# fruttasecca/approximated_personalized_pagerank

Measured on AMD Instinct MI355X. Metric: source-nodes/sec grank K=64 L=128 on RMAT-22; 1/2/4/8 MI355X + HBM GB/s, higher is better.
Workload: dtype f64

## Files before the change

approximated_personalized_pagerank_amd/csrc/grank.hip:

```cpp
#include <hip/hip_runtime.h>
#include <rccl/rccl.h>
#include <hipcub/hipcub.hpp>

#include <algorithm>
#include <atomic>
#include <chrono>
#include <cmath>
#include <condition_variable>
#include <cstdio>
#include <cstdlib>
#include <cstring>
#include <mutex>
#include <new>
#include <thread>
#include <vector>

#include "../../include/ppr_hip.h"
#include "merge_wave.h"
#include "wg_merge.h"
#include "merge_hub.h"
#include "merge_glb.h"
#include "merge_hot.h"
#include "merge_xs.h"
#include "merge_sv.h"
// ... 48 lines not shown
    for (int j = 0; j < l; j++) below += (uint32_t)__shfl((int)slot, j) == slot;
    if (below == 0) bad |= prev != 0xffffffffull;
    else bad |= (uint32_t)prev == 0xffffffffu || got != below;
    wave_fence();
  }
  if (bad) atomicAnd(&ok[1], 0);
}

}

int plan_alloc(int64_t n, const int64_t* row_ptr, const int32_t* colx, uint32_t K, uint32_t L,
               double damping, const ppr_opts* o, ppr_plan** out, bool mc) {
  const int64_t m = n ? row_ptr[n] : 0;
  for (int64_t v = 0; v < n; v++)
    if ((row_ptr[v + 1] - row_ptr[v]) * (int64_t)L + 1 > (int64_t)INT32_MAX) return PPR_ERR_RANGE;
  ppr_plan* p = new (std::nothrow) ppr_plan();
  if (!p) return PPR_ERR_OOM;
  p->n = n; p->m = m; p->K = K; p->L = L; p->damping = damping;
  p->Lp = pow2_at_least(L);
  p->flags = o ? o->flags : 0;
  p->device = (o && o->device >= 0) ? o->device : -1;
  if (p->device >= 0) { if (hipSetDevice(p->device) != hipSuccess) { plan_free(p); return PPR_ERR_HIP; } }
  else { if (hipGetDevice(&p->device) != hipSuccess) { plan_free(p); return PPR_ERR_HIP; } }
  if (o && o->stream) p->stream = (hipStream_t)o->stream;
  else {
    if (hipStreamCreateWithFlags(&p->stream, hipStreamNonBlocking) != hipSuccess) { plan_free(p); return PPR_ERR_HIP; }
    p->own_stream = true;
  }
  if (hipEventCreate(&p->ev_a) != hipSuccess || hipEventCreate(&p->ev_b) != hipSuccess ||
      hipEventCreate(&p->ev_m0) != hipSuccess || hipEventCreate(&p->ev_m1) != hipSuccess) { plan_free(p); return PPR_ERR_HIP; }

  {
    const char* env = getenv("PPR_TIER_MASK");
    const int mask = env ? (int)strtol(env, nullptr, 0) : 0xef;
    int T0 = 256;
    for (int t = 0; t < NT; t++) {
      const int T = T0 << t;
      if (!((mask >> t) & 1) || lds_wave_bytes(T, p->Lp) * WAVES_PER_BLOCK > 160 * 1024) { p->tierT[t] = 0; p->tierCap[t] = 0; continue; }
      p->tierT[t] = T;
      p->tierCap[t] = T / 4 * 3;
    }
    p->tierCap[NT] = 0;
    p->wg_lds = wg_lds_bytes(WG_T, p->Lp, wg_pl(p->Lp));
    const int pmax = WG_TIER_PASSES;
    p->hub_enabled = ((mask >> (NT + 1)) & 1) && pmax >= 1 && p->wg_lds <= 160 * 1024;
    if (((mask >> NT) & 1) && pmax >= 1 && p->wg_lds <= 160 * 1024)
      p->tierCap[NT] = pmax * WG_PASS_CAP;
    int run = 0;
    for (int t = 0; t <= NT; t++) {
      if (!p->tierCap[t]) continue;
      if (p->tierCap[t] < run) p->tierCap[t] = 0;
      else run = p->tierCap[t];
    }
  }
  std::vector<int32_t> all(n > 0 ? n : 1);
  {
    int64_t k = 0;
    for (int64_t v = 0; v < n; v++)
      if (row_ptr[v + 1] > row_ptr[v]) all[k++] = (int32_t)v;
    p->n_nd = k;
    for (int64_t v = 0; v < n; v++)
      if (row_ptr[v + 1] == row_ptr[v]) all[k++] = (int32_t)v;
  }
  p->h_rp.assign(row_ptr, row_ptr + n + 1);
  for (int64_t v = 0; v < n; v++) p->max_deg = std::max<int64_t>(p->max_deg, row_ptr[v + 1] - row_ptr[v]);

  const size_t slab = (size_t)2 * n * L;
  TRY(dalloc(&p->d_rp, n + 1));
  TRY(dalloc(&p->d_colx, m));
  TRY(dalloc(&p->d_part, n));
  TRY(dalloc(&p->d_ids, slab));
  TRY(dalloc(&p->d_sc, slab));
  TRY(dalloc(&p->d_len, 2 * n));
  TRY(dalloc(&p->d_rix, (size_t)2 * n * NRANGE));
  TRY(dalloc(&p->d_rmin, 2 * n));
  TRY(dalloc(&p->d_all, n));
  TRY(dalloc(&p->d_cand, n));
  TRY(dalloc(&p->d_tier_lists, (size_t)NLISTS * (n > 0 ? n : 1)));
  TRY(dalloc(&p->d_tier_cnt, NLISTS + 2));
  TRY(dalloc(&p->d_big, n));
  TRY(dalloc(&p->d_tier_cap, NT + 1));
  TRY(dalloc(&p->d_ovf, n));
  TRY(dalloc(&p->d_maxdiff, PPR_MAX_ITER_STATS + 1));
  TRY(dalloc(&p->d_stats, PPR_NSTATS));
  TRY(dalloc(&p->d_out_ids, (size_t)n * K));
  TRY(dalloc(&p->d_out_sc, (size_t)n * K));
  TRY(dalloc(&p->d_out_len, n));
  if (getenv("PPR_DIAG")) {
    TRY(dalloc(&p->d_diag, PPR_DIAG_SLOTS));
    if (hipMemset(p->d_diag, 0, PPR_DIAG_SLOTS * 8) != hipSuccess) { plan_free(p); return PPR_ERR_HIP; }
  }
  hipStream_t st = p->stream;
  if (n) {
    if (hipMemcpyAsync(p->d_rp, row_ptr, 8 * (n + 1), hipMemcpyHostToDevice, st) != hipSuccess ||
        (m && hipMemcpyAsync(p->d_colx, colx, 4 * m, hipMemcpyHostToDevice, st) != hipSuccess) ||
        hipMemsetAsync(p->d_part, 0, n, st) != hipSuccess ||
        hipMemsetAsync(p->d_len, 0, 8 * n, st) != hipSuccess ||
        hipMemsetAsync(p->d_rix, 0, sizeof(uint16_t) * 2 * n * NRANGE, st) != hipSuccess ||
        hipMemsetAsync(p->d_rmin, 0, 16 * n, st) != hipSuccess ||
        hipMemcpyAsync(p->d_all, all.data(), 4 * n, hipMemcpyHostToDevice, st) != hipSuccess) {
      plan_free(p); return PPR_ERR_HIP;
    }
  }
  int32_t caps[NT + 1];
  for (int t = 0; t <= NT; t++) caps[t] = p->tierCap[t];
  if (hipMemcpyAsync(p->d_tier_cap, caps, sizeof(caps), hipMemcpyHostToDevice, st) != hipSuccess ||
      hipStreamSynchronize(st) != hipSuccess) { plan_free(p); return PPR_ERR_HIP; }
  for (int t = 0; t < NT; t++)
    if (p->tierT[t]) {
      const size_t bytes = lds_wave_bytes(p->tierT[t], p->Lp) * WAVES_PER_BLOCK;
      if (bytes > 64 * 1024) {
        hipFuncSetAttribute((const void*)k_merge_lds<false>, hipFuncAttributeMaxDynamicSharedMemorySize, 160 * 1024);
        hipFuncSetAttribute((const void*)k_merge_lds<true>, hipFuncAttributeMaxDynamicSharedMemorySize, 160 * 1024);
        hipFuncSetAttribute((const void*)k_merge_lds<false, true>, hipFuncAttributeMaxDynamicSharedMemorySize, 160 * 1024);
        hipFuncSetAttribute((const void*)k_merge_lds<true, true>, hipFuncAttributeMaxDynamicSharedMemorySize, 160 * 1024);
      }
    }
  if (p->tierCap[NT])
    hipFuncSetAttribute((const void*)k_merge_wg, hipFuncAttributeMaxDynamicSharedMemorySize, 160 * 1024);
  p->hub_lds_wg = wg_lds_bytes(WG_T, p->Lp, wg_pl(p->Lp));
  p->hub_lds_final = wg_lds_bytes(0, p->Lp, 0);
  {
    const char* e1 = getenv("PPR_HUB_BUCKET");
    const char* e2 = getenv("PPR_HUB_WAVE_T");
    p->hub_bucket = e1 ? std::max(64, atoi(e1)) : (mc ? HUB_BUCKET_MC : HUB_BUCKET);
    p->hub_wave_t = e2 ? (std::max(256, atoi(e2)) + 63) / 64 * 64 : (mc ? HUB_WAVE_T_MC : HUB_WAVE_T);
    p->hub_wave_t = std::min(p->hub_wave_t, 8192);
    const char* e17 = getenv("PPR_BW_FILL");
    const int fill = e17 ? std::max(50, std::min(100, atoi(e17))) : 85;
    p->hub_bw_budget = std::max(WAVE, std::min(p->hub_wave_t, p->hub_wave_t * fill / 100));
  }
  {
    const char* e4 = getenv("PPR_BW_NG");
    const char* e5 = getenv("PPR_BW_WAVES");
    const char* s1 = getenv("PPR_HUB_SEG");
    const char* s2 = getenv("PPR_SEG_BUCKET");
    const char* s3 = getenv("PPR_SEG_T");
    const char* s4 = getenv("PPR_SEG_WPB");
    p->seg_enabled = s1 ? atoi(s1) != 0 : false;

    p->seg_bucket = s2 ? std::max(32, atoi(s2)) : 256;
    p->seg_t = s3 ? pow2_at_least(std::max(256, atoi(s3))) : 512;
    p->seg_t = std::min(p->seg_t, 4096);
    p->seg_wpb = s4 ? std::max(1, std::min(4, atoi(s4))) : 1;
    p->hub_bw_ng = e4 ? (atoi(e4) == 8 ? 8 : atoi(e4) == 4 ? 4 : atoi(e4) == 1 ? 1 : 2) : 2;
    p->hub_bw_waves = e5 ? std::max(1, std::min(4, atoi(e5))) : 1;
    const char* e19 = getenv("PPR_HUB_RANGE");
    if (e19) p->hub_range = std::max(0, std::min(32, atoi(e19)));
    const char* e6 = getenv("PPR_HUB_SLICE");
    p->hub_slice = std::max<int>(std::max<int>(64, (int)L), e6 ? atoi(e6) : HUB_SLICE);
    const char* e21 = getenv("PPR_RED_LDS");
    const size_t red_lds = wg_lds_bytes(0, p->Lp, p->hub_slice);
    p->red_pl = (!(e21 && atoi(e21) == 0) && red_lds <= 160 * 1024) ? p->hub_slice : 0;
    p->hub_lds_red = p->red_pl ? red_lds : p->hub_lds_final;
    if (p->red_pl)
      hipFuncSetAttribute((const void*)k_hub_reduce, hipFuncAttributeMaxDynamicSharedMemorySize, 160 * 1024);
    const char* e7 = getenv("PPR_HUB_STREAMS");
    p->hub_streams = (e7 && atoi(e7) == 1) ? 1 : 2;
    const char* e14 = getenv("PPR_WAVE_WPB");
    p->wave_wpb = e14 ? (atoi(e14) >= 4 ? 4 : atoi(e14) >= 2 ? 2 : 1) : 1;
    const char* e15 = getenv("PPR_TILE_WPB_P");
    p->tile_wpb_p = e15 ? std::max(1, atoi(e15)) : 4096;
    const char* e18 = getenv("PPR_HUB_REGIONS");
    p->hub_regions = e18 ? std::max(2, std::min(ppr_plan::MAX_REGIONS, atoi(e18))) : 3;
    const char* e10 = getenv("PPR_HUB_MIX");
    p->hub_mix = e10 ? std::max(0, std::min(HUB_MAX_LOGP, atoi(e10))) : 6;
    const char* e9 = getenv("PPR_HUB_TILE_PB");
    p->hub_tile_pb = e9 ? std::max(0, std::min(64, atoi(e9))) : HUB_TILE_PER_BUCKET;
    const char* e9b = getenv("PPR_HUB_TILE_CAND");
    if (e9b) p->hub_tile_cand = std::max(256, std::min(1 << 20, atoi(e9b)));
    const char* ets = getenv("PPR_TILE_SPLIT_LOGP");
    if (ets) p->tile_split_logp = std::max(0, std::min(HUB_MAX_LOGP, atoi(ets)));
    const char* esp = getenv("PPR_SPEC");
    if (esp) p->spec_ratio = std::max(0.0, std::min(1.0, atof(esp)));
    const char* esf = getenv("PPR_SPEC_FROM");
    if (esf) p->spec_from = std::max(0, atoi(esf));
    const char* ent = getenv("PPR_NT");
    if (ent) p->nt_loads = (int)strtol(ent, nullptr, 0) & 3;
    const char* ewi = getenv("PPR_WHATIF");
    if (ewi) p->whatif = (int)strtol(ewi, nullptr, 0);
    const char* ebd = getenv("PPR_WAVE_BY_D");
    if (ebd) p->wave_by_d = atoi(ebd) != 0;
    const char* etd = getenv("PPR_WAVE_TDIV");
    if (etd) p->wave_tdiv = std::max(0, std::min(6, atoi(etd)));
    const char* exr = getenv("PPR_XROUTE");
    if (exr && atoi(exr) == 0) p->xroute = false;
    const char* exb = getenv("PPR_XTEST_BADSIZE");
    if (exb) p->xtest_badsize = atoi(exb);
    const char* erp = getenv("PPR_TEST_RANK_PERMUTE");
    p->rank_permute = erp && atoi(erp) != 0;
    const char* exf = getenv("PPR_XTEST_FAIL");
    if (exf && sscanf(exf, "%d,%d", &p->xtest_fail_rank, &p->xtest_fail_it) != 2) p->xtest_fail_rank = -1;
    const char* ext = getenv("PPR_XTIMEOUT");
    if (ext) p->x_timeout_s = std::max(1.0, atof(ext));
    const char* e9e = getenv("PPR_WG_PASSES");
    if (e9e) p->wg_max_passes = std::max(1, std::min(WG_MAX_PASSES, atoi(e9e)));
    const char* e9d = getenv("PPR_FUSED_MAX");
    if (e9d) p->fused_max = std::max(0LL, atoll(e9d));
    const char* e9c = getenv("PPR_HUB_LONG_MIN");
    if (e9c) p->hub_long_min = std::max(0LL, atoll(e9c));
    const char* e8 = getenv("PPR_HUB_BUDGET");
    if (e8) p->hub_budget = std::max<int64_t>(1024, std::min<int64_t>(1LL << 28, atoll(e8)));
    const char* h1 = getenv("PPR_HOT_N");
    const char* h2 = getenv("PPR_HOT_AT");
    const char* h3 = getenv("PPR_HOT_STRIDE");
    if (h1) p->hot_cap = std::max(0, std::min(16384, atoi(h1)));
    if (h2) p->hot_at = std::max(0, atoi(h2));
    if (h3) p->hot_stride = std::max(1, atoi(h3));
    if (hot_wave_lds(p->hot_cap) > 160 * 1024) p->hot_cap = 0;
    const char* h4 = getenv("PPR_HOT_MAX");
    if (h4) p->hot_max_need = std::max(0, atoi(h4));
  }
  {
    const char* e = getenv("PPR_BW2");
    p->hub_bw2 = !(e && atoi(e) == 0);
  }
  p->hub_wave_stride = (int)std::max(hub_wave_lds(p->hub_wave_t, p->hub_bw_ng), p->hub_bw2 ? bw2_lds(p->hub_wave_t) : 0);
  p->hub_lds_wave = (size_t)p->hub_wave_stride * p->hub_bw_waves;
  if (p->hub_streams == 2) {
    const char* epr = getenv("PPR_SV_PRIO");
    int prio_lo = 0, prio_hi = 0;
    hipDeviceGetStreamPriorityRange(&prio_lo, &prio_hi);
    const int prio4 = (epr && atoi(epr) == 1) ? prio_hi : (epr && atoi(epr) == 2) ? prio_lo : 0;
    if (hipStreamCreateWithFlags(&p->stream2, hipStreamNonBlocking) != hipSuccess ||
        hipStreamCreateWithPriority(&p->stream4, hipStreamNonBlocking, prio4) != hipSuccess ||
        hipStreamCreateWithFlags(&p->stream3, hipStreamNonBlocking) != hipSuccess ||
        hipEventCreateWithFlags(&p->ev_wave, hipEventDisableTiming) != hipSuccess) { plan_free(p); return PPR_ERR_HIP; }
    if (hipStreamCreateWithFlags(&p->stream5, hipStreamNonBlocking) != hipSuccess ||
        hipEventCreateWithFlags(&p->ev_hot0, hipEventDisableTiming) != hipSuccess) { plan_free(p); return PPR_ERR_HIP; }
    for (int i = 0; i < ppr_plan::MAX_REGIONS; i++)
      if (hipEventCreateWithFlags(&p->ev_part[i], hipEventDisableTiming) != hipSuccess ||
          hipEventCreateWithFlags(&p->ev_buck[i], hipEventDisableTiming) != hipSuccess ||
          hipEventCreateWithFlags(&p->ev_fin[i], hipEventDisableTiming) != hipSuccess ||
          hipEventCreateWithFlags(&p->ev_hot[i], hipEventDisableTiming) != hipSuccess) { plan_free(p); return PPR_ERR_HIP; }
  }
  p->stream_wave = p->stream3;
  {
    hipDeviceProp_t prop;
    p->num_cus = hipGetDeviceProperties(&prop, p->device) == hipSuccess ? prop.multiProcessorCount : 256;
    const int per_cu = std::max<int>(1, std::min<int>(32 / p->hub_bw_waves, (int)((160 * 1024) / p->hub_lds_wave)));
    p->hub_bw_blocks = p->num_cus * per_cu;
  }
  {
    const char* e = getenv("PPR_LDS_RANK");
    int* d_ok = nullptr;
    int ok[2] = {0, 0};
    if ((!e || atoi(e) != 0) && hipMalloc(&d_ok, sizeof(ok)) == hipSuccess) {
      ok[0] = ok[1] = 1;
      if (hipMemcpy(d_ok, ok, sizeof(ok), hipMemcpyHostToDevice) == hipSuccess) {
        hipFuncSetAttribute((const void*)k_probe_lds_rank, hipFuncAttributeMaxDynamicSharedMemorySize, 160 * 1024);
        hipLaunchKernelGGL(k_probe_lds_rank, dim3((unsigned)p->hub_bw_blocks), dim3(64 * p->hub_bw_waves),
                           p->hub_lds_wave, p->stream, d_ok, 64, p->hub_wave_t,
                           p->hub_wave_stride);
        if (hipGetLastError() != hipSuccess || hipStreamSynchronize(p->stream) != hipSuccess ||
            hipMemcpy(ok, d_ok, sizeof(ok), hipMemcpyDeviceToHost) != hipSuccess)
          ok[0] = ok[1] = 0;
      } else {
        ok[0] = ok[1] = 0;
      }
      hipFree(d_ok);
    }
    p->lds_rank = ok[0] ? 1u : 0u;
    p->lds_rank64 = ok[1] ? 1u : 0u;
// ... 293 lines not shown
  const auto t4 = now();
  std::vector<int32_t> act[2];
  for (int64_t v = 0; v < n; v++)
    if (g->row_ptr[v + 1] > g->row_ptr[v]) act[part[v]].push_back((int32_t)v);
  for (int q = 0; q < 2; q++) {
    p->work[q].resize(act[q].size());
    pprh::parallel_for((int64_t)act[q].size(), nth, [&](int64_t b, int64_t e2, int) {
      for (int64_t i = b; i < e2; i++) {
        const int v = act[q][i];
        double w = 1.0;
        for (int64_t e = g->row_ptr[v]; e < g->row_ptr[v + 1]; e++) {
          const int u = g->col[e];
          w += (double)std::min<int64_t>(L, g->row_ptr[u + 1] - g->row_ptr[u] + 1);
        }
        p->work[q][i] = w;
      }
    });
  }
  if (timing)
    fprintf(stderr, "ppr_timing plan_create partitions_s %.3f colx_s %.3f alloc_upload_s %.3f work_s %.3f\n",
            sec(t0, t1) + part_dev_s, sec(t1, t2), sec(t2, t3), sec(t4, now()));
  p->nact[0] = (int64_t)act[0].size();
  p->nact[1] = (int64_t)act[1].size();
  if (p->hot_cap > 0 && n > 0) {
    std::vector<int32_t> indeg(n, 0);
    for (int64_t e = 0; e < m; e++) indeg[g->col[e]]++;
    p->hot_list_cap = p->hot_cap + 2 * std::min<int64_t>(n, 1 << 20);
    TRY(dalloc(&p->d_hot_bits, (n + 31) / 32));
    TRY(dalloc(&p->d_hot_idx, n));
    TRY(dalloc(&p->d_hot_keys, p->hot_cap));
    TRY(dalloc(&p->d_hot_w, n));
    TRY(dalloc(&p->d_hot_hist, HOT_BINS + 2));
    TRY(dalloc(&p->d_hot_list, p->hot_list_cap));
    TRY(dalloc(&p->d_indeg, n));
    if (hipMemcpy(p->d_indeg, indeg.data(), 4 * (size_t)n, hipMemcpyHostToDevice) != hipSuccess) {
      plan_free(p); return PPR_ERR_HIP;
    }
  } else {
    p->hot_cap = 0;
  }
  TRY(dalloc(&p->d_act[0], p->nact[0]));
  TRY(dalloc(&p->d_act[1], p->nact[1]));
  hipStream_t st = p->stream;
  if (n) {
    if (hipMemcpyAsync(p->d_part, part.data(), n, hipMemcpyHostToDevice, st) != hipSuccess ||
        (p->nact[0] && hipMemcpyAsync(p->d_act[0], act[0].data(), 4 * p->nact[0], hipMemcpyHostToDevice, st) != hipSuccess) ||
        (p->nact[1] && hipMemcpyAsync(p->d_act[1], act[1].data(), 4 * p->nact[1], hipMemcpyHostToDevice, st) != hipSuccess) ||
        hipStreamSynchronize(st) != hipSuccess) {
      plan_free(p); return PPR_ERR_HIP;
    }
  }
  *out = p;
  return PPR_OK;
}

extern "C" void ppr_grank_plan_destroy(ppr_plan* p) { plan_free(p); }
extern "C" void* ppr_grank_plan_stream(ppr_plan* p) { return p ? (void*)p->stream : nullptr; }

static IterArgs iter_args(const ppr_plan* p, int it, bool unit) {
  IterArgs a;
  a.damping = p->damping;
  a.mc = 0u;
  a.rp = p->d_rp;
  a.diag = p->d_diag;
  a.unit = unit ? 1u : 0u;
  a.stats = (p->flags & PPR_FLAG_STATS) ? 1u : 0u;
  a.lds_rank = p->lds_rank;
  a.nt = (uint32_t)p->nt_loads;
  a.whatif = ((uint32_t)p->whatif & 0xffffu) | (p->sv_p2skip ? 0u : WI_SV_NO_P2SKIP) |
             (p->rank_permute ? WI_RANK_PERMUTE : 0u);
  a.iter = unit ? -1 : it;
  a.spec = (unit || p->hot_cap > 0 || it < p->spec_from) ? 0.0 : p->spec_ratio;
  a.xs = p->xsum ? 1u : 0u;
  a.xsf = XS_F;
  if (unit) { a.sA = 0; a.sB = 0; a.active = -1; return a; }
  a.sA = ((it + 1) / 2) & 1;
  a.sB = (it / 2) & 1;
  a.active = it & 1;
  return a;
}

static int run_merge_impl(ppr_plan* p, const IterArgs& a, const int32_t* list, int64_t count,
                          unsigned long long* maxdiff);

static int ensure_scratch(ppr_plan* p, size_t need) {
  if (need <= p->scratch_bytes) return PPR_OK;
  HIP_OK(hipStreamSynchronize(p->stream));
  hipFree(p->d_scratch);
  p->d_scratch = nullptr;
  p->scratch_bytes = 0;
  if (hipMalloc(&p->d_scratch, need) != hipSuccess) return PPR_ERR_OOM;
  p->scratch_bytes = need;
  return PPR_OK;
}

static int ensure_dev(unsigned char** ptr, size_t* cap, size_t need);

static int ceil_log2(int64_t x) { return x <= 1 ? 0 : 64 - __builtin_clzll((unsigned long long)(x - 1)); }

static int run_hubs(ppr_plan* p, const IterArgs& a, const int32_t* big,
                    const int32_t* cand , size_t nbig, unsigned long long* maxdiff,
                    std::vector<int32_t>& fallback, const int32_t* dest = nullptr) {
  hipStream_t st = p->stream;
  DevGraph g{p->d_rp, p->d_colx, p->n};
  const DevSlab s = dev_slab(p);
  const int64_t L = p->L;
  const int64_t budget = p->hub_budget;
  const auto t_plan0 = std::chrono::steady_clock::now();
  p->last_nbig = (int64_t)nbig;
  p->last_maxneed = 0;
  for (size_t i = 0; i < nbig; i++) p->last_maxneed = std::max<int64_t>(p->last_maxneed, cand[i]);
  const int slice = p->hub_slice;
  using Batch = HubBatch;
  std::vector<Batch>& batches = p->hub_batches;
  batches.clear();
  {
    int rc0 = ensure_pinned(&p->h_desc_pin, &p->h_desc_bytes, sizeof(HubDesc) * (nbig + 1));
    if (rc0) return rc0;
  }
  HubDesc* desc = (HubDesc*)p->h_desc_pin;
  size_t nd_all = 0;
  const bool hot = p->hot_n > 0 && !a.unit && !a.mc;
  const HotSet H{p->d_hot_bits, p->d_hot_idx, p->d_hot_keys, hot ? p->hot_n : 0};
  const uint32_t hb = (uint32_t)p->hub_bucket, sgb = (uint32_t)p->seg_bucket;
  auto cdiv32 = [](uint32_t x, uint32_t d) { return x / d + (x % d != 0); };
  auto logp_of = [&](int64_t need) {
    return std::max(1, std::min(HUB_MAX_LOGP, ceil_log2((int64_t)cdiv32((uint32_t)need, hb))));
  };
  std::vector<uint8_t> lpv(nbig);
  if (a.xs) {
    const int64_t capb = (int64_t)p->xr_T * p->xr_fill / 100;
    for (size_t i = 0; i < nbig; i++)
      lpv[i] = (uint8_t)std::max(1, std::min(p->hub_max_logp, ceil_log2((dest[i] + capb - 1) / capb)));
  } else {
    for (size_t i = 0; i < nbig; i++) lpv[i] = (uint8_t)logp_of(cand[i]);
  }
  std::vector<uint32_t> order(nbig);
  if (p->hub_mix > 0) {
    std::vector<uint32_t> lg, sm;
    lg.reserve(nbig);
    sm.reserve(nbig);
    for (size_t i = 0; i < nbig; i++) (lpv[i] >= p->hub_mix ? lg : sm).push_back((uint32_t)i);
    size_t a0 = 0, b0 = 0, k = 0;
    while (a0 < lg.size() || b0 < sm.size()) {
      const bool take_lg = b0 >= sm.size() || (a0 < lg.size() && a0 * sm.size() <= b0 * lg.size());
      order[k++] = take_lg ? lg[a0++] : sm[b0++];
    }
  } else {
    for (size_t i = 0; i < nbig; i++) order[i] = (uint32_t)i;
  }
  const auto t_plan1 = std::chrono::steady_clock::now();
  int64_t need_all = 0;
  for (size_t i = 0; i < nbig; i++) need_all += cand[i];
  const int tile_pb = need_all >= p->hub_long_min ? p->hub_tile_pb : 1;
  int tw_of[HUB_MAX_LOGP + 1], nsl_of[HUB_MAX_LOGP + 1];
  int64_t ptc_of[HUB_MAX_LOGP + 1];
  for (int lp = 0; lp <= HUB_MAX_LOGP; lp++) {
    const int64_t tcand = std::max<int64_t>(p->hub_tile_cand, (int64_t)tile_pb << lp);
    const int64_t tw0 = std::max<int64_t>(1, tcand / L);
    tw_of[lp] = (int)(tw0 > WAVE ? (tw0 + WAVE - 1) / WAVE * WAVE : tw0);
    ptc_of[lp] = (int64_t)(1 << lp) * L;
    nsl_of[lp] = ptc_of[lp] > 2 * slice ? (int)((ptc_of[lp] + slice - 1) / slice) : 0;
  }
  {
    size_t oi = 0;
    while (oi < nbig) {
// ... 387 lines not shown
    const size_t o_b = off;  off = al(off + 8 * (size_t)T);
    const size_t o_st = off; off = al(off + sizeof(XgState));
    const size_t o_h = off;  off = al(off + 4 * (size_t)XG_BINS);
    const size_t o_e = off;  off = al(off + 4);
    const size_t zeroed = off;
    const size_t o_dk = off; off = al(off + 4 * (size_t)XG_CAP);
    const size_t o_dv = off; off = al(off + 8 * (size_t)XG_CAP);
    { int rc = ensure_dev(&p->d_xg, &p->xg_bytes, off); if (rc) return rc; }
    unsigned char* b = p->d_xg;
    uint32_t* keys = (uint32_t*)(b + o_k);
    unsigned long long* A = (unsigned long long*)(b + o_a);
    unsigned long long* B = (unsigned long long*)(b + o_b);
    XgState* stp = (XgState*)(b + o_st);
    uint32_t* hist = (uint32_t*)(b + o_h);
    int32_t* err = (int32_t*)(b + o_e);
    int32_t* dk = (int32_t*)(b + o_dk);
    double* dv = (double*)(b + o_dv);
    HIP_OK(hipMemsetAsync(b, 0, zeroed, st));
    const int64_t deg = p->h_rp[v + 1] - p->h_rp[v];
    const int64_t blocks = std::max<int64_t>(1, (deg + 4 * WAVE - 1) / (4 * WAVE));
    hipLaunchKernelGGL(k_xg_walk, dim3((unsigned)blocks), dim3(256), 0, st, g, s, a, v, T, keys, A, B, stp);
    HIP_OK(hipGetLastError());
    const unsigned gb = (unsigned)std::min<int64_t>(2048, (T + 1023) / 1024);
    for (int lvl = 0; lvl < XG_LEVELS; lvl++) {
      hipLaunchKernelGGL(k_xg_hist, dim3(gb), dim3(1024), 0, st, v, T, keys, A, B, stp, lvl, hist, a.xsf);
      HIP_OK(hipGetLastError());
      hipLaunchKernelGGL(k_xg_pick, dim3(1), dim3(256), 0, st, stp, lvl, hist, (int)p->L, p->xg_cap);
      HIP_OK(hipGetLastError());
    }
    hipLaunchKernelGGL(k_xg_compact, dim3((unsigned)std::min<int64_t>(8192, (T + 255) / 256)), dim3(256), 0, st, v, T,
                       keys, A, B, stp, dk, dv, a.xsf);
    HIP_OK(hipGetLastError());
    hipLaunchKernelGGL(k_xg_fin, dim3(1), dim3(64), xg_fin_lds_bytes(p->Lp), st, s, a, v, stp, dk, dv, p->Lp, maxdiff,
                       p->d_stats, err);
    HIP_OK(hipGetLastError());
    p->merge_launches += 4 + 2 * XG_LEVELS;
    int32_t herr = 0;
    HIP_OK(hipMemcpyAsync(&herr, err, 4, hipMemcpyDeviceToHost, st));
    HIP_OK(hipStreamSynchronize(st));
    if (herr) return PPR_ERR_HIP;
    p->xg_sources++;
  }
  return PPR_OK;
}

static void kst_reset(ppr_plan* p) {
  for (int g = 0; g < ppr_plan::NKST; g++) {
    p->kst_ms[g] = 0.0; p->kst_bytes[g] = 0.0; p->kst_pend_bytes[g] = 0.0;
    p->kst_launches[g] = 0; p->kst_live[g] = false;
  }
}
static void kst_begin(ppr_plan* p, int g, hipStream_t s) {
  if (!p->ev_k[2 * g] && hipEventCreate(&p->ev_k[2 * g]) != hipSuccess) return;
  if (!p->ev_k[2 * g + 1] && hipEventCreate(&p->ev_k[2 * g + 1]) != hipSuccess) return;
  hipEventRecord(p->ev_k[2 * g], s);
}
static void kst_end(ppr_plan* p, int g, hipStream_t s, double bytes) {
  if (!p->ev_k[2 * g + 1]) return;
  hipEventRecord(p->ev_k[2 * g + 1], s);
  p->kst_live[g] = true;
  p->kst_pend_bytes[g] = bytes;
}
static void kst_fold(ppr_plan* p, int g) {
  if (!p->kst_live[g]) return;
  p->kst_live[g] = false;
  float ms = 0.f;
  if (hipEventElapsedTime(&ms, p->ev_k[2 * g], p->ev_k[2 * g + 1]) == hipSuccess) {
    p->kst_ms[g] += ms;
    p->kst_bytes[g] += p->kst_pend_bytes[g];
    p->kst_launches[g]++;
  }
}

struct XhDefer {
  bool want = false;
  bool live = false;
  int depth = 0;
  size_t o_ov = 0;
  const std::vector<int32_t>* src = nullptr;
  const std::vector<int32_t>* cand = nullptr;
  const std::vector<int32_t>* deg = nullptr;
  const std::vector<int64_t>* dest = nullptr;
  std::vector<int32_t> xv;
};
static int xhubs_finish(ppr_plan* p, const IterArgs& a, XhDefer& df, unsigned long long* maxdiff);

static inline void sub_lap(ppr_plan* p, int k, std::chrono::steady_clock::time_point& t) {
  const auto t2 = std::chrono::steady_clock::now();
  p->xh_sub[k] += std::chrono::duration<double>(t2 - t).count();
  t = t2;
}

static int run_xhubs_list(ppr_plan* p, const IterArgs& a, const std::vector<int32_t>& src,
                          const std::vector<int32_t>& cand, const std::vector<int32_t>& deg,
                          const std::vector<int64_t>& dest, unsigned long long* maxdiff, int depth,
                          XhDefer* defer = nullptr) {
  const size_t n = src.size();
  if (!n) return PPR_OK;
  auto tsub = std::chrono::steady_clock::now();
  hipStream_t st = p->stream;
  hipStream_t sw = p->stream3 ? p->stream3 : st;
  DevGraph g{p->d_rp, p->d_colx, p->n};
  const DevSlab s = dev_slab(p);
  const int64_t L = p->L;
  struct Cls { int T, W; };
  const Cls cls[3] = {{std::min(2048, p->xr_T), std::min(2048, p->xr_T) / 512},
                      {std::min(4096, p->xr_T), std::min(4096, p->xr_T) / 512},
                      {p->xr_T, p->xr_T / 512}};
  auto cap_of = [&](int T) { return (int64_t)T * p->xr_fill / 100; };
  static thread_local std::vector<int32_t> rng_tl;
  static thread_local std::vector<uint8_t> ci_tl;
  static thread_local std::vector<XDesc> xd_tl;
  static thread_local std::vector<XTask> tasks_tl[3];
  std::vector<int32_t>& rng = rng_tl;
  std::vector<uint8_t>& ci = ci_tl;
  rng.resize(n);
  ci.resize(n);
  std::vector<int32_t> bsrc, bcand;
  std::vector<int32_t> bdest;
  const int64_t capA = cap_of(p->xr_T);
  const int64_t reach = capA << p->hub_max_logp;
  constexpr int XG_REDO = 8;
  std::vector<int32_t> xgs, xgc;
  for (size_t i = 0; i < n; i++) {
    const int64_t R = std::max<int64_t>(1, (dest[i] + capA - 1) / capA);
    if (depth > XG_REDO || (p->hub_enabled && R > p->xr_rmax && dest[i] > reach)) {
      rng[i] = -1;
      xgs.push_back(src[i]);
      xgc.push_back(cand[i]);
    } else if (R <= p->xr_rmax || !p->hub_enabled) {
      rng[i] = (int32_t)R;
      int c = 2;
      if (R == 1) c = dest[i] <= cap_of(cls[0].T) ? 0 : dest[i] <= cap_of(cls[1].T) ? 1 : 2;
      ci[i] = (uint8_t)c;
    } else {
      rng[i] = 0;
      bsrc.push_back(src[i]);
      bdest.push_back((int32_t)std::min<int64_t>(dest[i], INT32_MAX));
    }
  }
  sub_lap(p, 0, tsub);
  std::vector<XDesc>& xd = xd_tl;
  std::vector<XTask>* tasks = tasks_tl;
  xd.clear();
  for (int c = 0; c < 3; c++) tasks[c].clear();
  xd.reserve(n);
  tasks[0].reserve(n);
  int64_t pt = 0;
  for (int pass = 0; pass < 2; pass++)
    for (size_t i = 0; i < n; i++) {
      if (rng[i] <= 0 || (rng[i] > 1) != (pass == 0)) continue;
      const int32_t d = (int32_t)xd.size();
      XDesc x;
      x.v = src[i];
      x.R = rng[i];
      x.pt_off = pt;
      x.factor = a.mc ? 1.0 : p->damping / (double)deg[i];
      x.selfval = a.mc ? 1.0 / (p->damping / (double)deg[i]) : 1.0 - p->damping;
      pt += rng[i] == 1 ? (int64_t)std::max<int64_t>(L, p->xr_cap) : (int64_t)rng[i] * L;
      xd.push_back(x);
      for (int r = 0; r < rng[i]; r++) tasks[ci[i]].push_back(XTask{d, r});
    }
  sub_lap(p, 1, tsub);
  int64_t nmulti = 0;
  for (const XDesc& x : xd) nmulti += x.R > 1;
  const size_t nx = xd.size();
  const bool use_xm = p->xm && !a.unit && p->Lp <= 2 * WAVE && xm_lds_bytes(cls[0].T) <= 160 * 1024;
  std::vector<XmTask> xmt;
  if (use_xm) {
    xmt.reserve(tasks[0].size());
    for (const XTask& t : tasks[0]) {
      const XDesc& x = xd[(size_t)t.d];
      xmt.push_back(XmTask{x.pt_off, x.factor, x.selfval, t.d, x.v});
    }
    tasks[0].clear();
  }
  size_t ntask = 0;
  for (int c = 0; c < 3; c++) ntask += tasks[c].size();
  auto al = [](size_t x) { return (x + 255) & ~(size_t)255; };
  size_t off = 0;
  const size_t o_d = off;  off = al(off + sizeof(XDesc) * (nx + 1));
  const size_t o_t = off;  off = al(off + sizeof(XTask) * (ntask + 1));
  const size_t o_m = off;  off = al(off + sizeof(XmTask) * (xmt.size() + 1));
  const size_t o_k = off;  off = al(off + 4 * (size_t)(pt + 1));
  const size_t o_s = off;  off = al(off + 8 * (size_t)(pt + 1));
  const size_t o_z = off;
  const size_t o_pc = off; off = al(off + 4 * (nx + 1));
  const size_t o_ds = off; off = al(off + 4 * (nx + 1));
  const size_t o_of = off; off = al(off + 4 * (nx + 1));
  const size_t o_ov = off; off = al(off + 4 * (nx + 2));
  const size_t o_xt = off; off = al(off + 8 * (nx + 1));
  const size_t total = off;
  std::vector<int32_t> ovl_h;
  if (nx) {
    {
      int rc = ensure_dev(&p->d_xs, &p->xs_bytes, total);
      if (rc) return rc;
    }
    unsigned char* b = p->d_xs;
    XDesc* d_xd = (XDesc*)(b + o_d);
    XTask* d_tk = (XTask*)(b + o_t);
    int32_t* d_pk = (int32_t*)(b + o_k);
    double* d_ps = (double*)(b + o_s);
    uint32_t* d_pc = (uint32_t*)(b + o_pc);
    uint32_t* d_ds = (uint32_t*)(b + o_ds);
    int32_t* d_of = (int32_t*)(b + o_of);
    int32_t* d_ov = (int32_t*)(b + o_ov);
    unsigned long long* d_xt = (unsigned long long*)(b + o_xt);
    const size_t up = o_m + sizeof(XmTask) * xmt.size();
    {
      int rc = ensure_pinned(&p->h_xs_pin, &p->h_xs_bytes, up);
      if (rc) return rc;
    }
    unsigned char* hb = (unsigned char*)p->h_xs_pin;
    std::memcpy(hb + o_d, xd.data(), sizeof(XDesc) * nx);
    if (!xmt.empty()) std::memcpy(hb + o_m, xmt.data(), sizeof(XmTask) * xmt.size());
    size_t tofs[3];
    {
      size_t k = 0;
      for (int c = 0; c < 3; c++) {
        tofs[c] = k;
        if (!tasks[c].empty()) std::memcpy(hb + o_t + sizeof(XTask) * k, tasks[c].data(), sizeof(XTask) * tasks[c].size());
        k += tasks[c].size();
      }
    }
    sub_lap(p, 2, tsub);
    HIP_OK(hipMemcpyAsync(b, hb, up, hipMemcpyHostToDevice, sw));
    HIP_OK(hipMemsetAsync(b + o_z, 0, total - o_z, sw));
    if (!a.unit && !a.mc) {
      double bytes = 0.0;
      for (size_t i = 0; i < n; i++)
        if (rng[i] > 0)
          bytes += 8.0 + 8.0 * deg[i] + 12.0 * ((double)cand[i] - 1.0) +
                   24.0 * (double)std::min<int64_t>(L, (int64_t)cand[i] + 1) + 4.0;
      kst_begin(p, 5, sw);
      p->kst_pend_bytes[5] = bytes;
    }
    const bool big_first = p->xr_big_first;
    if (!xmt.empty()) {
      const int T = cls[0].T, W = cls[0].W;
      const int budget = p->xr_budget_over ? 2 * T : std::min(T * 85 / 100, T - W * WAVE - WAVE);
      hipLaunchKernelGGL(k_xm<4>, dim3((unsigned)xmt.size()), dim3(64 * 4), xm_lds_bytes(T), sw, g, s, a,
                         (const XmTask*)(b + o_m), T, budget, d_pk, d_ps, d_pc, d_ds, d_of, d_ov);
      HIP_OK(hipGetLastError());
      p->merge_launches++;
    }
    for (int c0 = 0; c0 < 3; c0++) {
      const int c = big_first ? 2 - c0 : c0;
      if (tasks[c].empty()) continue;
      const int T = cls[c].T, W = cls[c].W;
      const int budget = p->xr_budget_over ? 2 * T : std::min(T * 85 / 100, T - W * WAVE - WAVE);
      hipLaunchKernelGGL(k_xr, dim3((unsigned)tasks[c].size()), dim3(64 * W), xr_lds_bytes(T, W, p->Lp), sw, g, s, a,
                         d_xd, d_tk + tofs[c], T, budget, p->Lp, d_xt, d_pk, d_ps, d_pc, d_ds, d_of, d_ov, p->xr_cap);
      HIP_OK(hipGetLastError());
      p->merge_launches++;
    }
    if (nmulti) {
      hipLaunchKernelGGL(k_xfinal<XDesc>, dim3((unsigned)nmulti), dim3(256), xf_lds_bytes(p->Lp, p->xf_stage), sw, s, a,
                         d_xd, d_xt, d_pk, d_ps, d_pc, d_ds, d_of, p->d_dlast, p->Lp, p->xf_stage, maxdiff, p->d_stats);
      HIP_OK(hipGetLastError());
      p->merge_launches++;
    }
    if ((int64_t)nx > nmulti) {
      hipLaunchKernelGGL(k_xfin1, dim3((unsigned)((int64_t)nx - nmulti)), dim3(64), xf1_lds_bytes(p->Lp), sw, s, a, d_xd,
                         (int)nmulti, d_pk, d_ps, d_pc, d_ds, d_of, p->d_dlast, p->Lp, maxdiff, p->d_stats);
      HIP_OK(hipGetLastError());
      p->merge_launches++;
    }
    if (!a.unit && !a.mc) kst_end(p, 5, sw, p->kst_pend_bytes[5]);
  }
  sub_lap(p, 3, tsub);
  if (defer && defer->want && nx && bsrc.empty() && xgs.empty()) {
    defer->live = true;
    defer->depth = depth;
    defer->o_ov = o_ov;
    defer->src = &src; defer->cand = &cand; defer->deg = &deg; defer->dest = &dest;
    defer->xv.resize(nx);
    for (size_t i = 0; i < nx; i++) defer->xv[i] = xd[i].v;
    return PPR_OK;
  }
  std::vector<int32_t> fallback;
  if (!bsrc.empty()) {
    const size_t nb = bsrc.size();
    std::vector<int32_t> cd(2 * nb);
    {
      size_t k = 0;
      for (size_t i = 0; i < n; i++)
        if (rng[i] == 0) { cd[k] = cand[i]; cd[nb + k] = deg[i]; k++; }
    }
    int rc = run_hubs(p, a, bsrc.data(), cd.data(), nb, maxdiff, fallback, bdest.data());
    if (rc) return rc;
  }
  if (nx) {
    int32_t novf = 0;
    HIP_OK(hipMemcpyAsync(&novf, p->d_xs + o_ov, 4, hipMemcpyDeviceToHost, sw));
    HIP_OK(hipStreamSynchronize(sw));
    kst_fold(p, 5);
    if (novf) {
      std::vector<int32_t> od(novf);
      HIP_OK(hipMemcpyAsync(od.data(), p->d_xs + o_ov + 4, 4 * (size_t)novf, hipMemcpyDeviceToHost, sw));
      HIP_OK(hipStreamSynchronize(sw));
      for (int32_t d : od) fallback.push_back(xd[d].v);
    }
  }
  if (!xgs.empty()) { int rc = run_xg(p, a, xgs, xgc, maxdiff); if (rc) return rc; }
  if (fallback.empty()) return PPR_OK;
  p->xr_redo += (int64_t)fallback.size();
  std::vector<int32_t> rsrc, rcand, rdeg;
  std::vector<int64_t> rdest;
  {
    std::vector<std::pair<int32_t, int32_t>> idx(n);
    for (size_t i = 0; i < n; i++) idx[i] = {src[i], (int32_t)i};
    std::sort(idx.begin(), idx.end());
    for (int32_t v : fallback) {
      auto it = std::lower_bound(idx.begin(), idx.end(), std::make_pair(v, (int32_t)-1));
      if (it == idx.end() || it->first != v) return PPR_ERR_HIP;
      const size_t i = (size_t)it->second;
      rsrc.push_back(src[i]);
      rcand.push_back(cand[i]);
      rdeg.push_back(deg[i]);
      const int64_t grown = 4 * dest[i] + 64;
      rdest.push_back(dest[i] >= (int64_t)cand[i] ? grown : std::min<int64_t>((int64_t)cand[i], grown));
    }
  }
  return run_xhubs_list(p, a, rsrc, rcand, rdeg, rdest, maxdiff, depth + 1);
}

static int xhubs_finish(ppr_plan* p, const IterArgs& a, XhDefer& df, unsigned long long* maxdiff) {
  if (!df.live) return PPR_OK;
  df.live = false;
  hipStream_t sw = p->stream3 ? p->stream3 : p->stream;
  int32_t novf = 0;
  HIP_OK(hipMemcpyAsync(&novf, p->d_xs + df.o_ov, 4, hipMemcpyDeviceToHost, sw));
  HIP_OK(hipStreamSynchronize(sw));
  kst_fold(p, 5);
  if (!novf) return PPR_OK;
  std::vector<int32_t> od(novf);
  HIP_OK(hipMemcpyAsync(od.data(), p->d_xs + df.o_ov + 4, 4 * (size_t)novf, hipMemcpyDeviceToHost, sw));
  HIP_OK(hipStreamSynchronize(sw));
  p->xr_redo += novf;
  const std::vector<int32_t>& dsrc = *df.src;
  const std::vector<int32_t>& dcand = *df.cand;
  const std::vector<int32_t>& ddeg = *df.deg;
  const std::vector<int64_t>& ddest = *df.dest;
  std::vector<std::pair<int32_t, int32_t>> idx(dsrc.size());
  for (size_t i = 0; i < dsrc.size(); i++) idx[i] = {dsrc[i], (int32_t)i};
  std::sort(idx.begin(), idx.end());
  std::vector<int32_t> rsrc, rcand, rdeg;
  std::vector<int64_t> rdest;
  for (int32_t d : od) {
    const int32_t v = df.xv[(size_t)d];
    auto it = std::lower_bound(idx.begin(), idx.end(), std::make_pair(v, (int32_t)-1));
    if (it == idx.end() || it->first != v) return PPR_ERR_HIP;
    const size_t i = (size_t)it->second;
    rsrc.push_back(dsrc[i]);
    rcand.push_back(dcand[i]);
    rdeg.push_back(ddeg[i]);
    const int64_t grown = 4 * ddest[i] + 64;
    rdest.push_back(ddest[i] >= (int64_t)dcand[i] ? grown : std::min<int64_t>((int64_t)dcand[i], grown));
  }
  return run_xhubs_list(p, a, rsrc, rcand, rdeg, rdest, maxdiff, df.depth + 1);
}

struct SvRun {
  std::vector<int32_t> pos;
  size_t o_ovl = 0;
  size_t o_os = 0;
  size_t o_om = 0;
  size_t o_ol = 0;
  size_t o_cnt = 0;
  int part = 0;
  int64_t grid[SvHist::NLIST] = {-1, -1, -1};
  int64_t cnt[SvHist::NLIST] = {0, 0, 0};
  size_t cls_end[4] = {0, 0, 0, 0};
  bool live = false;
};

static int sieve_launch(ppr_plan* p, const IterArgs& a, const std::vector<int32_t>& src,
                        const std::vector<int32_t>& cand, const std::vector<int32_t>& deg, unsigned long long* maxdiff,
                        SvRun& run) {
  const size_t n = src.size();
  run.live = false;
  if (!n) return PPR_OK;
  auto tsub = std::chrono::steady_clock::now();
  DevGraph g{p->d_rp, p->d_colx, p->n};
  const DevSlab s = dev_slab(p);
  const int Lp = p->Lp;
  auto klass = [&](int64_t c) { return c > p->sv_slice ? 0 : c >= p->sv_mid ? 1 : c >= p->sv_small ? 2 : 3; };
  auto step = [](int64_t c) { return std::min(255, (int)(8.0 * std::log2((double)std::max<int64_t>(1, c)))); };
  constexpr int NKEY = 4 * 256;
  std::vector<uint32_t>& cnt = p->xhs.svcnt;
  cnt.assign(NKEY + 1, 0u);
  std::vector<uint16_t>& key = p->xhs.svkey;
  key.resize(n);
  for (size_t i = 0; i < n; i++) {
    key[i] = (uint16_t)(klass(cand[i]) * 256 + (255 - step(cand[i])));
    cnt[key[i] + 1]++;
  }
  for (int k = 0; k < NKEY; k++) cnt[k + 1] += cnt[k];
  const size_t nm = cnt[256], nx = n;
  size_t cls_end[3] = {cnt[512], cnt[768], cnt[NKEY]};
  run.pos.resize(nx);
  for (size_t i = 0; i < n; i++) run.pos[cnt[key[i]]++] = (int32_t)i;
  auto sv_algo_bytes = [&](size_t i) {
    return 8.0 + 8.0 * deg[i] + 12.0 * ((double)cand[i] - 1.0) + 24.0 * (double)p->L + 4.0;
  };
  sub_lap(p, 4, tsub);
  std::vector<SvDesc> desc(nm);
  std::vector<SvTask> tasks;
  int64_t tg_total = 0;
  for (size_t k = 0; k < nm; k++) {
    const size_t i = (size_t)run.pos[k];
    SvDesc& d = desc[k];
    d = SvDesc{};
    d.v = src[i];
    d.S = (int32_t)std::min<int64_t>(((int64_t)cand[i] + p->sv_slice - 1) / p->sv_slice, std::max<int32_t>(1, deg[i]));
    d.factor = p->damping / (double)deg[i];
    d.gsk = (int64_t)k * SV_R * (1 << SV_LARGE.wlog);
    d.gpt = (int64_t)k * 2 * Lp;
    d.tg = pow2_at_least(std::min<int64_t>(2 * (int64_t)d.S * (SV_LARGE.budget + SV_LARGE.threads() + 1),
                                           2 * (int64_t)cand[i] + 64));
    d.gxt = tg_total;
    tg_total += d.tg;
    for (int s2 = 0; s2 < d.S; s2++) tasks.push_back(SvTask{(int32_t)k, s2});
  }
  const size_t nt = tasks.size();
  auto al = [](size_t x) { return (x + 255) & ~(size_t)255; };
  size_t off = 0;
  const size_t o_v = off; off = al(off + 4 * nx);
  const size_t o_d = off; off = al(off + sizeof(SvDesc) * (nm + 1));
  const size_t o_t = off; off = al(off + sizeof(SvTask) * (nt + 1));
  const size_t up = off;
  const size_t o_sk = off; off = al(off + 4 * (size_t)sv_ostride(Lp) * nx);
  const size_t o_sv = off; off = al(off + 8 * (size_t)sv_ostride(Lp) * nx);
  const size_t o_z = off;
  const size_t o_ov = off; off = al(off + 4 * (1 + nx));
  const size_t o_os = off; off = al(off + 4 * (1 + nx));
  const size_t o_om = off; off = al(off + 4 * (1 + nx));
  const size_t o_ol = off; off = al(off + 4 * (1 + nx));
  const size_t o_sn = off; off = al(off + 4 * nx);
  const size_t o_cn = off; off = al(off + 4 * SVC_N);
  const size_t o_of = off; off = al(off + 4 * (nm + 1));
  const size_t o_mk = off; off = al(off + 4 * (nm + 1));
  const size_t o_sd = off; off = al(off + 4 * (size_t)Lp * (nm + 1));
  const size_t o_pt = off; off = al(off + 8 * 2 * (size_t)Lp * nm);
  const size_t o_gs = off; off = al(off + 4 * (size_t)SV_R * ((size_t)1 << SV_LARGE.wlog) * nm);
  const size_t o_gk = off; off = al(off + 4 * (size_t)tg_total);
  const size_t o_ga = off; off = al(off + 8 * (size_t)tg_total);
  const size_t o_gb = off; off = al(off + 8 * (size_t)tg_total);
  const size_t total = off;
  { int r = ensure_dev(&p->d_sv, &p->sv_bytes, total); if (r) return r; }
  { int r = ensure_pinned(&p->h_sv_pin, &p->h_sv_bytes, up); if (r) return r; }
  unsigned char* hb = (unsigned char*)p->h_sv_pin;
  int32_t* hv = (int32_t*)(hb + o_v);
  for (size_t k = 0; k < nx; k++) hv[k] = src[(size_t)run.pos[k]];
  if (nm) std::memcpy(hb + o_d, desc.data(), sizeof(SvDesc) * nm);
  if (nt) std::memcpy(hb + o_t, tasks.data(), sizeof(SvTask) * nt);
  unsigned char* b = p->d_sv;
  hipStream_t s1 = p->stream_sv, s2 = p->stream_sv2, s3 = p->stream_sv3;
  sub_lap(p, 5, tsub);
  HIP_OK(hipMemcpyAsync(b, hb, up, hipMemcpyHostToDevice, s3));
  HIP_OK(hipMemsetAsync(b + o_z, 0, total - o_z, s3));
  HIP_OK(hipEventRecord(p->ev_sv, s3));
  if (s1 != s3) HIP_OK(hipStreamWaitEvent(s1, p->ev_sv, 0));
  if (s2 != s3) HIP_OK(hipStreamWaitEvent(s2, p->ev_sv, 0));
  const int32_t* d_v = (const int32_t*)(b + o_v);
  const SvDesc* d_d = (const SvDesc*)(b + o_d);
  const SvTask* d_t = (const SvTask*)(b + o_t);
  int32_t* d_ov = (int32_t*)(b + o_ov);
  int32_t* d_os = (int32_t*)(b + o_os);
  int32_t* d_om = (int32_t*)(b + o_om);
  int32_t* d_of = (int32_t*)(b + o_of);
  int32_t* d_ol = (int32_t*)(b + o_ol);
  int32_t* d_cn = (int32_t*)(b + o_cn);
  int32_t* d_mk = (int32_t*)(b + o_mk);
  int32_t* d_sd = (int32_t*)(b + o_sd);
  auto seed_on = [&](const SvGeom& G) { return p->sv_reseed && std::min(p->sv_budget, G.budget) >= Lp; };
  auto seed_budget = [&](const SvGeom& G) {
    return std::min(p->sv_reseed_budget >= 0 ? p->sv_reseed_budget : p->sv_budget, G.budget);
  };
  unsigned long long* d_pt = (unsigned long long*)(b + o_pt);
  uint32_t* d_sk = (uint32_t*)(b + o_gs);
  int32_t* d_ok = (int32_t*)(b + o_sk);
  double* d_ovv = (double*)(b + o_sv);
  int32_t* d_on = (int32_t*)(b + o_sn);
  uint32_t* d_gk = (uint32_t*)(b + o_gk);
  unsigned long long* d_ga = (unsigned long long*)(b + o_ga);
  unsigned long long* d_gb = (unsigned long long*)(b + o_gb);
  const size_t lds = sv_lds_bytes(Lp, SV_LARGE);
  run.part = a.active == 1 ? 1 : 0;
  for (int k = 0; k < SvHist::NLIST; k++) run.grid[k] = -1;
  const SvHist& hist = p->sv_hist[run.part];
  auto retry_grid = [&](int list, size_t cnt) {
    const int64_t gr = hist.grid(list, (int64_t)cnt, p->sv_retry_mode);
    run.grid[list] = gr;
    run.cnt[list] = (int64_t)cnt;
    (gr > 0 ? p->sv_retry_launched : p->sv_retry_skipped)++;
    return gr;
  };
  {
    const SvGeom geo[3] = {SV_LARGE, SV_MID, SV_SMALL};
    hipStream_t cs[3] = {s2, s3, s3};
    size_t c0 = nm;
    for (int c = 0; c < 3; c++) {
      const size_t cnt_c = cls_end[c] - c0;
      const int d0 = (int)c0;
      double bytes = 0.0;
      for (size_t k = c0; k < cls_end[c]; k++) bytes += sv_algo_bytes((size_t)run.pos[k]);
      c0 = cls_end[c];
      if (!cnt_c) continue;
      const SvGeom G = geo[c];
      kst_begin(p, 1 + c, cs[c]);
      const bool redo = c == 2 && p->sv_redo_mid;
      const bool redo_l = c == 1 && p->sv_redo_large;
      const bool redo_s = c == 0 && seed_on(G);
      const int64_t gl = (redo_l || redo_s) ? retry_grid(c == 0 ? SvHist::LARGE : SvHist::MID, cnt_c) : -1;
      int32_t* first = redo ? d_os : gl <= 0 ? nullptr : redo_l ? d_om : d_ol;
      const int on = first && seed_on(G) ? 1 : 0;
      const SvSeed sd1{on ? first : nullptr, d_cn, on, 0,
                       gl == 0 ? d_cn + (c == 0 ? SVC_MISS_LARGE : SVC_MISS_MID) : nullptr};
      hipLaunchKernelGGL(k_sv1, dim3((unsigned)cnt_c), dim3(G.threads()), sv_lds_bytes(Lp, G), cs[c], g, s, a, d_v, d0,
                         Lp, G, std::min(p->sv_budget, G.budget), ((redo || redo_l) && first) ? first : d_ov, d_ok,
                         d_ovv, d_on, sd1);
      HIP_OK(hipGetLastError());
      if (gl > 0) {
        const SvSeed sd2{nullptr, d_cn, on, seed_budget(SV_LARGE), nullptr};
        hipLaunchKernelGGL(k_sv1_list, dim3((unsigned)gl), dim3(SV_LARGE.threads()), sv_lds_bytes(Lp, SV_LARGE), cs[c],
                           g, s, a, d_v, first, Lp, SV_LARGE, std::min(p->sv_budget, SV_LARGE.budget), d_ov, d_ok, d_ovv,
                           d_on, sd2);
        HIP_OK(hipGetLastError());
        p->merge_launches++;
      }
      if (redo) {
        const SvSeed sd2{nullptr, d_cn, on, seed_budget(SV_MID), nullptr};
        hipLaunchKernelGGL(k_sv1_redo, dim3((unsigned)std::min<size_t>(cnt_c, 512)), dim3(SV_MID.threads()),
                           sv_lds_bytes(Lp, SV_MID), cs[c], g, s, a, d_v, d_os, Lp, SV_MID,
                           std::min(p->sv_budget, SV_MID.budget), d_ov, d_ok, d_ovv, d_on, sd2);
        HIP_OK(hipGetLastError());
        p->merge_launches++;
      }
      hipLaunchKernelGGL(k_svfin, dim3((unsigned)cnt_c), dim3(64), svfin_lds_bytes(Lp), cs[c], s, a, d_v, d0, d_ok,
                         d_ovv, d_on, Lp, maxdiff, p->d_stats);
      HIP_OK(hipGetLastError());
      kst_end(p, 1 + c, cs[c], bytes);
      p->merge_launches += 2;
    }
  }
  if (nm) {
    double bytes = 0.0;
    for (size_t k = 0; k < nm; k++) bytes += sv_algo_bytes((size_t)run.pos[k]);
    kst_begin(p, 4, s1);
    const bool rs_can = seed_on(SV_LARGE);
    const int64_t gm = rs_can ? retry_grid(SvHist::MULTI, nm) : -1;
    const SvSeed rs{d_mk, d_cn, gm > 0 ? 1 : 0, seed_budget(SV_LARGE), gm == 0 ? d_cn + SVC_MISS_MULTI : nullptr};
    for (int retry = 0; retry <= rs.on; retry++) {
      hipLaunchKernelGGL(k_svA, dim3((unsigned)nt), dim3(SV_THREADS), lds, s1, g, s, a, d_d, d_t, Lp, d_sk, d_pt, rs,
                         d_sd, retry);
      HIP_OK(hipGetLastError());
      hipLaunchKernelGGL(k_svB, dim3((unsigned)nt), dim3(SV_THREADS), lds, s1, g, s, a, d_d, d_t, Lp, p->sv_budget,
                         d_sk, d_pt, d_gk, d_ga, d_gb, d_of, rs, d_sd, retry);
      HIP_OK(hipGetLastError());
      hipLaunchKernelGGL(k_svF, dim3((unsigned)nm), dim3(256), svf_lds_bytes(Lp), s1, s, a, d_d, Lp, d_pt, d_gk, d_ga,
                         d_gb, d_of, d_ov, maxdiff, p->d_stats, rs, d_sd, retry);
      HIP_OK(hipGetLastError());
      p->merge_launches += 3;
      if (!retry && rs.on) {
        hipLaunchKernelGGL(k_svS, dim3((unsigned)nm), dim3(256), 0, s1, s, a, d_d, Lp, d_pt, d_gk, d_ga, d_gb, d_sk,
                           d_of, rs, d_sd);
        HIP_OK(hipGetLastError());
        p->merge_launches++;
      }
    }
    kst_end(p, 4, s1, bytes);
  }
  sub_lap(p, 6, tsub);
  p->sv_sources += (int64_t)nx;
  run.o_ovl = o_ov;
  run.o_os = o_os;
  run.o_om = o_om;
  run.o_ol = o_ol;
  run.o_cnt = o_cn;
  run.cls_end[0] = nm;
  for (int c = 0; c < 3; c++) run.cls_end[1 + c] = cls_end[c];
  run.live = true;
  return PPR_OK;
}

static int sieve_collect(ppr_plan* p, SvRun& run, std::vector<int32_t>& back) {
  if (!run.live) return PPR_OK;
  run.live = false;
  if (p->stream_sv2 != p->stream_sv) {
    HIP_OK(hipEventRecord(p->ev_sv, p->stream_sv2));
    HIP_OK(hipStreamWaitEvent(p->stream_sv, p->ev_sv, 0));
  }
  if (p->stream_sv3 != p->stream_sv) {
    HIP_OK(hipEventRecord(p->ev_sv, p->stream_sv3));
    HIP_OK(hipStreamWaitEvent(p->stream_sv, p->ev_sv, 0));
  }
  int32_t novf = 0, nsm = 0, nmd = 0, nlg = 0, nrs[SVC_N] = {};
  HIP_OK(hipMemcpyAsync(nrs, p->d_sv + run.o_cnt, 4 * SVC_N, hipMemcpyDeviceToHost, p->stream_sv));
  HIP_OK(hipMemcpyAsync(&nlg, p->d_sv + run.o_ol, 4, hipMemcpyDeviceToHost, p->stream_sv));
  HIP_OK(hipMemcpyAsync(&novf, p->d_sv + run.o_ovl, 4, hipMemcpyDeviceToHost, p->stream_sv));
  HIP_OK(hipMemcpyAsync(&nsm, p->d_sv + run.o_os, 4, hipMemcpyDeviceToHost, p->stream_sv));
  HIP_OK(hipMemcpyAsync(&nmd, p->d_sv + run.o_om, 4, hipMemcpyDeviceToHost, p->stream_sv));
  HIP_OK(hipStreamSynchronize(p->stream_sv));
  p->sv_redo_dev += nsm + nmd;
  p->sv_reseed_n += nrs[0];
  p->sv_reseed_ok += nrs[1];
  p->sv_seedless_n += nrs[SVC_SEEDLESS];
  p->sv_seedless_done += nrs[SVC_SEEDLESS_DONE];
  {
    const int64_t first[SvHist::NLIST] = {(int64_t)nlg + nrs[SVC_MISS_LARGE],
                                          (run.grid[SvHist::MID] > 0 ? (int64_t)nmd : 0) + nrs[SVC_MISS_MID],
                                          (int64_t)nrs[SVC_MULTI] + nrs[SVC_MISS_MULTI]};
    for (int k = 0; k < SvHist::NLIST; k++) {
      if (run.grid[k] < 0) continue;
      p->sv_hist[run.part].push(k, first[k], run.cnt[k]);
      p->sv_past_grid += run.grid[k] == 0 ? first[k] : k == SvHist::MULTI ? 0 : std::max<int64_t>(0, first[k] - run.grid[k]);
    }
  }
  for (int g = 1; g < ppr_plan::NKST; g++) kst_fold(p, g);
  if (!novf) return PPR_OK;
  std::vector<int32_t> od(novf);
  HIP_OK(hipMemcpyAsync(od.data(), p->d_sv + run.o_ovl + 4, 4 * (size_t)novf, hipMemcpyDeviceToHost, p->stream_sv));
  HIP_OK(hipStreamSynchronize(p->stream_sv));
  for (int32_t d : od) back.push_back(run.pos[(size_t)d]);
  p->sv_redo += novf;
  return PPR_OK;
}

static int run_xhubs(ppr_plan* p, const IterArgs& a, const int32_t* d_list, int64_t count, unsigned long long* maxdiff) {
  if (count <= 0) return PPR_OK;
  auto now = [] { return std::chrono::steady_clock::now(); };
  double lapv[8] = {0, 0, 0, 0, 0, 0, 0, 0};
  auto lap = [&](int k, std::chrono::steady_clock::time_point& t) {
    const auto t2 = now();
    const double d = std::chrono::duration<double>(t2 - t).count();
    p->xh_s[k] += d;
    lapv[k] += d;
    t = t2;
  };
  auto tl = now();
  const auto t_in = tl;
  struct LapLog {
    ppr_plan* p; const IterArgs& a; double* v; std::chrono::steady_clock::time_point t0;
    ~LapLog() {
      if (!getenv("PPR_SV_LOG")) return;
      const double tot = std::chrono::duration<double>(std::chrono::steady_clock::now() - t0).count();
      fprintf(stderr, "ppr_xh_laps it %d total %.2f gather %.2f classify %.2f sieve_launch %.2f engines %.2f "
              "sieve_wait %.2f handback %.2f\n", a.iter, 1e3 * tot, 1e3 * v[0], 1e3 * v[1], 1e3 * v[2], 1e3 * v[3],
              1e3 * v[4], 1e3 * (v[5] + v[6]));
      const double* u = p->xh_sub;
      fprintf(stderr, "ppr_xh_sub it %d range classes %.2f descriptors %.2f staging %.2f launches %.2f sieve order %.2f "
              "descriptors+staging %.2f launches %.2f\n", a.iter, 1e3 * u[0], 1e3 * u[1], 1e3 * u[2], 1e3 * u[3],
              1e3 * u[4], 1e3 * u[5], 1e3 * u[6]);
      for (int k = 0; k < 8; k++) p->xh_sub[k] = 0.0;
    }
  } laplog{p, a, lapv, t_in};
  hipStream_t st = p->stream;
  const size_t nh = (size_t)count;
  {
    size_t capb = p->h_hub_cap * 12;
    void* ptr = p->h_hub_pin;
    int r = ensure_pinned(&ptr, &capb, 20 * nh);
    if (r) return r;
    p->h_hub_pin = (int32_t*)ptr;
    p->h_hub_cap = capb / 12;
  }
  if (4 * nh > (size_t)p->n) { int r = ensure_dev((unsigned char**)&p->d_gath, &p->gath_bytes, 16 * nh); if (r) return r; }
  int32_t* d_g = 4 * nh > (size_t)p->n ? p->d_gath : p->d_ovf;
  int32_t* h = p->h_hub_pin;
  HIP_OK(hipMemcpyAsync(h, d_list, 4 * nh, hipMemcpyDeviceToHost, st));
  hipLaunchKernelGGL(k_gather_sv, dim3((unsigned)((nh + 255) / 256)), dim3(256), 0, st, d_list, (int64_t)nh,
                     p->d_cand, p->d_rp, (const int32_t*)p->d_dlast, dev_slab(p), a, d_g);
  HIP_OK(hipGetLastError());
  HIP_OK(hipMemcpyAsync(h + nh, d_g, 16 * nh, hipMemcpyDeviceToHost, st));
  HIP_OK(hipStreamSynchronize(st));
  std::vector<int32_t>& hcopy = p->xhs.h;
  hcopy.assign(h, h + 5 * nh);
  h = hcopy.data();
  lap(0, tl);
  const bool sieve = p->sv_enabled && a.xs && !a.unit && !a.mc && p->hot_n == 0;
  std::vector<int32_t>& src = p->xhs.src; std::vector<int32_t>& cand = p->xhs.cand;
  std::vector<int32_t>& deg = p->xhs.deg; std::vector<int32_t>& ssrc = p->xhs.ssrc;
  std::vector<int32_t>& scand = p->xhs.scand; std::vector<int32_t>& sdeg = p->xhs.sdeg;
  std::vector<int32_t>& sidx = p->xhs.sidx;
  std::vector<int64_t>& dest = p->xhs.dest;
  src.clear(); cand.clear(); deg.clear(); ssrc.clear(); scand.clear(); sdeg.clear(); sidx.clear(); dest.clear();
  auto estimate = [&](size_t i) {
    const int64_t dl = h[3 * nh + i];
    const int64_t c = (int64_t)h[nh + i];
    int64_t x = std::min<int64_t>(c, dl > 0 ? dl + dl / 8 + 64 : c * 3 / 5 + 64);
    if (p->xr_dscale != 100) x = std::max<int64_t>(1, x * p->xr_dscale / 100);
    return x;
  };
  src.reserve(nh); cand.reserve(nh); deg.reserve(nh); dest.reserve(nh);
  if (sieve) { ssrc.reserve(nh); scand.reserve(nh); sdeg.reserve(nh); sidx.reserve(nh); }
  const bool seedless = sieve && p->sv_seedless && p->sv_reseed && std::min(p->sv_budget, SV_SMALL.budget) >= p->Lp;
  const SvHist& hist = p->sv_hist[a.active == 1 ? 1 : 0];
  auto retried = [&](int list) {
    return hist.grid(list, 1, p->sv_retry_mode) > 0;
  };
  const bool short_large = seedless && retried(SvHist::LARGE);
  const bool short_mid = seedless && p->sv_redo_large && retried(SvHist::MID);
  auto short_ok = [&](int64_t c) {
    if (c > p->sv_slice) return false;
    return c >= p->sv_mid ? short_large : c >= p->sv_small ? short_mid : p->sv_redo_mid;
  };
  for (size_t i = 0; i < nh; i++) {
    const int32_t c = h[nh + i];
    if (sieve && c >= p->sv_min && c < (1 << 30) &&
        (h[4 * nh + i] == (int32_t)p->L || (seedless && short_ok(c)))) {
      ssrc.push_back(h[i]);
      scand.push_back(c);
      sdeg.push_back(h[2 * nh + i]);
      sidx.push_back((int32_t)i);
    } else {
      src.push_back(h[i]);
      cand.push_back(c);
      deg.push_back(h[2 * nh + i]);
      dest.push_back(estimate(i));
    }
  }
  lap(1, tl);
  SvRun run;
  const int64_t rl0 = p->sv_retry_launched, rp0 = p->sv_retry_skipped;
  XhDefer df;
  df.want = p->xh_first && src.size() > ssrc.size();
  if (df.want) { int r = run_xhubs_list(p, a, src, cand, deg, dest, maxdiff, 0, &df); if (r) return r; }
  if (!ssrc.empty()) { int r = sieve_launch(p, a, ssrc, scand, sdeg, maxdiff, run); if (r) return r; }
  lap(2, tl);
  if (df.want) {
    int r = xhubs_finish(p, a, df, maxdiff);
    if (r) return r;
  } else if (!src.empty()) {
    int r = run_xhubs_list(p, a, src, cand, deg, dest, maxdiff, 0);
    if (r) return r;
  }
  lap(3, tl);
  std::vector<int32_t>& back = p->xhs.back;
  back.clear();
  const int64_t dev0 = p->sv_redo_dev, rs0 = p->sv_reseed_n, rk0 = p->sv_reseed_ok;
  const int64_t pg0 = p->sv_past_grid, sl0 = p->sv_seedless_n, sd0 = p->sv_seedless_done;
  { int r = sieve_collect(p, run, back); if (r) return r; }
  lap(4, tl);
  if (getenv("PPR_SV_LOG")) {
    long long hn[4] = {0, 0, 0, 0}, hc[4] = {0, 0, 0, 0}, sc = 0;
    std::vector<int32_t> desc_of(ssrc.size(), 0);
    for (size_t d = 0; d < run.pos.size(); d++) desc_of[(size_t)run.pos[d]] = (int32_t)d;
    for (size_t k = 0; k < back.size(); k++) {
      int c = 0;
      while (c < 3 && (size_t)desc_of[(size_t)back[k]] >= run.cls_end[c]) c++;
      hn[c]++;
      hc[c] += h[nh + (size_t)sidx[(size_t)back[k]]];
    }
    for (int32_t c : scand) sc += c;
    fprintf(stderr, "ppr_sv_log it %d sieved %zu range %zu dev_redo %lld handed_back %zu sieved_cand %lld "
            "hb_large %lld %lld hb_mid %lld %lld hb_small %lld %lld hb_multi %lld %lld reseed %lld reseed_ok %lld "
            "retry_launched %lld retry_skipped %lld past_grid %lld seedless %lld seedless_done %lld\n",
            a.iter, ssrc.size(), src.size(), (long long)(p->sv_redo_dev - dev0), back.size(), sc, hn[1], hc[1], hn[2],
            hc[2], hn[3], hc[3], hn[0], hc[0], (long long)(p->sv_reseed_n - rs0), (long long)(p->sv_reseed_ok - rk0),
            (long long)(p->sv_retry_launched - rl0), (long long)(p->sv_retry_skipped - rp0),
            (long long)(p->sv_past_grid - pg0), (long long)(p->sv_seedless_n - sl0),
            (long long)(p->sv_seedless_done - sd0));
  }
  if (back.empty()) return PPR_OK;
  src.clear(); cand.clear(); deg.clear(); dest.clear();
  for (int32_t k : back) {
    const size_t i = (size_t)sidx[(size_t)k];
    src.push_back(h[i]);
    cand.push_back(h[nh + i]);
    deg.push_back(h[2 * nh + i]);
    dest.push_back(estimate(i));
  }
  lap(5, tl);
  const int r = run_xhubs_list(p, a, src, cand, deg, dest, maxdiff, 0);
  lap(6, tl);
  return r;
}

int run_merge(ppr_plan* p, const IterArgs& a, const int32_t* list, int64_t count,
              unsigned long long* maxdiff) {
  if (count <= 0) return PPR_OK;
  if (!a.mc) HIP_OK(hipEventRecord(p->ev_m0, p->stream));
  p->wave_x_launched = false;
  int rc = run_merge_impl(p, a, list, count, maxdiff);
  if (p->stream_wave && p->stream_wave != p->stream) {
    HIP_OK(hipEventRecord(p->ev_wave, p->stream_wave));
    HIP_OK(hipStreamWaitEvent(p->stream, p->ev_wave, 0));
  }
  if (!rc && p->wave_x_launched) {
    int32_t nw = 0;
    HIP_OK(hipMemcpyAsync(&nw, p->d_wovl, 4, hipMemcpyDeviceToHost, p->stream));
    HIP_OK(hipStreamSynchronize(p->stream));
    if (nw) {
      p->wave_redo += nw;
      rc = run_xhubs(p, a, p->d_wovl + 1, nw, maxdiff);
    }
  }
  if (rc || a.mc) return rc;
  HIP_OK(hipEventRecord(p->ev_m1, p->stream));
  HIP_OK(hipEventSynchronize(p->ev_m1));
  kst_fold(p, 0);
  float ms = 0.f;
  HIP_OK(hipEventElapsedTime(&ms, p->ev_m0, p->ev_m1));
  if (!a.unit) p->merge_ms += ms;
  return PPR_OK;
}

static int run_glb(ppr_plan* p, const IterArgs& a, std::vector<int32_t>& big, unsigned long long* maxdiff) {
  hipStream_t st = p->stream;
  DevGraph g{p->d_rp, p->d_colx, p->n};
  const DevSlab s = dev_slab(p);
  if (big.empty()) return PPR_OK;
  std::vector<int32_t> cand(p->n);
  HIP_OK(hipMemcpyAsync(cand.data(), p->d_cand, 4 * (size_t)p->n, hipMemcpyDeviceToHost, st));
  HIP_OK(hipStreamSynchronize(st));
  const size_t budget_slots = (size_t)1 << 26;
  size_t i0 = 0;
  while (i0 < big.size()) {
    std::vector<GlbWork> work;
    int64_t off = 0;
    size_t i = i0;
    while (i < big.size()) {
      const int64_t T = pow2_at_least(std::max<int64_t>(2 * (int64_t)cand[big[i]], 64));
      if (!work.empty() && (size_t)(off + T) > budget_slots) break;
      work.push_back(GlbWork{big[i], 0, off, T});
      off += T;
      i++;
    }
    const size_t need = (size_t)off * 24;
    if (need > p->scratch_bytes) {
      hipFree(p->d_scratch);
      p->d_scratch = nullptr;
      if (hipMalloc(&p->d_scratch, need) != hipSuccess) return PPR_ERR_OOM;
      p->scratch_bytes = need;
    }
    if ((int64_t)work.size() > p->work_cap) {
      hipFree(p->d_work);
      if (hipMalloc((void**)&p->d_work, sizeof(GlbWork) * work.size()) != hipSuccess) return PPR_ERR_OOM;
      p->work_cap = (int64_t)work.size();
    }
    HIP_OK(hipMemcpyAsync(p->d_work, work.data(), sizeof(GlbWork) * work.size(), hipMemcpyHostToDevice, st));
    int32_t* gkeys = (int32_t*)p->d_scratch;
    double* gacc = (double*)((char*)p->d_scratch + (size_t)off * 4);
    int32_t* ckeys = (int32_t*)((char*)p->d_scratch + (size_t)off * 12);
    double* cacc = (double*)((char*)p->d_scratch + (size_t)off * 16);
    const size_t lds = (size_t)p->Lp * 12 + 1024 + (size_t)p->Lp * 4 * 5;
    hipLaunchKernelGGL(k_merge_glb, dim3((unsigned)work.size()), dim3(64), lds, st, g, s, a,
                       p->d_work, (int64_t)work.size(), gkeys, gacc, ckeys, cacc, p->Lp, maxdiff,
                       p->d_stats);
    HIP_OK(hipGetLastError());
    p->merge_launches++;
    HIP_OK(hipStreamSynchronize(st));
    i0 = i;
  }
  return PPR_OK;
}

static int flush_ovl(ppr_plan* p, const IterArgs& a, unsigned long long* maxdiff) {
  int32_t* ovl = p->ovl_pending;
  if (!ovl) return PPR_OK;
  p->ovl_pending = nullptr;
  hipStream_t st = p->stream;
  int32_t novf = 0;
  HIP_OK(hipMemcpyAsync(&novf, ovl, 4, hipMemcpyDeviceToHost, st));
  HIP_OK(hipStreamSynchronize(st));
  if (!novf) return PPR_OK;
  if (p->d_diag) fprintf(stderr, "ppr_diag: deferred hub overflow redo %d\n", novf);
  std::vector<int32_t> big(novf);
  HIP_OK(hipMemcpyAsync(big.data(), ovl + 1, 4 * (size_t)novf, hipMemcpyDeviceToHost, st));
  HIP_OK(hipStreamSynchronize(st));
  return run_glb(p, a, big, maxdiff);
}

int run_merge_flush(ppr_plan* p, const IterArgs& a, unsigned long long* maxdiff) {
  return flush_ovl(p, a, maxdiff);
}

static int run_merge_impl(ppr_plan* p, const IterArgs& a, const int32_t* list, int64_t count,
                          unsigned long long* maxdiff) {
  hipStream_t st = p->stream;
  DevGraph g{p->d_rp, p->d_colx, p->n};
  const DevSlab s = dev_slab(p);
  const bool fused = a.mc && count <= p->fused_max && GATHER_HDR + 3 * count <= p->n;
  if (!fused) {
    int r = flush_ovl(p, a, maxdiff);
    if (r) return r;
  } else {
    size_t capb = p->h_hub_cap * 12;
    void* ptr = p->h_hub_pin;
    int r = ensure_pinned(&ptr, &capb, 4 * (GATHER_HDR + 3 * (size_t)count));
    if (r) return r;
    p->h_hub_pin = (int32_t*)ptr;
    p->h_hub_cap = capb / 12;
  }
reclassify:
  HIP_OK(hipMemsetAsync(p->d_tier_cnt, 0, sizeof(uint32_t) * (NLISTS + 2), st));
  const int cls_pw = count <= CLS_SMALL ? 1 : CLS_PER_WAVE;
  const int64_t cls_pb = (int64_t)cls_pw * WAVES_PER_BLOCK;
  const int64_t nb = (count + cls_pb - 1) / cls_pb;
  hipLaunchKernelGGL(k_classify, dim3((unsigned)nb), dim3(256), 0, st, g, s, a, list, count,
                     p->d_tier_cap, p->d_tier_lists, p->d_tier_cnt, p->n, p->d_cand, p->d_stats, p->d_big, cls_pw,
                     (p->wave_by_d && a.xs && !a.unit && !a.mc) ? (const int32_t*)p->d_dlast : nullptr);
  HIP_OK(hipGetLastError());
  if (!a.unit && p->max_deg > CLS_BIG_DEG) {
    hipLaunchKernelGGL(k_classify_big, dim3((unsigned)std::min<int64_t>(256, count)), dim3(CLS_BIG_THREADS), 0, st, g,
                       s, a, p->d_tier_cap,
                       p->d_tier_lists, p->d_tier_cnt, p->n, p->d_cand, p->d_stats, p->d_big,
                       (p->wave_by_d && a.xs && !a.unit && !a.mc) ? (const int32_t*)p->d_dlast : nullptr);
  }
  HIP_OK(hipGetLastError());
  uint32_t cnt[NLISTS + 1];
  if (fused) {
    static_assert(NLISTS + 1 < GATHER_HDR, "tier counters and the pending count fit the header");
    hipLaunchKernelGGL(k_gather_cand_deg_dev, dim3((unsigned)((count + 255) / 256)), dim3(256), 0, st,
                       p->d_tier_lists + (int64_t)TIER_BIG * p->n, p->d_tier_cnt, NLISTS + 1, TIER_BIG,
                       p->ovl_pending, count, p->d_cand, p->d_rp, p->d_ovf);
    HIP_OK(hipGetLastError());
    HIP_OK(hipMemcpyAsync(p->h_hub_pin, p->d_ovf, 4 * (GATHER_HDR + 3 * (size_t)count), hipMemcpyDeviceToHost, st));
    HIP_OK(hipStreamSynchronize(st));
    std::memcpy(cnt, p->h_hub_pin, sizeof(cnt));
    const int32_t pend = p->h_hub_pin[NLISTS + 1];
    if (p->ovl_pending) {
      if (pend) {
        int r = flush_ovl(p, a, maxdiff);
        if (r) return r;
        goto reclassify;
      }
      p->ovl_pending = nullptr;
    }
  } else {
    HIP_OK(hipMemcpyAsync(cnt, p->d_tier_cnt, sizeof(cnt), hipMemcpyDeviceToHost, st));
    HIP_OK(hipStreamSynchronize(st));
  }
  hipStream_t sw = p->stream_wave ? p->stream_wave : st;
  bool wave_ev = false;
  WList wls[NT];
  const int wcap = p->wave_cap ? std::max<int>((int)p->L, p->wave_cap) : 2 * p->Lp;
  const size_t wrec = (size_t)wcap * 12 + 4;
  const int64_t wchunk = std::max<int64_t>(1, (int64_t)((p->wl_max - 512) / wrec));
  {
    int64_t most = 0;
    for (int t = 0; t < NT; t++) {
      wls[t] = WList{nullptr, nullptr, nullptr, 0};
      const int split_T = a.xs ? p->wave_split_T : a.mc ? p->wave_split_mc : p->wave_split_chain;
      if (!cnt[t] || !p->tierT[t] || a.unit || split_T <= 0 || std::max(64, p->tierT[t] >> p->wave_tdiv) < split_T)
        continue;
      wls[t].cap = wcap;
      most = std::max<int64_t>(most, std::min<int64_t>((int64_t)cnt[t], wchunk));
    }
    if (most) {
      int rc = ensure_dev(&p->d_wl, &p->wl_bytes, (size_t)most * wrec + 512);
      if (rc) return rc;
      const size_t nk = (size_t)most * (size_t)wcap;
      for (int t = 0; t < NT; t++)
        if (wls[t].cap) {
          wls[t].v = reinterpret_cast<double*>(p->d_wl);
          wls[t].k = reinterpret_cast<int32_t*>(p->d_wl + nk * 8);
          wls[t].n = reinterpret_cast<int32_t*>(p->d_wl + nk * 12);
        }
    }
  }
#ifndef PPR_WFIN_WPB
#define PPR_WFIN_WPB 1
#endif
  auto launch_wfin = [&](const int32_t* tl, int64_t c, const WList& wl) {
    constexpr int wpb = PPR_WFIN_WPB;
    hipLaunchKernelGGL(k_wfin, dim3((unsigned)((c + wpb - 1) / wpb)), dim3(64 * wpb), wfin_lds_bytes(p->Lp) * wpb, sw, s,
                       a, tl, c, wl, p->Lp, maxdiff, p->d_stats);
    p->merge_launches++;
  };
  for (int t = 0; t < NT; t++) {
    if (!cnt[t] || !p->tierT[t]) continue;
    if (!wave_ev && !a.unit && !a.mc) { kst_begin(p, 0, sw); wave_ev = true; }
    const int wpb = p->wave_wpb;
    const int64_t blocks = ((int64_t)cnt[t] + wpb - 1) / wpb;
    if (a.xs) {
      if (!p->wave_x_launched) HIP_OK(hipMemsetAsync(p->d_wovl, 0, 4, sw));
      p->wave_x_launched = true;
      const int Tw = std::max(64, p->tierT[t] >> p->wave_tdiv);
      const WList wl = wls[t];
      const bool split = wl.cap != 0;
      const int32_t* tl = p->d_tier_lists + (int64_t)t * p->n;
      const size_t wlds = split ? lds_wave_bytes_xs(Tw) : lds_wave_bytes_x(Tw, p->Lp);
      const int64_t step = split ? wchunk : (int64_t)cnt[t];
      for (int64_t c0 = 0; c0 < (int64_t)cnt[t]; c0 += step) {
        const int64_t c = std::min<int64_t>(step, (int64_t)cnt[t] - c0);
        hipLaunchKernelGGL(split ? k_merge_lds_x<true> : k_merge_lds_x<false>, dim3((unsigned)((c + wpb - 1) / wpb)),
                           dim3(64 * wpb), wlds * wpb, sw, g, s, a, tl + c0, c, Tw, p->Lp, maxdiff, p->d_stats,
                           p->d_dlast, p->d_wovl, wl);
        if (split) {
          HIP_OK(hipGetLastError());
          launch_wfin(tl + c0, c, wl);
        }
      }
    } else {
      const int Tw = std::max(64, p->tierT[t] >> p->wave_tdiv);
      const WList wl = wls[t];
      const bool split = wl.cap != 0;
      const int32_t* tl = p->d_tier_lists + (int64_t)t * p->n;
      const size_t bytes = (split ? lds_wave_bytes_s(Tw) : lds_wave_bytes(Tw, p->Lp)) * wpb;
      const bool hk = p->hot_n > 0;
      const int64_t step = split ? wchunk : (int64_t)cnt[t];
      for (int64_t c0 = 0; c0 < (int64_t)cnt[t]; c0 += step) {
        const int64_t c = std::min<int64_t>(step, (int64_t)cnt[t] - c0);
        hipLaunchKernelGGL(split ? (hk ? k_merge_lds<true, true> : k_merge_lds<false, true>)
                                 : (hk ? k_merge_lds<true, false> : k_merge_lds<false, false>),
                           dim3((unsigned)((c + wpb - 1) / wpb)), dim3(64 * wpb), bytes, sw, g, s, a, tl + c0, c, Tw,
                           p->Lp, maxdiff, p->d_stats, wl);
        if (split) {
          HIP_OK(hipGetLastError());
          launch_wfin(tl + c0, c, wl);
        }
      }
    }
    HIP_OK(hipGetLastError());
    p->merge_launches++;
  }
  if (wave_ev) kst_end(p, 0, sw, 0.0);
  if (a.xs) {
    int r = PPR_OK;
    for (int t = 0; t < NT && !r; t++)
      if (cnt[t] && !p->tierT[t]) r = run_xhubs(p, a, p->d_tier_lists + (int64_t)t * p->n, cnt[t], maxdiff);
    if (!r && cnt[TIER_WG]) r = run_xhubs(p, a, p->d_tier_lists + (int64_t)TIER_WG * p->n, cnt[TIER_WG], maxdiff);
    if (!r && cnt[TIER_BIG]) r = run_xhubs(p, a, p->d_tier_lists + (int64_t)TIER_BIG * p->n, cnt[TIER_BIG], maxdiff);
    return r;
  }
  if (cnt[TIER_WG]) {
    hipLaunchKernelGGL(k_merge_wg, dim3(cnt[TIER_WG]), dim3(WG_THREADS), p->wg_lds, st, g, s, a,
                       p->d_tier_lists + (int64_t)TIER_WG * p->n, (int64_t)cnt[TIER_WG], p->d_cand,
                       p->Lp, maxdiff, p->d_stats, p->d_ovf, p->d_tier_cnt + NLISTS, p->wg_max_passes);
    HIP_OK(hipGetLastError());
    p->merge_launches++;
    HIP_OK(hipMemcpyAsync(&cnt[NLISTS], p->d_tier_cnt + NLISTS, 4, hipMemcpyDeviceToHost, st));
    HIP_OK(hipStreamSynchronize(st));
  }
  std::vector<int32_t> big;
  auto pull = [&](const int32_t* dptr, uint32_t k) -> int {
    if (!k) return PPR_OK;
    std::vector<int32_t> tmp(k);
    HIP_OK(hipMemcpyAsync(tmp.data(), dptr, 4 * (size_t)k, hipMemcpyDeviceToHost, st));
    HIP_OK(hipStreamSynchronize(st));
    big.insert(big.end(), tmp.begin(), tmp.end());
    return PPR_OK;
  };
  for (int t = 0; t < NT; t++)
    if (cnt[t] && !p->tierT[t]) { int r = pull(p->d_tier_lists + (int64_t)t * p->n, cnt[t]); if (r) return r; }
  { int r = pull(p->d_ovf, cnt[NLISTS]); if (r) return r; }
  if (cnt[TIER_BIG] && fused) {
    const size_t nh = cnt[TIER_BIG];
    if (p->hub_enabled) {
      int r = run_hubs(p, a, p->h_hub_pin + GATHER_HDR, p->h_hub_pin + GATHER_HDR + count, nh, maxdiff, big);
      if (r) return r;
    } else {
      big.insert(big.end(), p->h_hub_pin + GATHER_HDR, p->h_hub_pin + GATHER_HDR + nh);
    }
  } else if (cnt[TIER_BIG]) {
    const size_t nh = cnt[TIER_BIG];
    {
      size_t capb = p->h_hub_cap * 12;
      void* ptr = p->h_hub_pin;
      int r = ensure_pinned(&ptr, &capb, 12 * nh);
      if (r) return r;
      p->h_hub_pin = (int32_t*)ptr;
      p->h_hub_cap = capb / 12;
    }
    int32_t* hubs = p->h_hub_pin;
    int32_t* hcand = p->h_hub_pin + nh;
    HIP_OK(hipMemcpyAsync(hubs, p->d_tier_lists + (int64_t)TIER_BIG * p->n, 4 * nh, hipMemcpyDeviceToHost, st));
    if (2 * nh > (size_t)p->n) { int r = ensure_dev((unsigned char**)&p->d_gath, &p->gath_bytes, 8 * nh); if (r) return r; }
    int32_t* d_g = 2 * nh > (size_t)p->n ? p->d_gath : p->d_ovf;
    hipLaunchKernelGGL(k_gather_cand_deg, dim3((unsigned)((nh + 255) / 256)), dim3(256), 0, st,
                       p->d_tier_lists + (int64_t)TIER_BIG * p->n, (int64_t)nh, p->d_cand, p->d_rp, d_g);
    HIP_OK(hipGetLastError());
    HIP_OK(hipMemcpyAsync(hcand, d_g, 8 * nh, hipMemcpyDeviceToHost, st));
    HIP_OK(hipStreamSynchronize(st));
    if (p->hub_enabled) {
      int r = run_hubs(p, a, hubs, hcand, nh, maxdiff, big);
      if (r) return r;
    } else {
      big.insert(big.end(), hubs, hubs + nh);
    }
  }
  if (!big.empty() && p->ovl_pending) {
    int r = flush_ovl(p, a, maxdiff);
    if (r) return r;
  }
  return run_glb(p, a, big, maxdiff);
}

static double xs_single_host(double p, int F) {
  uint64_t b;
  std::memcpy(&b, &p, 8);
  int e = (int)((b >> 52) & 0x7ffu);
  uint64_t m = b & ((1ull << 52) - 1ull);
  if (e) m |= 1ull << 52; else e = 1;
  const int sh = e - 1075 + F;
  const unsigned __int128 X = sh >= 0 ? ((unsigned __int128)m << sh) : (sh > -64 ? (unsigned __int128)(m >> -sh) : 0);
  return std::ldexp((double)X, -F);
}

static int init_dangling(ppr_plan* p, const int32_t* list, int64_t cnt) {
  if (cnt <= 0) return PPR_OK;
  const int64_t th = cnt * NRANGE;
  const double seed = p->xsum ? xs_single_host(1.0 - p->damping, XS_F) : 1.0 - p->damping;
  hipLaunchKernelGGL(k_init_dangling, dim3((unsigned)std::min<int64_t>((th + 255) / 256, 1 << 20)), dim3(256), 0,
                     p->stream, dev_slab(p), list, cnt, seed);
  HIP_OK(hipGetLastError());
  return PPR_OK;
}

extern "C" int ppr_grank_plan_init(ppr_plan* p) {
  if (!p) return PPR_ERR_ARG;
  HIP_OK(hipSetDevice(p->device));
  p->md_shared_it = -1;
  p->hot_n = 0;
  p->hot_built_it = -1;
  if (p->d_dlast) HIP_OK(hipMemsetAsync(p->d_dlast, 0, 4 * (size_t)std::max<int64_t>(1, p->n), p->stream));
  p->sv_hist[0] = p->sv_hist[1] = SvHist{};
  IterArgs a = iter_args(p, 0, true);
  int rc = init_dangling(p, p->d_all + p->n_nd, p->n - p->n_nd);
  if (rc) return rc;
  return run_merge(p, a, p->d_all, p->n_nd, p->d_maxdiff + PPR_MAX_ITER_STATS);
}

extern "C" int ppr_grank_plan_active_count(ppr_plan* p, int32_t it, int64_t* count) {
  if (!p || !count || it < 0) return PPR_ERR_ARG;
  *count = p->nact[it & 1];
  return PPR_OK;
}

extern "C" int ppr_grank_plan_iterate(ppr_plan* p, int32_t it, int64_t begin, int64_t end) {
  if (!p || it < 0) return PPR_ERR_ARG;
  HIP_OK(hipSetDevice(p->device));
  const int part = it & 1;
  begin = std::max<int64_t>(0, begin);
  end = std::min<int64_t>(p->nact[part], end);
  if (p->hot_cap > 0 && it == p->hot_at && p->hot_built_it != it) {
    int rc0 = hot_build(p, it);
    if (rc0) return rc0;
    p->hot_built_it = it;
  }
  unsigned long long* md = p->d_maxdiff + (it < PPR_MAX_ITER_STATS ? it : PPR_MAX_ITER_STATS);
  if (it >= PPR_MAX_ITER_STATS && p->md_shared_it != it) {
    HIP_OK(hipMemsetAsync(md, 0, 8, p->stream));
    p->md_shared_it = it;
  }
  if (end <= begin) return PPR_OK;
  IterArgs a = iter_args(p, it, false);
  int rc = run_merge(p, a, p->d_act[part] + begin, end - begin, md);
  if (rc) return rc;
  if (a.stats) {
    const DevSlab s = dev_slab(p);
    const int64_t cnt = end - begin;
    const unsigned blocks = (unsigned)std::min<int64_t>((cnt + 255) / 256, 1024);
    hipLaunchKernelGGL(k_stat_written, dim3(blocks), dim3(256), 0, p->stream, s, a,
                       p->d_act[part] + begin, cnt, p->d_stats);
    HIP_OK(hipGetLastError());
  }
  return PPR_OK;
}

extern "C" int ppr_grank_plan_read_maxdiff(ppr_plan* p, int32_t it, double* maxdiff) {
  if (!p || !maxdiff || it < 0) return PPR_ERR_ARG;
  unsigned long long b = 0;
  HIP_OK(hipMemcpyAsync(&b, p->d_maxdiff + (it < PPR_MAX_ITER_STATS ? it : PPR_MAX_ITER_STATS),
                        8, hipMemcpyDeviceToHost, p->stream));
  HIP_OK(hipStreamSynchronize(p->stream));
  double d;
  std::memcpy(&d, &b, 8);
  *maxdiff = d;
  return PPR_OK;
}

int probe_take() {
  unsigned int v = 0u;
  HIP_OK(hipMemcpyFromSymbol(&v, HIP_SYMBOL(g_probe_err), sizeof(v), 0, hipMemcpyDeviceToHost));
  if (!v) return PPR_OK;
  const unsigned int z = 0u;
  HIP_OK(hipMemcpyToSymbol(HIP_SYMBOL(g_probe_err), &z, sizeof(z), 0, hipMemcpyHostToDevice));
  return PPR_ERR_PROBE;
}

extern "C" int ppr_grank_plan_finish(ppr_plan* p, int32_t iterations_run) {
  if (!p || iterations_run < 0) return PPR_ERR_ARG;
  if (p->n == 0) return PPR_OK;
  HIP_OK(hipSetDevice(p->device));
  const int rc = launch_topk(p, ((iterations_run + 1) / 2) & 1, (iterations_run / 2) & 1, nullptr, 0);
  if (rc) return rc;
  return probe_take();
}

int launch_topk(ppr_plan* p, int sA, int sB, const int8_t* owner, int rank) {
  if (p->n == 0) return PPR_OK;
  const DevSlab s = dev_slab(p);
  const int wpb = p->Lp <= 1024 ? 4 : 1;
  const int64_t blocks = (p->n + wpb - 1) / wpb;
  hipLaunchKernelGGL(k_topk, dim3((unsigned)blocks), dim3(64 * wpb), (size_t)wpb * p->Lp * 12, p->stream, s,
                     p->d_part, sA, sB, (int)p->K, p->Lp, p->d_out_ids, p->d_out_sc, p->d_out_len, owner, rank);
  HIP_OK(hipGetLastError());
  return PPR_OK;
}
// ... 122 lines not shown
    std::vector<int32_t> ti(p->n * L), tl(p->n);
    std::vector<double> ts(p->n * L);
    if (p->n) {
      HIP_OK(hipMemcpyAsync(ti.data(), p->d_ids + (size_t)sl * p->n * L, 4 * p->n * L, hipMemcpyDeviceToHost, st));
      HIP_OK(hipMemcpyAsync(ts.data(), p->d_sc + (size_t)sl * p->n * L, 8 * p->n * L, hipMemcpyDeviceToHost, st));
      HIP_OK(hipMemcpyAsync(tl.data(), p->d_len + (size_t)sl * p->n, 4 * p->n, hipMemcpyDeviceToHost, st));
      HIP_OK(hipStreamSynchronize(st));
    }
    std::vector<std::pair<double, int32_t>> row(L);
    for (int64_t v = 0; v < p->n; v++) {
      const int want = part[v] ? sB : sA;
      if (want != sl) continue;
      const int ln = tl[v];
      if (len) len[v] = ln;
      for (int i = 0; i < ln; i++) {
        const int32_t id = ti[v * L + i];
        row[i] = {ts[v * L + i], id >= 0 ? id : p->h_hot_keys[(uint32_t)id & 0x7fffffffu]};
      }
      std::sort(row.begin(), row.begin() + ln, [](const std::pair<double, int32_t>& x, const std::pair<double, int32_t>& y) {
        return x.first > y.first || (x.first == y.first && x.second < y.second);
      });
      for (size_t i = 0; i < L; i++) {
        const bool in = (int)i < ln;
        if (ids) ids[v * L + i] = in ? row[i].second : -1;
        if (scores) scores[v * L + i] = in ? row[i].first : 0.0;
      }
    }
  }
  return PPR_OK;
}

extern "C" int ppr_grank_plan_row_bytes(ppr_plan* p, int64_t* bytes) {
  if (!p || !bytes) return PPR_ERR_ARG;
  const int64_t Le = ((int64_t)p->L + 1) & ~1LL;
  *bytes = 8 + 4 * Le + 8 * (int64_t)p->L;
  return PPR_OK;
}

static int ensure_dev(unsigned char** ptr, size_t* cap, size_t need);

struct XRange {
  int64_t begin, cnt;
  int nxt;
  const int32_t* list;
};

static int xrange(ppr_plan* p, int32_t it, int64_t begin, int64_t end, XRange* x) {
  if (!p || it < 0) return PPR_ERR_ARG;
  const int part = it & 1;
  begin = std::max<int64_t>(0, begin);
  end = std::min<int64_t>(p->nact[part], end);
  x->begin = begin;
  x->cnt = std::max<int64_t>(0, end - begin);
  const IterArgs a = iter_args(p, it, false);
  x->nxt = ((a.active == 1) ? a.sB : a.sA) ^ 1;
  x->list = p->d_act[part] + begin;
  return PPR_OK;
}

static int xpack_nodes(ppr_plan* p, int nxt, const int32_t* list, int64_t cnt, unsigned char* buf, int64_t* d_total) {
  hipStream_t st = p->stream;
  int64_t* off = reinterpret_cast<int64_t*>(buf);
  if (cnt == 0) {
    HIP_OK(hipMemsetAsync(buf, 0, 8, st));
    if (d_total) hipLaunchKernelGGL(k_xtotal, dim3(1), dim3(64), 0, st, (const int64_t*)off, (int64_t)0, d_total);
    HIP_OK(hipGetLastError());
    return PPR_OK;
  }
  const DevSlab s = dev_slab(p);
  int64_t* sz = reinterpret_cast<int64_t*>(buf + 8 * (cnt + 1));
  hipLaunchKernelGGL(k_xsize, dim3((unsigned)((cnt + 256) / 256)), dim3(256), 0, st, s, nxt, list, cnt, sz);
  size_t tmp = 0;
  HIP_OK(hipcub::DeviceScan::ExclusiveSum(nullptr, tmp, sz, off, (int)(cnt + 1), st));
  int rc = ensure_dev(&p->d_xtmp, &p->xtmp_bytes, tmp);
  if (rc) return rc;
  HIP_OK(hipcub::DeviceScan::ExclusiveSum(p->d_xtmp, tmp, sz, off, (int)(cnt + 1), st));
  hipLaunchKernelGGL(k_xpack, dim3((unsigned)((cnt + 3) / 4)), dim3(256), 0, st, s, nxt, list, cnt, buf);
  if (d_total) hipLaunchKernelGGL(k_xtotal, dim3(1), dim3(64), 0, st, (const int64_t*)off, cnt, d_total);
  HIP_OK(hipGetLastError());
  return PPR_OK;
}

static int xunpack_nodes(ppr_plan* p, int nxt, const int32_t* list, int64_t cnt, const unsigned char* buf) {
  if (cnt == 0) return PPR_OK;
  hipLaunchKernelGGL(k_xunpack, dim3((unsigned)((cnt + 3) / 4)), dim3(256), 0, p->stream, dev_slab(p), nxt, list, cnt,
                     buf);
  HIP_OK(hipGetLastError());
  return PPR_OK;
}

static int xpack(ppr_plan* p, int32_t it, int64_t begin, int64_t end, unsigned char* buf, int64_t cap,
                 int64_t* d_total) {
  XRange x;
  int rc = xrange(p, it, begin, end, &x);
  if (rc) return rc;
  int64_t rb = 0;
  ppr_grank_plan_row_bytes(p, &rb);
  if (!buf || cap < 8 + x.cnt * rb) return PPR_ERR_ARG;
  HIP_OK(hipSetDevice(p->device));
  return xpack_nodes(p, x.nxt, x.list, x.cnt, buf, d_total);
}

static int xunpack(ppr_plan* p, int32_t it, int64_t begin, int64_t end, const unsigned char* buf) {
  XRange x;
  int rc = xrange(p, it, begin, end, &x);
  if (rc) return rc;
  if (x.cnt == 0) return PPR_OK;
  if (!buf) return PPR_ERR_ARG;
  HIP_OK(hipSetDevice(p->device));
  return xunpack_nodes(p, x.nxt, x.list, x.cnt, buf);
}

extern "C" int ppr_grank_plan_pack(ppr_plan* p, int32_t it, int64_t begin, int64_t end, void* dev_buf,
                                   int64_t cap) {
  return xpack(p, it, begin, end, (unsigned char*)dev_buf, cap, nullptr);
}

extern "C" int ppr_grank_plan_unpack(ppr_plan* p, int32_t it, int64_t begin, int64_t end, const void* dev_buf) {
  return xunpack(p, it, begin, end, (const unsigned char*)dev_buf);
}

extern "C" int ppr_grank_plan_fold_maxdiff(ppr_plan* p, int32_t it, double maxdiff) {
  if (!p || it < 0) return PPR_ERR_ARG;
  unsigned long long b;
  std::memcpy(&b, &maxdiff, 8);
  HIP_OK(hipMemcpyAsync(p->d_maxdiff + (it < PPR_MAX_ITER_STATS ? it : PPR_MAX_ITER_STATS), &b, 8,
                        hipMemcpyHostToDevice, p->stream));
  HIP_OK(hipStreamSynchronize(p->stream));
  return PPR_OK;
}

extern "C" int ppr_grank_plan_active_list(ppr_plan* p, int32_t it, int32_t* out) {
  if (!p || !out || it < 0) return PPR_ERR_ARG;
  const int part = it & 1;
  if (p->nact[part])
    HIP_OK(hipMemcpy(out, p->d_act[part], 4 * (size_t)p->nact[part], hipMemcpyDeviceToHost));
  return PPR_OK;
}

#define NCCL_OK(expr)                                                                        \
  do {                                                                                       \
    ncclResult_t _r = (expr);                                                                \
    if (_r != ncclSuccess) {                                                                 \
      fprintf(stderr, "ppr_hip: %s failed: %s\n", #expr, ncclGetErrorString(_r));           \
      return PPR_ERR_HIP;                                                                    \
    }                                                                                        \
  } while (0)

extern "C" int ppr_device_count(int32_t* count) {
  if (!count) return PPR_ERR_ARG;
  int c = 0;
  if (hipGetDeviceCount(&c) != hipSuccess) c = 0;
  *count = c;
  return PPR_OK;
}

extern "C" int ppr_comm_unique_id(void* id_out) {
  if (!id_out) return PPR_ERR_ARG;
  ncclUniqueId id;
  NCCL_OK(ncclGetUniqueId(&id));
  std::memcpy(id_out, &id, sizeof(id));
  return PPR_OK;
}

extern "C" int ppr_grank_plan_comm_init(ppr_plan* p, const void* id, int32_t nranks, int32_t rank) {
  if (!p || !id || nranks < 1 || rank < 0 || rank >= nranks) return PPR_ERR_ARG;
// ... 385 lines not shown
  if (rc) return rc;
  rc = ensure_dev(&p->d_xrecv, &p->xrecv_bytes, std::max<size_t>(8, xo[W]));
  if (rc) return rc;
  const int64_t mine = b[me + 1] - b[me];
  const int32_t* ml = p->d_act[q] + b[me];
  unsigned char* buf = p->d_xsend;
  int64_t* off = reinterpret_cast<int64_t*>(buf);
  if (mine == 0) {
    HIP_OK(hipMemsetAsync(buf, 0, 8, s));
  } else {
    int64_t* rsz = reinterpret_cast<int64_t*>(buf + 8 * (mine + 1));
    hipLaunchKernelGGL(k_osize, dim3((unsigned)((mine + 256) / 256)), dim3(256), 0, s, p->d_out_len, ml, mine, rsz);
    size_t tmp = 0;
    HIP_OK(hipcub::DeviceScan::ExclusiveSum(nullptr, tmp, rsz, off, (int)(mine + 1), s));
    rc = ensure_dev(&p->d_xtmp, &p->xtmp_bytes, tmp);
    if (rc) return rc;
    HIP_OK(hipcub::DeviceScan::ExclusiveSum(p->d_xtmp, tmp, rsz, off, (int)(mine + 1), s));
    hipLaunchKernelGGL(k_opack, dim3((unsigned)((mine + 3) / 4)), dim3(256), 0, s, p->d_out_ids, p->d_out_sc,
                       p->d_out_len, (int)K, ml, mine, buf);
    HIP_OK(hipGetLastError());
  }
  p->x_bytes += (int64_t)xo[W];
  rc = x_blocks(p, b, sz, xo, s);
  if (rc) return rc;
  for (int r = 0; r < W; r++) {
    const int64_t c = b[r + 1] - b[r];
    if (r == me || !c) continue;
    hipLaunchKernelGGL(k_ounpack, dim3((unsigned)((c + 3) / 4)), dim3(256), 0, s, p->d_out_ids, p->d_out_sc,
                       p->d_out_len, (int)K, p->d_act[q] + b[r], c, p->d_xrecv + xo[r]);
    HIP_OK(hipGetLastError());
  }
  return PPR_OK;
}

extern "C" int ppr_grank_plan_ends_time(ppr_plan* p, int32_t world, int32_t rank, int32_t iterations_run,
                                        int32_t what, double* ms_out) {
  if (!p || world < 1 || rank < 0 || rank >= world || world > 127 || iterations_run < 0 || what < 0 || what > 1)
    return PPR_ERR_ARG;
  HIP_OK(hipSetDevice(p->device));
  hipStream_t s = p->stream;
  std::vector<int64_t> bd[2];
  shard_bounds(p->work[0], world, bd[0]);
  shard_bounds(p->work[1], world, bd[1]);
  float ms = 0.f;
  if (what == 0) {
    if (!p->d_xowner) { int rc = dalloc(&p->d_xowner, p->n); if (rc) return rc; }
    HIP_OK(hipMemsetAsync(p->d_xowner, 0xff, (size_t)p->n, s));
    for (int q = 0; q < 2; q++) {
      if (!p->nact[q]) continue;
      XBounds xb{};
      xb.world = world;
      for (int r = 0; r <= world; r++) xb.b[r] = bd[q][r];
      hipLaunchKernelGGL(k_xowner, dim3((unsigned)((p->nact[q] + 255) / 256)), dim3(256), 0, s, p->d_act[q],
                         p->nact[q], xb, p->d_xowner);
    }
    HIP_OK(hipGetLastError());
    HIP_OK(hipEventRecord(p->ev_a, s));
    int rc = launch_topk(p, ((iterations_run + 1) / 2) & 1, (iterations_run / 2) & 1, p->d_xowner, rank);
    if (rc) return rc;
  } else {
    const int64_t m0 = bd[0][rank + 1] - bd[0][rank], m1 = bd[1][rank + 1] - bd[1][rank];
    if (!p->d_own) { int rc = dalloc(&p->d_own, std::max<int64_t>(1, p->n)); if (rc) return rc; }
    p->own_world = 0;
    if (m0) HIP_OK(hipMemcpyAsync(p->d_own, p->d_act[0] + bd[0][rank], 4 * (size_t)m0, hipMemcpyDeviceToDevice, s));
    if (m1) HIP_OK(hipMemcpyAsync(p->d_own + m0, p->d_act[1] + bd[1][rank], 4 * (size_t)m1, hipMemcpyDeviceToDevice, s));
    HIP_OK(hipEventRecord(p->ev_a, s));
    IterArgs a = iter_args(p, 0, true);
    int rc = init_dangling(p, p->d_all + p->n_nd, p->n - p->n_nd);
    if (rc) return rc;
    rc = run_merge(p, a, p->d_own, m0 + m1, p->d_maxdiff + PPR_MAX_ITER_STATS);
    if (rc) return rc;
  }
  HIP_OK(hipEventRecord(p->ev_b, s));
  HIP_OK(hipEventSynchronize(p->ev_b));
  hipEventElapsedTime(&ms, p->ev_a, p->ev_b);
  if (ms_out) *ms_out = ms;
  return probe_take();
}

static int run_sharded_impl(ppr_plan* p, uint32_t iterations, double tolerance, ppr_stats* st) {
  if (iterations == 0) return PPR_ERR_ITERS;
  if (p->nranks > 1 && !p->comm && !p->lgroup) return PPR_ERR_ARG;
  HIP_OK(hipSetDevice(p->device));
  hipStream_t s = p->stream;
  HIP_OK(hipMemsetAsync(p->d_maxdiff, 0, 8 * (PPR_MAX_ITER_STATS + 1), s));
  HIP_OK(hipMemsetAsync(p->d_stats, 0, 8 * PPR_NSTATS, s));
  p->merge_launches = 0;
  p->merge_ms = 0.0;
  p->x_bytes = 0;
  p->x_rows_sent = 0;
  HIP_OK(hipEventRecord(p->ev_a, s));
  std::vector<int64_t> bd[2];
  shard_bounds(p->work[0], p->nranks, bd[0]);
  shard_bounds(p->work[1], p->nranks, bd[1]);
  const bool route = p->nranks > 1 && p->nranks <= 32 && p->xroute;
  const bool shard_ends = route && p->xshard_ends;
  XRoute xr;
  int rc = PPR_OK;
  if (route) { rc = xroute_build(p, bd, xr); if (rc) return rc; }
  rc = shard_ends ? init_sharded(p, bd, xr) : ppr_grank_plan_init(p);
  if (rc) return rc;
  double md[2] = {tolerance, tolerance};
  uint32_t it = 0;
  for (; it < iterations && std::max(md[0], md[1]) >= tolerance; it++) {
    const std::vector<int64_t>& b = bd[it & 1];
    rc = ppr_grank_plan_iterate(p, (int32_t)it, b[p->rank], b[p->rank + 1]);
    if (rc) return rc;
    if (p->rank == p->xtest_fail_rank && (int)it == p->xtest_fail_it) return PPR_ERR_HIP;
    unsigned long long* mdp = p->d_maxdiff + (it < PPR_MAX_ITER_STATS ? it : PPR_MAX_ITER_STATS);
    if (p->nranks > 1) {
      rc = route ? x_exchange_routed(p, it, xr) : x_exchange_bulk(p, it, bd[it & 1]);
      if (rc) return rc;
      rc = x_allreduce_max(p, mdp, s);
      if (rc) return rc;
      rc = x_sync(p, s);
      if (rc) return rc;
    }
    if (tolerance > 0) {
      double d = 0.0;
      rc = ppr_grank_plan_read_maxdiff(p, (int32_t)it, &d);
      if (rc) return rc;
      md[0] = d;
      std::swap(md[0], md[1]);
    }
  }
  if (shard_ends) {
    rc = x_sync(p, s);
    if (rc) return rc;
    rc = launch_topk(p, ((it + 1) / 2) & 1, (it / 2) & 1, p->d_xowner, p->rank);
    if (rc) return rc;
    for (int q = 0; q < 2; q++) {
      rc = x_gather_topk(p, q, bd[q]);
      if (rc) return rc;
    }
    rc = probe_take();
    if (rc) return rc;
  } else {
    if (route)
      for (int q = 0; q < 2; q++) {
        const int64_t last = (int64_t)it - 1 - (((int64_t)it - 1 - q) & 1);
        if (last < 0 || (last & 1) != q) continue;
        rc = x_exchange_bulk(p, (uint32_t)last, bd[q]);
        if (rc) return rc;
      }
    rc = x_sync(p, s);
    if (rc) return rc;
    rc = ppr_grank_plan_finish(p, (int32_t)it);
    if (rc) return rc;
  }
  HIP_OK(hipEventRecord(p->ev_b, s));
  rc = x_sync_event(p, p->ev_b);
  if (rc) return rc;
  if (st) {
    rc = read_maxdiff_history(p, it, st);
    if (rc) return rc;
    float ms = 0;
    hipEventElapsedTime(&ms, p->ev_a, p->ev_b);
    st->iterations_run = (int32_t)it;
    st->device_ms = ms;
    st->merge_ms = p->merge_ms;
    unsigned long long sv[2];
    HIP_OK(hipMemcpyAsync(sv, p->d_stats, 16, hipMemcpyDeviceToHost, s));
    HIP_OK(hipStreamSynchronize(s));
    st->candidates = (int64_t)sv[0];
    st->algo_bytes = (int64_t)sv[1];
    st->merge_launches = p->merge_launches;
// ... 269 lines not shown
```

approximated_personalized_pagerank_amd/csrc/mccp2.hip:

```cpp
#include <hip/hip_runtime.h>

#include <algorithm>
#include <cmath>
#include <cstring>
#include <new>
#include <vector>

#include "plan.h"
#include "merge_mc.h"

namespace {
int mc_table_slots(uint32_t L) {
  return pow2_at_least(((int64_t)L + 64) * 3 / 2);
}
}

extern "C" int ppr_mccp2_plan_create(const ppr_csr* g, uint32_t K, uint32_t L, double damping,
                                     const ppr_opts* o, ppr_plan** out) {
  if (!g || !out || g->n < 0 || (g->n > 0 && !g->row_ptr)) return PPR_ERR_ARG;
  if (g->n > 0 && g->row_ptr[g->n] > 0 && !g->col) return PPR_ERR_ARG;
  int rc = check_params(K, L, 1, damping);
  if (rc != PPR_OK) return rc;
  if (L > (uint32_t)MAX_L) return PPR_ERR_RANGE;
  if (g->n >= (1LL << 31) - 1) return PPR_ERR_RANGE;
// ... 5 lines not shown
  std::vector<int32_t> order(n > 0 ? n : 1);
  if (n) { rc = ppr_execution_order_csr(g, order.data()); if (rc) return rc; }
  std::vector<int32_t> pos(n > 0 ? n : 1);
  for (int64_t i = 0; i < n; i++) pos[order[i]] = (int32_t)i;

  std::vector<int32_t> colx(m > 0 ? m : 1);
  std::vector<uint8_t> inW(n > 0 ? n : 1, 0);
  for (int64_t v = 0; v < n; v++)
    for (int64_t e = rp[v]; e < rp[v + 1]; e++) {
      const int32_t s = g->col[e];
      const bool walk = pos[s] >= pos[v];
      colx[e] = s | (walk ? (int32_t)0x80000000 : 0);
      if (walk) inW[s] = 1;
    }
  std::vector<int32_t> level(n > 0 ? n : 1, -1);
  int32_t maxlev = -1;
  for (int64_t i = 0; i < n; i++) {
    const int32_t v = order[i];
    if (rp[v + 1] == rp[v]) continue;
    int32_t lv = 0;
    for (int64_t e = rp[v]; e < rp[v + 1]; e++)
      if (colx[e] >= 0) lv = std::max(lv, level[colx[e]] + 1);
    level[v] = lv;
    maxlev = std::max(maxlev, lv);
  }
  ppr_plan* p = nullptr;
  rc = plan_alloc(n, rp, colx.data(), K, L, damping, o, &p, true);
  if (rc) return rc;
  p->mc = true;
  std::vector<int64_t> off(maxlev + 2, 0);
  std::vector<int32_t> walk, dang;
  for (int64_t v = 0; v < n; v++) {
    if (level[v] >= 0) off[level[v] + 1]++;
    else dang.push_back((int32_t)v);
    if (inW[v]) walk.push_back((int32_t)v);
  }
  for (int32_t l = 0; l <= maxlev; l++) off[l + 1] += off[l];
  std::vector<int32_t> byl(off[maxlev + 1] > 0 ? off[maxlev + 1] : 1);
  {
    std::vector<int64_t> fill(off.begin(), off.end() - 1);
    for (int64_t i = 0; i < n; i++) {
      const int32_t v = order[i];
      if (level[v] >= 0) byl[fill[level[v]]++] = v;
    }
  }
  p->mc_level_off = off;
  p->mc_nwalk = (int64_t)walk.size();
  p->mc_ndangling = (int64_t)dang.size();
  p->mc_T = mc_table_slots(L);
  TRY(dalloc(&p->d_mc_walk, walk.size()));
  TRY(dalloc(&p->d_mc_levels, byl.size()));
  TRY(dalloc(&p->d_mc_dangling, dang.size()));
  hipStream_t st = p->stream;
  if ((!walk.empty() && hipMemcpyAsync(p->d_mc_walk, walk.data(), 4 * walk.size(), hipMemcpyHostToDevice, st) != hipSuccess) ||
      (off[maxlev + 1] > 0 && hipMemcpyAsync(p->d_mc_levels, byl.data(), 4 * (size_t)off[maxlev + 1], hipMemcpyHostToDevice, st) != hipSuccess) ||
      (!dang.empty() && hipMemcpyAsync(p->d_mc_dangling, dang.data(), 4 * dang.size(), hipMemcpyHostToDevice, st) != hipSuccess) ||
      hipStreamSynchronize(st) != hipSuccess) {
    plan_free(p);
    return PPR_ERR_HIP;
  }
  const size_t lds = mc_wave_lds(p->mc_T);
  if (lds > 160 * 1024) { plan_free(p); return PPR_ERR_RANGE; }
  if (lds > 64 * 1024)
    hipFuncSetAttribute((const void*)k_mc_walk, hipFuncAttributeMaxDynamicSharedMemorySize, 160 * 1024);
  *out = p;
  return PPR_OK;
}

extern "C" int ppr_mccp2_plan_info(ppr_plan* p, int64_t* walk_nodes, int64_t* levels, int64_t* dangling) {
  if (!p || !p->mc) return PPR_ERR_ARG;
  if (walk_nodes) *walk_nodes = p->mc_nwalk;
  if (levels) *levels = (int64_t)p->mc_level_off.size() - 1;
  if (dangling) *dangling = p->mc_ndangling;
  return PPR_OK;
}

extern "C" int ppr_mccp2_plan_walk(ppr_plan* p, uint32_t walks, uint64_t seed, int64_t begin, int64_t end) {
  if (!p || !p->mc) return PPR_ERR_ARG;
  if (walks == 0) return PPR_ERR_ITERS;
  begin = std::max<int64_t>(0, begin);
  end = std::min<int64_t>(p->mc_nwalk, end);
  if (end <= begin) return PPR_OK;
  HIP_OK(hipSetDevice(p->device));
  McArgs m;
  m.R = walks;
  m.nw = (uint64_t)((double)walks * p->damping);
  m.damping = p->damping;
  m.seed = seed;
  m.T = p->mc_T;
  m.slot = 1;
  DevGraph g{p->d_rp, p->d_colx, p->n};
  const DevSlab s = dev_slab(p);
  HIP_OK(hipEventRecord(p->ev_m0, p->stream));
  hipLaunchKernelGGL(k_mc_walk, dim3((unsigned)(end - begin)), dim3(64), mc_wave_lds(p->mc_T), p->stream, g, s, m,
                     p->d_mc_walk + begin, end - begin);
  HIP_OK(hipGetLastError());
  HIP_OK(hipEventRecord(p->ev_m1, p->stream));
  HIP_OK(hipEventSynchronize(p->ev_m1));
  float ms = 0.f;
  HIP_OK(hipEventElapsedTime(&ms, p->ev_m0, p->ev_m1));
  p->mc_walk_ms += ms;
  p->mc_walks += (int64_t)m.nw * (end - begin);
  return PPR_OK;
}

extern "C" int ppr_mccp2_plan_combine(ppr_plan* p) {
  if (!p || !p->mc) return PPR_ERR_ARG;
  if (p->n == 0) return PPR_OK;
  HIP_OK(hipSetDevice(p->device));
  const DevSlab s = dev_slab(p);
  if (p->mc_ndangling) {
    hipLaunchKernelGGL(k_mc_selfrow, dim3((unsigned)((p->mc_ndangling + 3) / 4)), dim3(256), 0, p->stream, s,
                       p->d_mc_dangling, p->mc_ndangling, 0);
    HIP_OK(hipGetLastError());
  }
  IterArgs a;
  a.sA = 0;
  a.sB = 1;
  a.active = 0;
  a.damping = p->damping;
  a.unit = 0u;
  a.stats = (p->flags & PPR_FLAG_STATS) ? 1u : 0u;
  a.mc = 1u;
  a.xs = p->xsum ? 1u : 0u;
  a.xsf = XS_F_MC;
  a.rp = p->d_rp;
  a.diag = p->d_diag;
  a.lds_rank = p->lds_rank;
  a.nt = (uint32_t)p->nt_loads;
  a.whatif = ((uint32_t)p->whatif & 0xffffu) | (p->rank_permute ? WI_RANK_PERMUTE : 0u);
  a.iter = -1;
  a.spec = 0.0;
  const int64_t nl = (int64_t)p->mc_level_off.size() - 1;
  HIP_OK(hipEventRecord(p->ev_m0, p->stream));
  p->ovl_pending = nullptr;
  const bool lvlog = getenv("PPR_MC_LEVEL_LOG") != nullptr;
  for (int64_t l = 0; l < nl; l++) {
    const int64_t b = p->mc_level_off[l], e = p->mc_level_off[l + 1];
    if (lvlog) { HIP_OK(hipEventRecord(p->ev_a, p->stream)); p->last_nbig = p->last_maxneed = 0; }
    int rc = run_merge(p, a, p->d_mc_levels + b, e - b, p->d_maxdiff + PPR_MAX_ITER_STATS);
    if (rc) return rc;
    if (lvlog) {
      HIP_OK(hipEventRecord(p->ev_b, p->stream));
      HIP_OK(hipEventSynchronize(p->ev_b));
      float ms = 0.f;
      hipEventElapsedTime(&ms, p->ev_a, p->ev_b);
      fprintf(stderr, "mc_level %lld %lld %lld %lld %.4f\n", (long long)l, (long long)(e - b),
              (long long)p->last_nbig, (long long)p->last_maxneed, ms);
    }
  }
  {
    int rc = run_merge_flush(p, a, p->d_maxdiff + PPR_MAX_ITER_STATS);
    if (rc) return rc;
  }
  HIP_OK(hipEventRecord(p->ev_m1, p->stream));
  HIP_OK(hipEventSynchronize(p->ev_m1));
  {
    float ms = 0.f;
    HIP_OK(hipEventElapsedTime(&ms, p->ev_m0, p->ev_m1));
    p->merge_ms += ms;
  }
  {
    const int rc = launch_topk(p, 0, 0);
    if (rc) return rc;
  }
  {
    const int rc = probe_take();
    if (rc) return rc;
  }
  unsigned int v = 0u;
  HIP_OK(hipMemcpyFromSymbol(&v, HIP_SYMBOL(g_probe_err), sizeof(v), 0, hipMemcpyDeviceToHost));
  if (v) {
    const unsigned int z = 0u;
    HIP_OK(hipMemcpyToSymbol(HIP_SYMBOL(g_probe_err), &z, sizeof(z), 0, hipMemcpyHostToDevice));
    return PPR_ERR_PROBE;
  }
  return PPR_OK;
}

extern "C" int ppr_mccp2_plan_run(ppr_plan* p, uint32_t walks, uint64_t seed, ppr_mc_stats* st) {
  if (!p || !p->mc) return PPR_ERR_ARG;
  if (walks == 0) return PPR_ERR_ITERS;
  HIP_OK(hipSetDevice(p->device));
  hipStream_t s = p->stream;
  HIP_OK(hipMemsetAsync(p->d_stats, 0, 8 * PPR_NSTATS, s));
  p->merge_launches = 0;
  p->merge_ms = 0.0;
  p->mc_walk_ms = 0.0;
  p->mc_walks = 0;
  HIP_OK(hipEventRecord(p->ev_a, s));
  int rc = ppr_mccp2_plan_walk(p, walks, seed, 0, p->mc_nwalk);
  if (rc) return rc;
// ... 53 lines not shown
```

approximated_personalized_pagerank_amd/csrc/merge_wave.h:

```cpp
#pragma once
#include <type_traits>

#include "ppr_common.h"

namespace pprk {

constexpr int CLS_PER_WAVE = 16;
constexpr int CLS_PER_BLOCK = CLS_PER_WAVE * WAVES_PER_BLOCK;
constexpr int64_t CLS_SMALL = 65536;
constexpr int CLS_BIG_DEG = 512;
constexpr int CLS_BIG_THREADS = 1024;

__device__ __forceinline__ long long succ_len_sum(const DevGraph& g, const DevSlab& s, const IterArgs& a,
                                                  int64_t i0, int64_t e, int stride) {
  long long c = 0;
  int64_t i = i0;
  for (; i + 3 * (int64_t)stride < e; i += 4 * (int64_t)stride) {
    int32_t cx[4];
#pragma unroll
    for (int k = 0; k < 4; k++) cx[k] = g.colx[i + k * (int64_t)stride];
#pragma unroll
    for (int k = 0; k < 4; k++) c += s.len[s.lrow(read_slot(a, cx[k]), cx[k] & 0x7fffffff)];
  }
  for (; i < e; i += stride) {
// ... 57 lines not shown
      my_c += (unsigned long long)c;
      my_b += (unsigned long long)(8 + 8 * (e - b) + 12 * c + 12 * ownlen);
      if (t < NT) my_w += (unsigned long long)(8 + 8 * (e - b) + 12 * c + 12 * ownlen);
    }
  }
  __syncthreads();
  if (threadIdx.x < NLISTS) {
    uint32_t n = 0;
    for (int i = 0; i < per_block; i++) n += s_tier[i] == (int)threadIdx.x;
    s_base[threadIdx.x] = n ? atomicAdd(&tier_cnt[threadIdx.x], n) : 0u;
  }
  if (a.stats && lane_id() == 0) { s_red[0][wv] = my_c; s_red[1][wv] = my_b; s_red[2][wv] = my_w; }
  __syncthreads();
  if ((int)threadIdx.x < per_block) {
    const int t = s_tier[threadIdx.x];
    if (t >= 0) {
      uint32_t r = 0;
      for (int i = 0; i < (int)threadIdx.x; i++) r += s_tier[i] == t;
      tier_lists[(int64_t)t * list_cap + s_base[t] + r] = s_src[threadIdx.x];
    }
  }
  if (a.stats && threadIdx.x == 0) {
    unsigned long long sc = 0, sb = 0, sw = 0;
    for (int i = 0; i < WAVES_PER_BLOCK; i++) { sc += s_red[0][i]; sb += s_red[1][i]; sw += s_red[2][i]; }
    if (sc) atomicAdd(&stats[0], sc);
    if (sb) atomicAdd(&stats[1], sb);
    if (sw) atomicAdd(&stats[2], sw);
  }
}

__global__ void __launch_bounds__(CLS_BIG_THREADS) k_classify_big(DevGraph g, DevSlab s, IterArgs a,
                                                                  const int32_t* tier_cap, int32_t* tier_lists,
                                                                  uint32_t* tier_cnt, int64_t list_cap,
                                                                  int32_t* cand, unsigned long long* stats,
                                                                  const int32_t* big_list, const int32_t* dlast) {
  __shared__ long long red[CLS_BIG_THREADS / WAVE];
  const uint32_t nbig = __hip_atomic_load(&tier_cnt[NLISTS + 1], __ATOMIC_RELAXED, __HIP_MEMORY_SCOPE_AGENT);
  for (uint32_t i = blockIdx.x; i < nbig; i += gridDim.x) {
    const int v = big_list[i];
    const int64_t b = g.rp[v], e = g.rp[v + 1];
    long long c = succ_len_sum(g, s, a, b + threadIdx.x, e, CLS_BIG_THREADS);
#pragma unroll
    for (int o = 32; o; o >>= 1) c += __shfl_xor(c, o);
    if (lane_id() == 0) red[threadIdx.x >> 6] = c;
    __syncthreads();
    if (threadIdx.x == 0) {
      c = 0;
      for (int k = 0; k < CLS_BIG_THREADS / WAVE; k++) c += red[k];
      const int64_t need = c + 1;
      cand[v] = (int32_t)(need > 0x7fffffff ? 0x7fffffff : need);
      int t = 0;
      const int64_t tneed = tier_need(need, dlast, v);
      while (t < NT + 1 && tneed > tier_cap[t]) t++;
      tier_lists[(int64_t)t * list_cap + atomicAdd(&tier_cnt[t], 1u)] = v;
      if (a.stats) {
        const int ownlen = a.mc ? 0 : s.len[s.lrow(a.active == 0 ? a.sA : a.sB, v)];
        atomicAdd(&stats[0], (unsigned long long)c);
        atomicAdd(&stats[1], (unsigned long long)(8 + 8 * (e - b) + 12 * c + 12 * ownlen));
        if (t < NT) atomicAdd(&stats[2], (unsigned long long)(8 + 8 * (e - b) + 12 * c + 12 * ownlen));
      }
    }
    __syncthreads();
  }
}

__global__ void __launch_bounds__(256) k_stat_written(DevSlab s, IterArgs a, const int32_t* list,
                                                      int64_t count, unsigned long long* stats) {
  __shared__ unsigned long long red[WAVES_PER_BLOCK];
  const int nxt = write_slot(a);
  unsigned long long b = 0;
  for (int64_t i = (int64_t)blockIdx.x * blockDim.x + threadIdx.x; i < count; i += (int64_t)gridDim.x * blockDim.x)
    b += 12ull * (unsigned long long)s.len[s.lrow(nxt, list[i])] + 4ull;
#pragma unroll
  for (int o = 32; o; o >>= 1) b += __shfl_xor(b, o);
  if (lane_id() == 0) red[threadIdx.x >> 6] = b;
  __syncthreads();
  if (threadIdx.x == 0) {
    unsigned long long t = 0;
    for (int i = 0; i < WAVES_PER_BLOCK; i++) t += red[i];
    atomicAdd(&stats[1], t);
  }
}

__host__ __device__ constexpr size_t lds_wave_bytes(int T, int Lp) {
  return (size_t)T * 13 + (size_t)Lp * 12 + 1024 + (size_t)Lp * 20;
}

#ifndef PPR_TW_BATCH
#define PPR_TW_BATCH 8
#endif
constexpr int HUB_TW_BATCH = PPR_TW_BATCH;

template <class F, class S>
__device__ __forceinline__ void hub_window_walk_part(const DevGraph& g, const DevSlab& s, const IterArgs& a,
                                                     int64_t i0, int64_t e, uint8_t* fl, F f, S succ, int part,
                                                     int nparts) {
  const int64_t i = i0 + lane_id();
  if (a.unit) {
    const bool valid = i < e;
    if constexpr (std::is_invocable_v<F, bool, int, double, bool, int, int>)
      f(valid, valid ? (g.colx[i] & 0x7fffffff) : 0, 1.0, false, lane_id(), WAVE);
    else
      f(valid, valid ? (g.colx[i] & 0x7fffffff) : 0, 1.0, false);
    return;
  }
  int u = 0, sl = 0, ln = 0;
  unsigned long long rm = 0;
  if (i < e) {
    const int32_t cx = g.colx[i];
    u = cx & 0x7fffffff;
    sl = read_slot(a, cx);
    ln = s.len[s.lrow(sl, u)];
    if (S::kWant) rm = dbits(s.rmin[s.lrow(sl, u)]);
  }
  succ(ln, rm);
  const int incl = wave_incl_scan(ln);
  const int total = __builtin_amdgcn_readlane(incl, WAVE - 1);
  const bool flags = fl != nullptr && !__ballot(i < e && ln == 0);
  constexpr bool kRows = std::is_invocable_v<F, bool, int, double, bool, int, int>;
  constexpr int RW = (HUB_TW_BATCH + 3) / 4;
  auto load = [&](int g0, int (&key)[HUB_TW_BATCH], double (&sv)[HUB_TW_BATCH], bool (&one)[HUB_TW_BATCH],
                  uint32_t (&rr)[RW], int (&nr)[HUB_TW_BATCH]) {
    if (kRows)
#pragma unroll
      for (int q = 0; q < RW; q++) rr[q] = 0u;
    if (flags) {
#pragma unroll
      for (int q = 0; q < HUB_TW_BATCH / 4; q++)
        reinterpret_cast<uint32_t*>(fl)[q * WAVE + lane_id()] = 0u;
      wave_fence();
      if (incl > g0 && incl < g0 + WAVE * HUB_TW_BATCH) fl[incl - g0] = 1;
      wave_fence();
    }
#pragma unroll
    for (int k = 0; k < HUB_TW_BATCH; k++) {
      const int c = g0 + k * WAVE + lane_id();
      const bool valid = c < total;
      int j = 0;
      if (flags) {
        const int G = g0 + k * WAVE;
        const uint64_t ends = __ballot(fl[k * WAVE + lane_id()] != 0) & ~1ull;
        j = __popcll(__ballot(incl <= G)) + __popcll(ends & (lanemask_lt() | (1ull << lane_id())));
      } else {
#pragma unroll
        for (int step = 32; step; step >>= 1) {
          const int pv = __shfl(incl, j + step - 1);
          if (pv <= c) j += step;
        }
      }
      const int jj = j < WAVE ? j : WAVE - 1;
      one[k] = !__ballot(valid && jj != __builtin_amdgcn_readlane(jj, 0));
      if (kRows) {
        const uint64_t vm = __ballot(valid);
        const int j0 = __builtin_amdgcn_readlane(jj, 0);
        rr[k / 4] |= (uint32_t)min(jj - j0, 255) << (8 * (k % 4));
        nr[k] = __builtin_amdgcn_readfirstlane(vm ? __shfl(jj, 63 - __clzll((long long)vm)) - j0 + 1 : 1);
      }
      const int exv = __shfl(incl, jj > 0 ? jj - 1 : 0);
      const int ex = jj > 0 ? exv : 0;
      const int uj = __shfl(u, jj);
      const int sj = __shfl(sl, jj);
      key[k] = 0;
      sv[k] = 0.0;
      if (valid) {
        const int64_t r = s.row(sj, uj) + (c - ex);
        key[k] = ld_nt(&s.ids[r], a.nt & 1u);
// ... 151 lines not shown
```

approximated_personalized_pagerank_amd/csrc/plan.h:

```cpp
#pragma once
#include <hip/hip_runtime.h>
#include <rccl/rccl.h>

#include <cstdio>
#include <cstdlib>
#include <vector>

#include "../../include/ppr_hip.h"
#include "ppr_common.h"
#include "sv_plan.h"

using namespace pprk;

#define HIP_OK(expr)                                  \
  do {                                                \
    hipError_t _e = (expr);                           \
    if (_e != hipSuccess) {                           \
      fprintf(stderr, "ppr_hip: %s failed: %s (%s:%d)\n", #expr, hipGetErrorString(_e), __FILE__, __LINE__); \
      return PPR_ERR_HIP;                             \
    }                                                 \
  } while (0)

constexpr int WG_TIER_PASSES = 3;

inline int pow2_at_least(int64_t x) {
  int p = 1;
  while (p < x) p <<= 1;
  return p;
}


struct ppr_plan {
  int device = 0;
  hipStream_t stream = nullptr;
  bool own_stream = false;
  int64_t n = 0, m = 0;
  uint32_t K = 0, L = 0;
  int Lp = 1;
  double damping = 0.85;
  int64_t* d_rp = nullptr;
  int32_t* d_colx = nullptr;
  uint8_t* d_part = nullptr;
  int32_t* d_ids = nullptr;
  double* d_sc = nullptr;
  int32_t* d_len = nullptr;
  uint16_t* d_rix = nullptr;
  double* d_rmin = nullptr;
  int32_t* d_all = nullptr;
  int64_t n_nd = 0;
  int32_t* d_act[2] = {nullptr, nullptr};
  int64_t nact[2] = {0, 0};
  int32_t* d_cand = nullptr;
  int32_t* d_tier_lists = nullptr;
  uint32_t* d_tier_cnt = nullptr;
  int32_t* d_big = nullptr;
  int64_t max_deg = 0;
  int32_t* d_tier_cap = nullptr;
  int32_t* d_ovf = nullptr;
  int tierT[NT] = {0, 0, 0, 0};
  int tierCap[NT + 1] = {0, 0, 0, 0, 0};
  size_t wg_lds = 0;
  int whatif = 0;
  int nt_loads = 0;
  double spec_ratio = 0.0;
  int spec_from = 6;
  int64_t spec_redo = 0;
  int wg_max_passes = 64;
  bool hub_enabled = true;
  unsigned long long* d_maxdiff = nullptr;
  int32_t md_shared_it = -1;
  unsigned long long* d_stats = nullptr;
  static constexpr int NKST = 6;
  hipEvent_t ev_k[2 * NKST] = {};
  bool kst_live[NKST] = {};
  double kst_ms[NKST] = {}, kst_bytes[NKST] = {}, kst_pend_bytes[NKST] = {};
  int64_t kst_launches[NKST] = {};
  GlbWork* d_work = nullptr;
  int64_t work_cap = 0;
  void* d_scratch = nullptr;
  size_t scratch_bytes = 0;
  int32_t* d_out_ids = nullptr;
  double* d_out_sc = nullptr;
  int32_t* d_out_len = nullptr;
  int flags = 0;
  std::vector<int64_t> h_rp;
  size_t hub_lds_count = 0, hub_lds_wg = 0, hub_lds_final = 0, hub_lds_wave = 0;
  size_t hub_lds_red = 0;
  int red_pl = 0;
  int hub_bucket = 448, hub_wave_t = 512;
  int32_t* h_hub_pin = nullptr;
  size_t h_hub_cap = 0;
  void* h_desc_pin = nullptr;
  size_t h_desc_bytes = 0;
  std::vector<HubBatch> hub_batches;
  int32_t* d_gath = nullptr;
  size_t gath_bytes = 0;
  int num_cus = 256;
  int hub_bw_blocks = 0;
  bool rank_permute = false;
  uint32_t lds_rank = 0;
  uint32_t lds_rank64 = 0;
  bool seg_enabled = false;
  int seg_bucket = 256, seg_t = 512, seg_wpb = 1;
  int hub_bw_ng = 2;
  bool hub_bw2 = true;
  int hub_wave_stride = 0;
  int hub_bw_waves = 1;
  int hub_range = 0;
  int hub_slice = 8192;
  ncclComm_t comm = nullptr;
  double x_timeout_s = 600.0;
  int xtest_fail_rank = -1, xtest_fail_it = -1;
  struct LocalGroup* lgroup = nullptr;
// ... 4 lines not shown
  unsigned char* d_xsz = nullptr;
  unsigned char* d_xtmp = nullptr;
  size_t xsend_bytes = 0, xrecv_bytes = 0, xsz_bytes = 0, xtmp_bytes = 0;
  int64_t fused_max = 65536;
  int64_t last_nbig = 0, last_maxneed = 0;
  double host_plan_s = 0.0;
  int64_t host_plan_calls = 0, host_plan_hubs = 0;
  double host_plan_part[2] = {0.0, 0.0};
  int32_t* ovl_pending = nullptr;
  int64_t x_bytes = 0;
  bool xroute = true;
  int xtest_badsize = -1;
  int8_t* d_xowner = nullptr;
  int32_t* d_own = nullptr;
  int64_t own_cnt = 0;
  int own_world = 0, own_rank = -1;
  uint32_t* d_xcmask = nullptr;
  int32_t* d_xlists = nullptr;
  size_t xlists_cap = 0;
  int64_t x_rows_sent = 0;
  int64_t merge_launches = 0;
  double merge_ms = 0.0;
  hipEvent_t ev_a = nullptr, ev_b = nullptr, ev_m0 = nullptr, ev_m1 = nullptr;
  int hub_streams = 2;
  hipStream_t stream_wave = nullptr;
  int wave_wpb = 1;
  int tile_wpb_p = 4096;
  int tile_split_logp = 10;
  int hub_bw_budget = 380;
  int hub_mix = 6;
  int hub_tile_cand = 4096;
  int64_t hub_long_min = 1LL << 26;
  int hub_tile_pb = 16;
  int64_t hub_budget = 1LL << 28;
  static constexpr int MAX_REGIONS = 4;
  int hub_regions = 3;
  hipStream_t stream2 = nullptr, stream3 = nullptr, stream4 = nullptr;
  hipEvent_t ev_part[MAX_REGIONS] = {}, ev_buck[MAX_REGIONS] = {}, ev_fin[MAX_REGIONS] = {}, ev_wave = nullptr;
  unsigned long long* d_diag = nullptr;
  int hot_cap = 0, hot_at = 2, hot_stride = 16;
  int hot_n = 0;
  int32_t hot_built_it = -1;
  std::vector<int32_t> h_hot_keys;
  int hot_max_need = 0x7fffffff;
  double diag_cap_cand = 0.0, diag_cap_src = 0.0;
  double diag_hub_cand = 0.0;
  uint32_t* d_hot_bits = nullptr;
  uint16_t* d_hot_idx = nullptr;
  int32_t* d_hot_keys = nullptr;
  uint32_t* d_hot_w = nullptr;
  uint32_t* d_hot_hist = nullptr;
  int32_t* d_hot_list = nullptr;
  int64_t hot_list_cap = 0;
  int32_t* d_indeg = nullptr;
  hipStream_t stream5 = nullptr;
  hipEvent_t ev_hot0 = nullptr, ev_hot[MAX_REGIONS] = {};
  bool xsum = false;
  int32_t* d_dlast = nullptr;
  int xr_T = 8192, xr_W = 16;
  int xr_rmax = 3;
  int xr_fill = 85;
  int xf_stage = 4096;
  int xr_dscale = 100;
  unsigned char* d_xs = nullptr;
  size_t xs_bytes = 0;
  void* h_xs_pin = nullptr;
  size_t h_xs_bytes = 0;
  int64_t xr_redo = 0;
  int hub_max_logp = 12;
  unsigned char* d_xg = nullptr;
  size_t xg_bytes = 0;
  int64_t xg_sources = 0;
  int32_t* d_wovl = nullptr;
  int wave_split_T = 256;
  int wave_split_chain = 256;
  int wave_split_mc = 0;
  struct XhScratch {
    std::vector<int32_t> h, src, cand, deg, ssrc, scand, sdeg, sidx, back;
    std::vector<int64_t> dest;
    std::vector<uint16_t> svkey;
    std::vector<uint32_t> svcnt;
  } xhs;
  double xh_sub[8] = {0, 0, 0, 0, 0, 0, 0, 0};
  int xr_cap = 0;
  int wave_cap = 0;
  unsigned char* d_wl = nullptr;
  size_t wl_max = (size_t)4 << 30;
  size_t wl_bytes = 0;
  bool wave_x_launched = false;
  int wave_tdiv = 0;
  bool wave_by_d = false;
  bool xr_budget_over = false;
  int64_t wave_redo = 0;
  int xg_cap = 1 << 16;
  bool sv_enabled = false;
  int64_t sv_slice = 1LL << 19;
  bool xm = false;
  bool xr_big_first = false;
  bool xh_first = true;
  bool xshard_ends = true;
  int64_t sv_min = 4096;
  bool sv_redo_mid = true;
  bool sv_p2skip = true;
  bool sv_redo_large = false;
  int sv_budget = 2457;
  bool sv_reseed = true;
  int sv_reseed_budget = -1;
  int sv_retry_mode = SV_GRID_AUTO;
  bool sv_seedless = false;
  SvHist sv_hist[2];
  int64_t sv_small = 32768, sv_mid = 65536;
  hipStream_t stream_sv = nullptr, stream_sv2 = nullptr, stream_sv3 = nullptr;
  hipEvent_t ev_sv = nullptr;
  unsigned char* d_sv = nullptr;
  size_t sv_bytes = 0;
  void* h_sv_pin = nullptr;
  size_t h_sv_bytes = 0;
  int64_t sv_sources = 0, sv_redo = 0;
  int64_t sv_redo_dev = 0;
  int64_t sv_reseed_n = 0, sv_reseed_ok = 0;
  int64_t sv_retry_launched = 0, sv_retry_skipped = 0, sv_past_grid = 0, sv_seedless_n = 0, sv_seedless_done = 0;
  double xh_s[8] = {};
  unsigned char* d_q = nullptr;
  unsigned char* d_ql = nullptr;
  size_t q_bytes = 0, ql_bytes = 0;
  unsigned char* d_r = nullptr;
  unsigned char* d_rl = nullptr;
  unsigned char* d_rt = nullptr;
  size_t r_bytes = 0, rl_bytes = 0, rt_bytes = 0;
  bool mc = false;
  int32_t* d_mc_walk = nullptr;
  int64_t mc_nwalk = 0;
  int32_t* d_mc_levels = nullptr;
  std::vector<int64_t> mc_level_off;
  int32_t* d_mc_dangling = nullptr;
  int64_t mc_ndangling = 0;
  int mc_T = 0;
  double mc_walk_ms = 0.0;
  int64_t mc_walks = 0;
};

inline void plan_free(ppr_plan* p) {
  if (!p) return;
  hipFree(p->d_rp); hipFree(p->d_colx); hipFree(p->d_part); hipFree(p->d_ids); hipFree(p->d_sc); hipFree(p->d_rix); hipFree(p->d_rmin);
  hipFree(p->d_len); hipFree(p->d_all); hipFree(p->d_act[0]); hipFree(p->d_act[1]);
  hipFree(p->d_cand); hipFree(p->d_tier_lists); hipFree(p->d_tier_cnt); hipFree(p->d_tier_cap); hipFree(p->d_big);
  hipFree(p->d_ovf); hipFree(p->d_gath); hipFree(p->d_dlast); hipFree(p->d_xs);
  hipFree(p->d_maxdiff); hipFree(p->d_stats); hipFree(p->d_work); hipFree(p->d_scratch);
  hipFree(p->d_out_ids); hipFree(p->d_out_sc); hipFree(p->d_out_len);
  if (p->ev_a) hipEventDestroy(p->ev_a);
  if (p->ev_b) hipEventDestroy(p->ev_b);
  if (p->ev_m0) hipEventDestroy(p->ev_m0);
  if (p->ev_m1) hipEventDestroy(p->ev_m1);
  for (int i = 0; i < ppr_plan::MAX_REGIONS; i++) {
    if (p->ev_part[i]) hipEventDestroy(p->ev_part[i]);
    if (p->ev_buck[i]) hipEventDestroy(p->ev_buck[i]);
    if (p->ev_fin[i]) hipEventDestroy(p->ev_fin[i]);
  }
  if (p->ev_wave) hipEventDestroy(p->ev_wave);
  for (int i = 0; i < 2 * ppr_plan::NKST; i++)
    if (p->ev_k[i]) hipEventDestroy(p->ev_k[i]);
  if (p->ev_hot0) hipEventDestroy(p->ev_hot0);
  for (int i = 0; i < ppr_plan::MAX_REGIONS; i++)
    if (p->ev_hot[i]) hipEventDestroy(p->ev_hot[i]);
  if (p->stream5) hipStreamDestroy(p->stream5);
  hipFree(p->d_hot_bits); hipFree(p->d_hot_idx); hipFree(p->d_hot_keys); hipFree(p->d_hot_w);
  hipFree(p->d_hot_hist); hipFree(p->d_hot_list); hipFree(p->d_indeg);
  if (p->stream2) hipStreamDestroy(p->stream2);
  if (p->stream3) hipStreamDestroy(p->stream3);
  if (p->stream4) hipStreamDestroy(p->stream4);
  if (p->comm) ncclCommDestroy(p->comm);
  hipFree(p->d_xsend); hipFree(p->d_xrecv); hipFree(p->d_xsz); hipFree(p->d_xtmp);
  hipFree(p->d_xowner); hipFree(p->d_xcmask); hipFree(p->d_xlists); hipFree(p->d_own);
  if (p->h_hub_pin) hipHostFree(p->h_hub_pin);
  if (p->h_desc_pin) hipHostFree(p->h_desc_pin);
  if (p->h_xs_pin) hipHostFree(p->h_xs_pin);
  hipFree(p->d_sv);
  hipFree(p->d_xg);
  hipFree(p->d_wovl);
  hipFree(p->d_wl);
  hipFree(p->d_q); hipFree(p->d_ql);
  hipFree(p->d_r); hipFree(p->d_rl); hipFree(p->d_rt);
  if (p->h_sv_pin) hipHostFree(p->h_sv_pin);
  if (p->ev_sv) hipEventDestroy(p->ev_sv);
  if (getenv("PPR_TIMING") && p->sv_sources)
    fprintf(stderr, "ppr_timing sieve_sources %lld sieve_redo %lld sieve_redo_dev %lld sieve_reseed %lld "
            "sieve_reseed_ok %lld\n", (long long)p->sv_sources, (long long)p->sv_redo, (long long)p->sv_redo_dev,
            (long long)p->sv_reseed_n, (long long)p->sv_reseed_ok);
  if (getenv("PPR_TIMING") && p->sv_sources)
    fprintf(stderr, "ppr_timing sieve_retry launched %lld skipped %lld past_grid %lld seedless %lld seedless_done %lld\n",
            (long long)p->sv_retry_launched, (long long)p->sv_retry_skipped, (long long)p->sv_past_grid,
            (long long)p->sv_seedless_n, (long long)p->sv_seedless_done);
  if (getenv("PPR_TIMING") && p->sv_sources)
    fprintf(stderr, "ppr_timing xhubs_host_s gather %.4f classify %.4f sieve_launch %.4f engines %.4f sieve_wait %.4f "
            "handback_plan %.4f handback_run %.4f\n", p->xh_s[0], p->xh_s[1], p->xh_s[2], p->xh_s[3], p->xh_s[4],
            p->xh_s[5], p->xh_s[6]);
  if (getenv("PPR_TIMING") && p->xr_redo)
    fprintf(stderr, "ppr_timing xr_redo_sources %lld\n", (long long)p->xr_redo);
  if (getenv("PPR_TIMING") && p->wave_redo)
    fprintf(stderr, "ppr_timing wave_redo_sources %lld\n", (long long)p->wave_redo);
  if (getenv("PPR_TIMING") && p->xg_sources)
    fprintf(stderr, "ppr_timing hbm_table_sources %lld\n", (long long)p->xg_sources);
  if (getenv("PPR_TIMING") && p->spec_redo)
    fprintf(stderr, "ppr_timing spec_redo_sources %lld\n", (long long)p->spec_redo);
  if (getenv("PPR_TIMING") && p->host_plan_calls)
    fprintf(stderr, "ppr_timing hub_paths lds_rank %u lds_rank64 %u one_shot %d\n", p->lds_rank, p->lds_rank64,
            (int)p->hub_bw2);
  if (getenv("PPR_TIMING") && p->host_plan_calls)
    fprintf(stderr, "ppr_timing hub_planning host_s %.4f calls %lld hubs %lld order_s %.4f batches_s %.4f\n",
            p->host_plan_s, (long long)p->host_plan_calls, (long long)p->host_plan_hubs, p->host_plan_part[0],
            p->host_plan_part[1]);
  if (p->d_diag) {
    std::vector<unsigned long long> hv(PPR_DIAG_SLOTS);
    if (hipMemcpy(hv.data(), p->d_diag, 8 * hv.size(), hipMemcpyDeviceToHost) == hipSuccess) {
      unsigned long long h[PPR_DIAG_BASE];
      for (int i = 0; i < PPR_DIAG_BASE; i++) {
        h[i] = hv[i];
        for (int sh = 1; sh <= PPR_DIAG_SHARDS; sh++) h[i] += hv[(size_t)sh * PPR_DIAG_BASE + i];
      }
      fprintf(stderr, "ppr_diag bucket_w: log2(x) | buckets by len, Mcycles | by distinct keys | by kept keys\n");
      for (int b = 0; b < 32; b++)
        if (h[b] || h[64 + b] || h[96 + b])
          fprintf(stderr, "ppr_diag %2d %12llu %12.1f | %12llu | %12llu\n", b, h[b], h[32 + b] / 1e6,
                  h[64 + b], h[96 + b]);
      if (h[144])
        fprintf(stderr, "ppr_diag hot pass: %d keys, %llu tasks, hub candidates %.3e staged (cold) %.3e (%.1f %%), "
                "task ms: longest %.2f, first %.2f, sum %.1f\n", p->hot_n, h[144], p->diag_hub_cand, (double)h[140],
                100.0 * (double)h[140] / (p->diag_hub_cand > 0 ? p->diag_hub_cand : 1.0), h[141] / 1e5, h[143] / 1e5,
                h[142] / 1e5);
      if (p->diag_cap_src > 0)
        fprintf(stderr, "ppr_diag sources beyond the bucket cap %.0f, candidates %.3e of %.3e\n", p->diag_cap_src,
                p->diag_cap_cand, p->diag_hub_cand);
      if (h[296]) {
        const double tot = (double)(h[288] + h[289] + h[290] + h[291] + h[292] + h[293] + h[294] + h[295]);
        fprintf(stderr, "ppr_diag one-shot buckets %llu, %.1f K cycles each: loads+clear %.1f %% P1 %.1f %% P2 %.1f %% "
                "P3 %.1f %% P4 %.1f %% count+select %.1f %% append atomic %.1f %% emit %.1f %%\n", h[296],
                tot / 1e3 / (double)h[296], 100.0 * h[288] / tot, 100.0 * h[289] / tot, 100.0 * h[290] / tot,
                100.0 * h[291] / tot, 100.0 * h[292] / tot, 100.0 * h[293] / tot, 100.0 * h[294] / tot,
                100.0 * h[295] / tot);
      }
      if (h[152])
        fprintf(stderr, "ppr_diag spilled buckets %llu, records %llu (%.1f per bucket)\n", h[152], h[153],
                (double)h[153] / (double)h[152]);
      if (h[150])
        fprintf(stderr, "ppr_diag rows merged %llu, unchanged (norm1 = 0) %llu (%.2f %%)\n", h[150], h[151],
                100.0 * (double)h[151] / (double)h[150]);
      if (h[180]) {
        fprintf(stderr, "ppr_diag speculative bound: %llu hub sources, %llu failed (%.3f %%); failures by iteration:",
                h[180], h[181], 100.0 * (double)h[181] / (double)h[180]);
        for (int it = 0; it < 32; it++)
          if (h[224 + it]) fprintf(stderr, " %d:%llu", it, h[224 + it]);
        fprintf(stderr, "\n");
      }
      if (h[166]) {
        const double tot = (double)(h[160] + h[161] + h[162] + h[163] + h[164] + h[165]);
        fprintf(stderr, "ppr_diag bucket_w phases, 1 wave in 8 (%llu waves, %.3e records, %.1f Gcycles): work+setup %.1f %% loads %.1f %% "
                "insert %.1f %% accumulate %.1f %% compact+select %.1f %% append %.1f %%; buckets selecting (U > L) %llu, "
                "entries appended %.3e\n", h[166], (double)h[167], tot / 1e9, 100.0 * h[160] / tot, 100.0 * h[161] / tot,
                100.0 * h[162] / tot, 100.0 * h[163] / tot, 100.0 * h[164] / tot, 100.0 * h[165] / tot, h[168],
                (double)h[169]);
        const double acc = (double)(h[172] + h[173] + h[174] + h[175]);
        if (acc > 0)
          fprintf(stderr, "ppr_diag bucket_w accumulate phases: A occurrence ranks %.1f %% B slot offsets %.1f %% "
                  "C value placement %.1f %% D per-slot chains %.1f %%\n", 100.0 * h[172] / acc, 100.0 * h[173] / acc,
                  100.0 * h[174] / acc, 100.0 * h[175] / acc);
      }
      if (h[182])
// ... 95 lines not shown
```

approximated_personalized_pagerank_amd/csrc/ppr_common.h:

```cpp
#pragma once
#include <hip/hip_runtime.h>

#include "ppr_device.h"

namespace pprk {
using namespace pprd;

constexpr int NT = 4;
constexpr int TIER_WG = NT;
constexpr int TIER_BIG = NT + 1;
constexpr int NLISTS = NT + 2;
constexpr int MAX_L = 4096;
constexpr int WAVES_PER_BLOCK = 4;
constexpr int PPR_NSTATS = 8;
constexpr int PPR_DIAG_BASE = 304;
constexpr int PPR_DIAG_SHARDS = 256;
constexpr int PPR_DIAG_SLOTS = PPR_DIAG_BASE * (1 + PPR_DIAG_SHARDS);
__device__ __forceinline__ void diag_add(unsigned long long* d, int idx, unsigned long long v) {
  const uint32_t sh = (blockIdx.x * 7u + (threadIdx.x >> 6)) & (uint32_t)(PPR_DIAG_SHARDS - 1);
  atomicAdd(&d[(size_t)PPR_DIAG_BASE * (1 + sh) + idx], v);
}

struct GlbWork {
  int32_t v;
  int32_t pad;
  int64_t off;
  int64_t T;
};

__device__ __forceinline__ int64_t xcd_block(int64_t b, int64_t nb) {
  const int64_t q = nb / 8, r = nb % 8, x = b % 8;
  return (x < r ? x * (q + 1) : r * (q + 1) + (x - r) * q) + b / 8;
}

struct HubBatch {
  size_t d0, d1; int64_t cm, stg, pt, ntiles, nbuck, nrt, red, nseg; int maxP; int64_t nrange = 0;
  int64_t ntiles_s = 0; int maxP_s = 1;
};

struct DevGraph {
  const int64_t* rp;
  const int32_t* colx;
  int64_t n;
};

constexpr int NRANGE = 64;
constexpr int RANGE_BITS = 6;
__device__ __forceinline__ uint32_t row_range(int key) { return hash_b((uint32_t)key) >> (32 - RANGE_BITS); }

constexpr uint32_t HOT_TAG = 0x80000000u;

struct DevSlab {
  int32_t* ids;
  double* sc;
  int32_t* len;
  int64_t n;
  int32_t L;
  uint16_t* rix;
  double* rmin;
  const uint32_t* hbits;
  const uint16_t* hidx;
  const int32_t* hkeys;
  int hn;
  __device__ __forceinline__ int64_t row(int slot, int64_t u) const { return ((int64_t)slot * n + u) * L; }
  __device__ __forceinline__ int64_t lrow(int slot, int64_t u) const { return (int64_t)slot * n + u; }
  __device__ __forceinline__ int64_t xrow(int slot, int64_t u) const { return ((int64_t)slot * n + u) * NRANGE; }
  __device__ __forceinline__ int key(int32_t id) const { return id >= 0 ? id : hkeys[(uint32_t)id & 0x7fffffffu]; }
  template <bool HK>
  __device__ __forceinline__ int keyd(int32_t id) const { return HK ? key(id) : id; }
  __device__ __forceinline__ int32_t enc(int key) const {
    if (hn && ((hbits[(uint32_t)key >> 5] >> ((uint32_t)key & 31u)) & 1u)) return (int32_t)(HOT_TAG | hidx[key]);
    return key;
  }
};

__device__ __forceinline__ uint64_t wave_min_u64(uint64_t x) {
#pragma unroll
  for (int o = 32; o; o >>= 1) { const uint64_t y = (uint64_t)__shfl_xor((unsigned long long)x, o); x = y < x ? y : x; }
  return x;
}

__device__ __forceinline__ void write_row(const DevSlab& s, int slot, int v, uint64_t* rv, int* rk, int cnt,
                                          int Lp, bool scaled, double scale) {
  row_sort_hash(rv, rk, cnt, Lp);
  const int64_t r = s.row(slot, v);
  uint64_t mn = ~0ull;
  for (int i = lane_id(); i < cnt; i += WAVE) {
    double x = bitsd(rv[i]);
    if (scaled) x *= scale;
    s.ids[r + i] = s.enc(rk[i]);
    s.sc[r + i] = x;
    const uint64_t b = dbits(x);
    mn = b < mn ? b : mn;
  }
  mn = wave_min_u64(mn);
  const uint32_t q = (uint32_t)lane_id();
  int pos = 0;
// ... 136 lines not shown
  }
  wave_fence();
  double* dd = reinterpret_cast<double*>(hist);
#pragma unroll
  for (int q = 0; q < 2; q++) {
    if (!(q ? e1 : e0)) continue;
    const int key = q ? k1 : k0;
    uint32_t h = hash32((uint32_t)key) & hmask;
    double o = 0.0;
    for (int c = 0; c < hsize; c++) {
      const int cur = hk[h];
      if (cur == key) { const int j = hv[h]; o = bitsd(rv[j]); mf[j] = 1; break; }
      if (cur == EMPTY) break;
      h = (h + 1) & hmask;
    }
    dd[q ? r1 : r0] = fabs(bitsd(q ? v1 : v0) - o);
  }
  wave_fence();
  double p = 0.0;
  if (e0) p += dd[l];
  if (e1) p += dd[l + WAVE];
  if (f0 && !mf[l]) p += os0;
  if (f1 && !mf[l + WAVE]) p += os1;
#pragma unroll
  for (int o = 32; o; o >>= 1) p = p + __shfl_xor(p, o);
  wave_fence();
  return p;
}

template <class KeyAt, class ValAt>
__device__ __forceinline__ void finish_source(int v, int U, KeyAt keyat, ValAt valat,
                                              const DevSlab& s, const IterArgs& a, uint32_t* hist,
                                              uint64_t* rv, int* rk, int Lp, int* hk, int* hv,
                                              int* mf, unsigned long long* maxdiff,
                                              unsigned long long* stats, int dg = -1) {
  const int L = s.L;
  U = __builtin_amdgcn_readfirstlane(U);
  long long tl = (dg >= 0 && a.diag) ? (long long)clock64() : 0;
  const bool reg = Lp <= 2 * WAVE && !a.unit && !a.mc;
  const int cur = (a.active == 1) ? a.sB : a.sA;
  int o0 = EMPTY, o1 = EMPTY, olen = 0;
  double os0 = 0.0, os1 = 0.0;
  if (reg) {
    const int64_t ro = s.row(cur, v);
    const int l = lane_id();
    olen = __builtin_amdgcn_readfirstlane(s.len[s.lrow(cur, v)]);
    if (l < L) { o0 = s.ids[ro + l]; os0 = s.sc[ro + l]; }
    if (l + WAVE < L) { o1 = s.ids[ro + l + WAVE]; os1 = s.sc[ro + l + WAVE]; }
  }
  int cnt;
  if (U <= L) {
    for (int i = lane_id(); i < U; i += WAVE) { rv[i] = dbits(valat(i)); rk[i] = keyat(i); }
    cnt = U;
  } else {
    const uint32_t ts = tie_salt(v);
    const SelCrit c = select_top(U, L, keyat, valat, hist, ts);
    int base = 0;
    for (int i0 = 0; i0 < U; i0 += WAVE) {
      const int i = i0 + lane_id();
      bool sel = false;
      uint64_t vb = 0;
      int key = 0;
      if (i < U) { key = keyat(i); vb = dbits(valat(i)); sel = sel_test(c, vb, tie_w(key, ts)); }
      const uint64_t m = __ballot(sel);
      if (sel) { const int pos = base + __popcll(m & lanemask_lt()); rv[pos] = vb; rk[pos] = key; }
      base += __popcll(m);
    }
    cnt = L;
  }
  wave_fence();
  if (a.unit) {
    write_row(s, 0, v, rv, rk, cnt, Lp, false, 1.0);
    write_row(s, 1, v, rv, rk, cnt, Lp, false, 1.0);
    return;
  }
  if (a.mc) {
    const double f = a.damping / (double)(a.rp[v + 1] - a.rp[v]);
    write_row(s, 0, v, rv, rk, cnt, Lp, true, f);
    return;
  }
  const int nxt = cur ^ 1;
  fs_lap(a, dg, 0, tl);
  double d1;
  if (reg) {
    const int l = lane_id();
    const int k0 = l < cnt ? rk[l] : EMPTY, k1 = l + WAVE < cnt ? rk[l + WAVE] : EMPTY;
    const uint64_t v0 = l < cnt ? rv[l] : 0ull, v1 = l + WAVE < cnt ? rv[l + WAVE] : 0ull;
    wave_fence();
    d1 = finish_row_reg(s, nxt, v, cnt, k0, v0, k1, v1, l < olen ? s.key(o0) : EMPTY, os0,
                        l + WAVE < olen ? s.key(o1) : EMPTY, os1, olen, rv, hist, hk, hv, mf, Lp, a, dg, tl);
  } else {
    write_row(s, nxt, v, rv, rk, cnt, Lp, false, 1.0);
    fs_lap(a, dg, 1, tl);
    const int64_t ro = s.row(cur, v);
    const int olen2 = s.len[s.lrow(cur, v)];
    d1 = row_norm1(rv, rk, cnt, s.ids + ro, s.sc + ro, olen2, hk, hv, mf, 2 * Lp,
                   [&](int32_t id) { return s.key(id); });
  }
  fs_lap(a, dg, 2, tl);
  if (lane_id() == 0) {
    const unsigned long long b = (unsigned long long)dbits(d1);
    if (b > __hip_atomic_load(maxdiff, __ATOMIC_RELAXED, __HIP_MEMORY_SCOPE_AGENT)) atomicMax(maxdiff, b);
    if (a.diag) {
      atomicAdd(&a.diag[150], 1ull);
      if (d1 == 0.0) atomicAdd(&a.diag[151], 1ull);
    }
  }
  (void)stats;
}

}
```

Baseline: 3.892 million.

## Record and replay hub-merge plans across iterations when no row lengths changed

Splits the host-side planning of the xhubs and sieve paths (task classification, descriptor building, pinned upload) from kernel queueing. Planned descriptors are stored in device-side replay records so later iterations can skip the host rebuild and re-queue the same kernels. Replay is valid only while no row length has changed, which a new sharded device counter in the row-finish path tracks. This targets per-iteration host planning and H2D upload overhead, at the cost of an extra atomic per changed row, stats allocation and memset, and extra device buffers. Replay is disabled for sharded/multi-rank, hot, wave_by_d and seedless modes.

After: 3.987 million, median of 6. +2.5%, better.

```diff
diff --git a/approximated_personalized_pagerank_amd/csrc/grank.hip b/approximated_personalized_pagerank_amd/csrc/grank.hip
--- a/approximated_personalized_pagerank_amd/csrc/grank.hip
+++ b/approximated_personalized_pagerank_amd/csrc/grank.hip
@@ -154,7 +154,8 @@
   TRY(dalloc(&p->d_tier_cap, NT + 1));
   TRY(dalloc(&p->d_ovf, n));
   TRY(dalloc(&p->d_maxdiff, PPR_MAX_ITER_STATS + 1));
-  TRY(dalloc(&p->d_stats, PPR_NSTATS));
+  TRY(dalloc(&p->d_stats, PPR_NSTATS_ALL));
+  TRY(hipMemset(p->d_stats, 0, 8 * PPR_NSTATS_ALL) == hipSuccess ? PPR_OK : PPR_ERR_HIP);
   TRY(dalloc(&p->d_out_ids, (size_t)n * K));
   TRY(dalloc(&p->d_out_sc, (size_t)n * K));
   TRY(dalloc(&p->d_out_len, n));
@@ -251,6 +252,8 @@
     if (ent) p->nt_loads = (int)strtol(ent, nullptr, 0) & 3;
     const char* ewi = getenv("PPR_WHATIF");
     if (ewi) p->whatif = (int)strtol(ewi, nullptr, 0);
+    const char* erpl = getenv("PPR_REPLAY");
+    if (erpl) p->replay = atoi(erpl) != 0;
     const char* ebd = getenv("PPR_WAVE_BY_D");
     if (ebd) p->wave_by_d = atoi(ebd) != 0;
     const char* etd = getenv("PPR_WAVE_TDIV");
@@ -710,6 +713,15 @@
 
 static int run_merge_impl(ppr_plan* p, const IterArgs& a, const int32_t* list, int64_t count,
                           unsigned long long* maxdiff);
+static inline ReplayKnobs replay_knobs(const ppr_plan* p) {
+  ReplayKnobs k;
+  k.enabled = p->replay;
+  k.sharded = p->replay_sharded || p->comm != nullptr || p->lgroup != nullptr || p->nranks > 1;
+  k.wave_by_d = p->wave_by_d;
+  k.sv_seedless = p->sv_seedless;
+  k.hot = p->hot_cap > 0 || p->hot_n > 0;
+  return k;
+}
 
 static int ensure_scratch(ppr_plan* p, size_t need) {
   if (need <= p->scratch_bytes) return PPR_OK;
@@ -1263,6 +1275,7 @@
   const std::vector<int32_t>* deg = nullptr;
   const std::vector<int64_t>* dest = nullptr;
   std::vector<int32_t> xv;
+  const std::vector<int32_t>* xvp = nullptr;
 };
 static int xhubs_finish(ppr_plan* p, const IterArgs& a, XhDefer& df, unsigned long long* maxdiff);
 
@@ -1272,22 +1285,86 @@
   t = t2;
 }
 
+struct XrCls { int T, W; };
+static inline void xr_classes(const ppr_plan* p, XrCls (&cls)[3]) {
+  cls[0] = XrCls{std::min(2048, p->xr_T), std::min(2048, p->xr_T) / 512};
+  cls[1] = XrCls{std::min(4096, p->xr_T), std::min(4096, p->xr_T) / 512};
+  cls[2] = XrCls{p->xr_T, p->xr_T / 512};
+}
+
+static int xr_queue(ppr_plan* p, const IterArgs& a, const XrPlan& P, unsigned long long* maxdiff) {
+  hipStream_t sw = p->stream3 ? p->stream3 : p->stream;
+  DevGraph g{p->d_rp, p->d_colx, p->n};
+  const DevSlab s = dev_slab(p);
+  XrCls cls[3];
+  xr_classes(p, cls);
+  {
+    int rc = ensure_dev(&p->d_xs, &p->xs_bytes, P.total);
+    if (rc) return rc;
+  }
+  unsigned char* b = p->d_xs;
+  const XDesc* d_xd = (const XDesc*)(P.d_up + P.o_d);
+  const XTask* d_tk = (const XTask*)(P.d_up + P.o_t);
+  int32_t* d_pk = (int32_t*)(b + P.o_k);
+  double* d_ps = (double*)(b + P.o_s);
+  uint32_t* d_pc = (uint32_t*)(b + P.o_pc);
+  uint32_t* d_ds = (uint32_t*)(b + P.o_ds);
+  int32_t* d_of = (int32_t*)(b + P.o_of);
+  int32_t* d_ov = (int32_t*)(b + P.o_ov);
+  unsigned long long* d_xt = (unsigned long long*)(b + P.o_xt);
+  HIP_OK(hipMemsetAsync(b + P.o_z, 0, P.total - P.o_z, sw));
+  if (!a.unit && !a.mc) {
+    kst_begin(p, 5, sw);
+    p->kst_pend_bytes[5] = P.bytes;
+  }
+  const bool big_first = p->xr_big_first;
+  if (P.nxm) {
+    const int T = cls[0].T, W = cls[0].W;
+    const int budget = p->xr_budget_over ? 2 * T : std::min(T * 85 / 100, T - W * WAVE - WAVE);
+    hipLaunchKernelGGL(k_xm<4>, dim3((unsigned)P.nxm), dim3(64 * 4), xm_lds_bytes(T), sw, g, s, a,
+                       (const XmTask*)(P.d_up + P.o_m), T, budget, d_pk, d_ps, d_pc, d_ds, d_of, d_ov);
+    HIP_OK(hipGetLastError());
+    p->merge_launches++;
+  }
+  for (int c0 = 0; c0 < 3; c0++) {
+    const int c = big_first ? 2 - c0 : c0;
+    if (!P.tcount[c]) continue;
+    const int T = cls[c].T, W = cls[c].W;
+    const int budget = p->xr_budget_over ? 2 * T : std::min(T * 85 / 100, T - W * WAVE - WAVE);
+    hipLaunchKernelGGL(k_xr, dim3((unsigned)P.tcount[c]), dim3(64 * W), xr_lds_bytes(T, W, p->Lp), sw, g, s, a,
+                       d_xd, d_tk + P.tofs[c], T, budget, p->Lp, d_xt, d_pk, d_ps, d_pc, d_ds, d_of, d_ov, p->xr_cap);
+    HIP_OK(hipGetLastError());
+    p->merge_launches++;
+  }
+  if (P.nmulti) {
+    hipLaunchKernelGGL(k_xfinal<XDesc>, dim3((unsigned)P.nmulti), dim3(256), xf_lds_bytes(p->Lp, p->xf_stage), sw, s, a,
+                       d_xd, d_xt, d_pk, d_ps, d_pc, d_ds, d_of, p->d_dlast, p->Lp, p->xf_stage, maxdiff, p->d_stats);
+    HIP_OK(hipGetLastError());
+    p->merge_launches++;
+  }
+  if (P.nx > P.nmulti) {
+    hipLaunchKernelGGL(k_xfin1, dim3((unsigned)(P.nx - P.nmulti)), dim3(64), xf1_lds_bytes(p->Lp), sw, s, a, d_xd,
+                       (int)P.nmulti, d_pk, d_ps, d_pc, d_ds, d_of, p->d_dlast, p->Lp, maxdiff, p->d_stats);
+    HIP_OK(hipGetLastError());
+    p->merge_launches++;
+  }
+  if (!a.unit && !a.mc) kst_end(p, 5, sw, p->kst_pend_bytes[5]);
+  return PPR_OK;
+}
+
 static int run_xhubs_list(ppr_plan* p, const IterArgs& a, const std::vector<int32_t>& src,
                           const std::vector<int32_t>& cand, const std::vector<int32_t>& deg,
                           const std::vector<int64_t>& dest, unsigned long long* maxdiff, int depth,
-                          XhDefer* defer = nullptr) {
+                          XhDefer* defer = nullptr, XhRec* rec = nullptr) {
   const size_t n = src.size();
+  if (rec) rec->xr.simple = false;
   if (!n) return PPR_OK;
   auto tsub = std::chrono::steady_clock::now();
   hipStream_t st = p->stream;
   hipStream_t sw = p->stream3 ? p->stream3 : st;
-  DevGraph g{p->d_rp, p->d_colx, p->n};
-  const DevSlab s = dev_slab(p);
   const int64_t L = p->L;
-  struct Cls { int T, W; };
-  const Cls cls[3] = {{std::min(2048, p->xr_T), std::min(2048, p->xr_T) / 512},
-                      {std::min(4096, p->xr_T), std::min(4096, p->xr_T) / 512},
-                      {p->xr_T, p->xr_T / 512}};
+  XrCls cls[3];
+  xr_classes(p, cls);
   auto cap_of = [&](int T) { return (int64_t)T * p->xr_fill / 100; };
   static thread_local std::vector<int32_t> rng_tl;
   static thread_local std::vector<uint8_t> ci_tl;
@@ -1372,23 +1449,25 @@
   const size_t o_ov = off; off = al(off + 4 * (nx + 2));
   const size_t o_xt = off; off = al(off + 8 * (nx + 1));
   const size_t total = off;
-  std::vector<int32_t> ovl_h;
+  XrPlan lplan;
+  XrPlan& P = rec ? rec->xr : lplan;
+  P.n = n; P.nx = nx; P.nmulti = (size_t)nmulti; P.nxm = xmt.size(); P.ntask = ntask; P.pt = pt;
+  P.o_d = o_d; P.o_t = o_t; P.o_m = o_m; P.o_k = o_k; P.o_s = o_s; P.o_z = o_z; P.o_pc = o_pc; P.o_ds = o_ds;
+  P.o_of = o_of; P.o_ov = o_ov; P.o_xt = o_xt; P.total = total;
+  P.simple = nx && bsrc.empty() && xgs.empty();
   if (nx) {
     {
       int rc = ensure_dev(&p->d_xs, &p->xs_bytes, total);
       if (rc) return rc;
     }
-    unsigned char* b = p->d_xs;
-    XDesc* d_xd = (XDesc*)(b + o_d);
-    XTask* d_tk = (XTask*)(b + o_t);
-    int32_t* d_pk = (int32_t*)(b + o_k);
-    double* d_ps = (double*)(b + o_s);
-    uint32_t* d_pc = (uint32_t*)(b + o_pc);
-    uint32_t* d_ds = (uint32_t*)(b + o_ds);
-    int32_t* d_of = (int32_t*)(b + o_of);
-    int32_t* d_ov = (int32_t*)(b + o_ov);
-    unsigned long long* d_xt = (unsigned long long*)(b + o_xt);
     const size_t up = o_m + sizeof(XmTask) * xmt.size();
+    P.up = up;
+    P.d_up = p->d_xs;
+    if (rec && P.simple) {
+      int rc = ensure_dev(&rec->d_xr_up, &rec->xr_up_bytes, up + 256);
+      if (rc) return rc;
+      P.d_up = rec->d_xr_up;
+    }
     {
       int rc = ensure_pinned(&p->h_xs_pin, &p->h_xs_bytes, up);
       if (rc) return rc;
@@ -1396,59 +1475,29 @@
     unsigned char* hb = (unsigned char*)p->h_xs_pin;
     std::memcpy(hb + o_d, xd.data(), sizeof(XDesc) * nx);
     if (!xmt.empty()) std::memcpy(hb + o_m, xmt.data(), sizeof(XmTask) * xmt.size());
-    size_t tofs[3];
     {
       size_t k = 0;
       for (int c = 0; c < 3; c++) {
-        tofs[c] = k;
+        P.tofs[c] = k;
+        P.tcount[c] = tasks[c].size();
         if (!tasks[c].empty()) std::memcpy(hb + o_t + sizeof(XTask) * k, tasks[c].data(), sizeof(XTask) * tasks[c].size());
         k += tasks[c].size();
       }
     }
     sub_lap(p, 2, tsub);
-    HIP_OK(hipMemcpyAsync(b, hb, up, hipMemcpyHostToDevice, sw));
-    HIP_OK(hipMemsetAsync(b + o_z, 0, total - o_z, sw));
-    if (!a.unit && !a.mc) {
-      double bytes = 0.0;
+    HIP_OK(hipMemcpyAsync(P.d_up, hb, up, hipMemcpyHostToDevice, sw));
+    P.bytes = 0.0;
+    if (!a.unit && !a.mc)
       for (size_t i = 0; i < n; i++)
         if (rng[i] > 0)
-          bytes += 8.0 + 8.0 * deg[i] + 12.0 * ((double)cand[i] - 1.0) +
-                   24.0 * (double)std::min<int64_t>(L, (int64_t)cand[i] + 1) + 4.0;
-      kst_begin(p, 5, sw);
-      p->kst_pend_bytes[5] = bytes;
-    }
-    const bool big_first = p->xr_big_first;
-    if (!xmt.empty()) {
-      const int T = cls[0].T, W = cls[0].W;
-      const int budget = p->xr_budget_over ? 2 * T : std::min(T * 85 / 100, T - W * WAVE - WAVE);
-      hipLaunchKernelGGL(k_xm<4>, dim3((unsigned)xmt.size()), dim3(64 * 4), xm_lds_bytes(T), sw, g, s, a,
-                         (const XmTask*)(b + o_m), T, budget, d_pk, d_ps, d_pc, d_ds, d_of, d_ov);
-      HIP_OK(hipGetLastError());
-      p->merge_launches++;
-    }
-    for (int c0 = 0; c0 < 3; c0++) {
-      const int c = big_first ? 2 - c0 : c0;
-      if (tasks[c].empty()) continue;
-      const int T = cls[c].T, W = cls[c].W;
-      const int budget = p->xr_budget_over ? 2 * T : std::min(T * 85 / 100, T - W * WAVE - WAVE);
-      hipLaunchKernelGGL(k_xr, dim3((unsigned)tasks[c].size()), dim3(64 * W), xr_lds_bytes(T, W, p->Lp), sw, g, s, a,
-                         d_xd, d_tk + tofs[c], T, budget, p->Lp, d_xt, d_pk, d_ps, d_pc, d_ds, d_of, d_ov, p->xr_cap);
-      HIP_OK(hipGetLastError());
-      p->merge_launches++;
-    }
-    if (nmulti) {
-      hipLaunchKernelGGL(k_xfinal<XDesc>, dim3((unsigned)nmulti), dim3(256), xf_lds_bytes(p->Lp, p->xf_stage), sw, s, a,
-                         d_xd, d_xt, d_pk, d_ps, d_pc, d_ds, d_of, p->d_dlast, p->Lp, p->xf_stage, maxdiff, p->d_stats);
-      HIP_OK(hipGetLastError());
-      p->merge_launches++;
-    }
-    if ((int64_t)nx > nmulti) {
-      hipLaunchKernelGGL(k_xfin1, dim3((unsigned)((int64_t)nx - nmulti)), dim3(64), xf1_lds_bytes(p->Lp), sw, s, a, d_xd,
-                         (int)nmulti, d_pk, d_ps, d_pc, d_ds, d_of, p->d_dlast, p->Lp, maxdiff, p->d_stats);
-      HIP_OK(hipGetLastError());
-      p->merge_launches++;
-    }
-    if (!a.unit && !a.mc) kst_end(p, 5, sw, p->kst_pend_bytes[5]);
+          P.bytes += 8.0 + 8.0 * deg[i] + 12.0 * ((double)cand[i] - 1.0) +
+                     24.0 * (double)std::min<int64_t>(L, (int64_t)cand[i] + 1) + 4.0;
+    P.xv.resize(nx);
+    for (size_t i = 0; i < nx; i++) P.xv[i] = xd[i].v;
+    {
+      int rc = xr_queue(p, a, P, maxdiff);
+      if (rc) return rc;
+    }
   }
   sub_lap(p, 3, tsub);
   if (defer && defer->want && nx && bsrc.empty() && xgs.empty()) {
@@ -1456,8 +1505,8 @@
     defer->depth = depth;
     defer->o_ov = o_ov;
     defer->src = &src; defer->cand = &cand; defer->deg = &deg; defer->dest = &dest;
-    defer->xv.resize(nx);
-    for (size_t i = 0; i < nx; i++) defer->xv[i] = xd[i].v;
+    defer->xv = P.xv;
+    defer->xvp = nullptr;
     return PPR_OK;
   }
   std::vector<int32_t> fallback;
@@ -1530,7 +1579,7 @@
   std::vector<int32_t> rsrc, rcand, rdeg;
   std::vector<int64_t> rdest;
   for (int32_t d : od) {
-    const int32_t v = df.xv[(size_t)d];
+    const int32_t v = (df.xvp ? *df.xvp : df.xv)[(size_t)d];
     auto it = std::lower_bound(idx.begin(), idx.end(), std::make_pair(v, (int32_t)-1));
     if (it == idx.end() || it->first != v) return PPR_ERR_HIP;
     const size_t i = (size_t)it->second;
@@ -1544,7 +1593,7 @@
 }
 
 struct SvRun {
-  std::vector<int32_t> pos;
+  const SvPlan* plan = nullptr;
   size_t o_ovl = 0;
   size_t o_os = 0;
   size_t o_om = 0;
@@ -1557,16 +1606,14 @@
   bool live = false;
 };
 
-static int sieve_launch(ppr_plan* p, const IterArgs& a, const std::vector<int32_t>& src,
-                        const std::vector<int32_t>& cand, const std::vector<int32_t>& deg, unsigned long long* maxdiff,
-                        SvRun& run) {
+static int sieve_plan(ppr_plan* p, const std::vector<int32_t>& src, const std::vector<int32_t>& cand,
+                      const std::vector<int32_t>& deg, SvPlan& P, XhRec* rec) {
   const size_t n = src.size();
-  run.live = false;
+  P.n = n;
   if (!n) return PPR_OK;
   auto tsub = std::chrono::steady_clock::now();
-  DevGraph g{p->d_rp, p->d_colx, p->n};
-  const DevSlab s = dev_slab(p);
   const int Lp = p->Lp;
+  std::vector<int32_t>& pos = P.pos;
   auto klass = [&](int64_t c) { return c > p->sv_slice ? 0 : c >= p->sv_mid ? 1 : c >= p->sv_small ? 2 : 3; };
   auto step = [](int64_t c) { return std::min(255, (int)(8.0 * std::log2((double)std::max<int64_t>(1, c)))); };
   constexpr int NKEY = 4 * 256;
@@ -1581,8 +1628,8 @@
   for (int k = 0; k < NKEY; k++) cnt[k + 1] += cnt[k];
   const size_t nm = cnt[256], nx = n;
   size_t cls_end[3] = {cnt[512], cnt[768], cnt[NKEY]};
-  run.pos.resize(nx);
-  for (size_t i = 0; i < n; i++) run.pos[cnt[key[i]]++] = (int32_t)i;
+  pos.resize(nx);
+  for (size_t i = 0; i < n; i++) pos[cnt[key[i]]++] = (int32_t)i;
   auto sv_algo_bytes = [&](size_t i) {
     return 8.0 + 8.0 * deg[i] + 12.0 * ((double)cand[i] - 1.0) + 24.0 * (double)p->L + 4.0;
   };
@@ -1591,7 +1638,7 @@
   std::vector<SvTask> tasks;
   int64_t tg_total = 0;
   for (size_t k = 0; k < nm; k++) {
-    const size_t i = (size_t)run.pos[k];
+    const size_t i = (size_t)pos[k];
     SvDesc& d = desc[k];
     d = SvDesc{};
     d.v = src[i];
@@ -1634,20 +1681,62 @@
   { int r = ensure_pinned(&p->h_sv_pin, &p->h_sv_bytes, up); if (r) return r; }
   unsigned char* hb = (unsigned char*)p->h_sv_pin;
   int32_t* hv = (int32_t*)(hb + o_v);
-  for (size_t k = 0; k < nx; k++) hv[k] = src[(size_t)run.pos[k]];
+  for (size_t k = 0; k < nx; k++) hv[k] = src[(size_t)pos[k]];
   if (nm) std::memcpy(hb + o_d, desc.data(), sizeof(SvDesc) * nm);
   if (nt) std::memcpy(hb + o_t, tasks.data(), sizeof(SvTask) * nt);
+  P.nm = nm; P.nt = nt;
+  for (int c = 0; c < 3; c++) P.cls_end[c] = cls_end[c];
+  P.o_v = o_v; P.o_d = o_d; P.o_t = o_t; P.up = up; P.o_sk = o_sk; P.o_sv = o_sv; P.o_z = o_z; P.o_ov = o_ov;
+  P.o_os = o_os; P.o_om = o_om; P.o_ol = o_ol; P.o_sn = o_sn; P.o_cn = o_cn; P.o_of = o_of; P.o_mk = o_mk;
+  P.o_sd = o_sd; P.o_pt = o_pt; P.o_gs = o_gs; P.o_gk = o_gk; P.o_ga = o_ga; P.o_gb = o_gb; P.total = total;
+  {
+    size_t c0 = nm;
+    for (int c = 0; c < 3; c++) {
+      double bytes = 0.0;
+      for (size_t k = c0; k < cls_end[c]; k++) bytes += sv_algo_bytes((size_t)pos[k]);
+      c0 = cls_end[c];
+      P.bytes[c] = bytes;
+    }
+    double bytes = 0.0;
+    for (size_t k = 0; k < nm; k++) bytes += sv_algo_bytes((size_t)pos[k]);
+    P.bytes[3] = bytes;
+  }
+  P.d_up = p->d_sv;
+  if (rec) {
+    int r = ensure_dev(&rec->d_sv_up, &rec->sv_up_bytes, up + 256);
+    if (r) return r;
+    P.d_up = rec->d_sv_up;
+  }
+  sub_lap(p, 5, tsub);
+  HIP_OK(hipMemcpyAsync(P.d_up, hb, up, hipMemcpyHostToDevice, p->stream_sv3));
+  return PPR_OK;
+}
+
+static int sieve_queue(ppr_plan* p, const IterArgs& a, const SvPlan& P, unsigned long long* maxdiff, SvRun& run) {
+  run.live = false;
+  run.plan = &P;
+  if (!P.n) return PPR_OK;
+  auto tsub = std::chrono::steady_clock::now();
+  DevGraph g{p->d_rp, p->d_colx, p->n};
+  const DevSlab s = dev_slab(p);
+  const int Lp = p->Lp;
+  const size_t nm = P.nm, nt = P.nt, nx = P.n;
+  const size_t* cls_end = P.cls_end;
+  const size_t o_v = P.o_v, o_d = P.o_d, o_t = P.o_t, o_sk = P.o_sk, o_sv = P.o_sv, o_z = P.o_z, o_ov = P.o_ov,
+               o_os = P.o_os, o_om = P.o_om, o_ol = P.o_ol, o_sn = P.o_sn, o_cn = P.o_cn, o_of = P.o_of,
+               o_mk = P.o_mk, o_sd = P.o_sd, o_pt = P.o_pt, o_gs = P.o_gs, o_gk = P.o_gk, o_ga = P.o_ga,
+               o_gb = P.o_gb, total = P.total;
+  { int r = ensure_dev(&p->d_sv, &p->sv_bytes, total); if (r) return r; }
   unsigned char* b = p->d_sv;
+  const unsigned char* bu = P.d_up;
   hipStream_t s1 = p->stream_sv, s2 = p->stream_sv2, s3 = p->stream_sv3;
-  sub_lap(p, 5, tsub);
-  HIP_OK(hipMemcpyAsync(b, hb, up, hipMemcpyHostToDevice, s3));
   HIP_OK(hipMemsetAsync(b + o_z, 0, total - o_z, s3));
   HIP_OK(hipEventRecord(p->ev_sv, s3));
   if (s1 != s3) HIP_OK(hipStreamWaitEvent(s1, p->ev_sv, 0));
   if (s2 != s3) HIP_OK(hipStreamWaitEvent(s2, p->ev_sv, 0));
-  const int32_t* d_v = (const int32_t*)(b + o_v);
-  const SvDesc* d_d = (const SvDesc*)(b + o_d);
-  const SvTask* d_t = (const SvTask*)(b + o_t);
+  const int32_t* d_v = (const int32_t*)(bu + o_v);
+  const SvDesc* d_d = (const SvDesc*)(bu + o_d);
+  const SvTask* d_t = (const SvTask*)(bu + o_t);
   int32_t* d_ov = (int32_t*)(b + o_ov);
   int32_t* d_os = (int32_t*)(b + o_os);
   int32_t* d_om = (int32_t*)(b + o_om);
@@ -1686,8 +1775,7 @@
     for (int c = 0; c < 3; c++) {
       const size_t cnt_c = cls_end[c] - c0;
       const int d0 = (int)c0;
-      double bytes = 0.0;
-      for (size_t k = c0; k < cls_end[c]; k++) bytes += sv_algo_bytes((size_t)run.pos[k]);
+      const double bytes = P.bytes[c];
       c0 = cls_end[c];
       if (!cnt_c) continue;
       const SvGeom G = geo[c];
@@ -1728,8 +1816,7 @@
     }
   }
   if (nm) {
-    double bytes = 0.0;
-    for (size_t k = 0; k < nm; k++) bytes += sv_algo_bytes((size_t)run.pos[k]);
+    const double bytes = P.bytes[3];
     kst_begin(p, 4, s1);
     const bool rs_can = seed_on(SV_LARGE);
     const int64_t gm = rs_can ? retry_grid(SvHist::MULTI, nm) : -1;
@@ -1805,13 +1892,16 @@
   std::vector<int32_t> od(novf);
   HIP_OK(hipMemcpyAsync(od.data(), p->d_sv + run.o_ovl + 4, 4 * (size_t)novf, hipMemcpyDeviceToHost, p->stream_sv));
   HIP_OK(hipStreamSynchronize(p->stream_sv));
-  for (int32_t d : od) back.push_back(run.pos[(size_t)d]);
+  for (int32_t d : od) back.push_back(run.plan->pos[(size_t)d]);
   p->sv_redo += novf;
   return PPR_OK;
 }
 
-static int run_xhubs(ppr_plan* p, const IterArgs& a, const int32_t* d_list, int64_t count, unsigned long long* maxdiff) {
+static int run_xhubs(ppr_plan* p, const IterArgs& a, const int32_t* d_list, int64_t count, unsigned long long* maxdiff,
+                     XhRec* R = nullptr, bool replay = false) {
   if (count <= 0) return PPR_OK;
+  replay = replay && R && R->live && R->count == count;
+  if (R && !replay) R->live = false;
   auto now = [] { return std::chrono::steady_clock::now(); };
   double lapv[8] = {0, 0, 0, 0, 0, 0, 0, 0};
   auto lap = [&](int k, std::chrono::steady_clock::time_point& t) {
@@ -1840,34 +1930,38 @@
   } laplog{p, a, lapv, t_in};
   hipStream_t st = p->stream;
   const size_t nh = (size_t)count;
-  {
-    size_t capb = p->h_hub_cap * 12;
-    void* ptr = p->h_hub_pin;
-    int r = ensure_pinned(&ptr, &capb, 20 * nh);
-    if (r) return r;
-    p->h_hub_pin = (int32_t*)ptr;
-    p->h_hub_cap = capb / 12;
-  }
-  if (4 * nh > (size_t)p->n) { int r = ensure_dev((unsigned char**)&p->d_gath, &p->gath_bytes, 16 * nh); if (r) return r; }
-  int32_t* d_g = 4 * nh > (size_t)p->n ? p->d_gath : p->d_ovf;
-  int32_t* h = p->h_hub_pin;
-  HIP_OK(hipMemcpyAsync(h, d_list, 4 * nh, hipMemcpyDeviceToHost, st));
-  hipLaunchKernelGGL(k_gather_sv, dim3((unsigned)((nh + 255) / 256)), dim3(256), 0, st, d_list, (int64_t)nh,
-                     p->d_cand, p->d_rp, (const int32_t*)p->d_dlast, dev_slab(p), a, d_g);
-  HIP_OK(hipGetLastError());
-  HIP_OK(hipMemcpyAsync(h + nh, d_g, 16 * nh, hipMemcpyDeviceToHost, st));
-  HIP_OK(hipStreamSynchronize(st));
-  std::vector<int32_t>& hcopy = p->xhs.h;
-  hcopy.assign(h, h + 5 * nh);
-  h = hcopy.data();
+  std::vector<int32_t>& hcopy = R ? R->h : p->xhs.h;
+  if (!replay) {
+    {
+      size_t capb = p->h_hub_cap * 12;
+      void* ptr = p->h_hub_pin;
+      int r = ensure_pinned(&ptr, &capb, 20 * nh);
+      if (r) return r;
+      p->h_hub_pin = (int32_t*)ptr;
+      p->h_hub_cap = capb / 12;
+    }
+    if (4 * nh > (size_t)p->n) { int r = ensure_dev((unsigned char**)&p->d_gath, &p->gath_bytes, 16 * nh); if (r) return r; }
+    int32_t* d_g = 4 * nh > (size_t)p->n ? p->d_gath : p->d_ovf;
+    int32_t* hp = p->h_hub_pin;
+    HIP_OK(hipMemcpyAsync(hp, d_list, 4 * nh, hipMemcpyDeviceToHost, st));
+    hipLaunchKernelGGL(k_gather_sv, dim3((unsigned)((nh + 255) / 256)), dim3(256), 0, st, d_list, (int64_t)nh,
+                       p->d_cand, p->d_rp, (const int32_t*)p->d_dlast, dev_slab(p), a, d_g);
+    HIP_OK(hipGetLastError());
+    HIP_OK(hipMemcpyAsync(hp + nh, d_g, 16 * nh, hipMemcpyDeviceToHost, st));
+    HIP_OK(hipStreamSynchronize(st));
+    hcopy.assign(hp, hp + 5 * nh);
+  }
+  const int32_t* h = hcopy.data();
   lap(0, tl);
   const bool sieve = p->sv_enabled && a.xs && !a.unit && !a.mc && p->hot_n == 0;
-  std::vector<int32_t>& src = p->xhs.src; std::vector<int32_t>& cand = p->xhs.cand;
-  std::vector<int32_t>& deg = p->xhs.deg; std::vector<int32_t>& ssrc = p->xhs.ssrc;
-  std::vector<int32_t>& scand = p->xhs.scand; std::vector<int32_t>& sdeg = p->xhs.sdeg;
-  std::vector<int32_t>& sidx = p->xhs.sidx;
-  std::vector<int64_t>& dest = p->xhs.dest;
-  src.clear(); cand.clear(); deg.clear(); ssrc.clear(); scand.clear(); sdeg.clear(); sidx.clear(); dest.clear();
+  std::vector<int32_t>& src = R ? R->src : p->xhs.src; std::vector<int32_t>& cand = R ? R->cand : p->xhs.cand;
+  std::vector<int32_t>& deg = R ? R->deg : p->xhs.deg; std::vector<int32_t>& ssrc = R ? R->ssrc : p->xhs.ssrc;
+  std::vector<int32_t>& scand = R ? R->scand : p->xhs.scand; std::vector<int32_t>& sdeg = R ? R->sdeg : p->xhs.sdeg;
+  std::vector<int32_t>& sidx = R ? R->sidx : p->xhs.sidx;
+  std::vector<int64_t>& dest = R ? R->dest : p->xhs.dest;
+  if (!replay) {
+    src.clear(); cand.clear(); deg.clear(); ssrc.clear(); scand.clear(); sdeg.clear(); sidx.clear(); dest.clear();
+  }
   auto estimate = [&](size_t i) {
     const int64_t dl = h[3 * nh + i];
     const int64_t c = (int64_t)h[nh + i];
@@ -1888,7 +1982,7 @@
     if (c > p->sv_slice) return false;
     return c >= p->sv_mid ? short_large : c >= p->sv_small ? short_mid : p->sv_redo_mid;
   };
-  for (size_t i = 0; i < nh; i++) {
+  for (size_t i = 0; i < nh && !replay; i++) {
     const int32_t c = h[nh + i];
     if (sieve && c >= p->sv_min && c < (1 << 30) &&
         (h[4 * nh + i] == (int32_t)p->L || (seedless && short_ok(c)))) {
@@ -1905,18 +1999,41 @@
   }
   lap(1, tl);
   SvRun run;
+  SvPlan svl;
+  SvPlan& svp = R ? R->sv : svl;
   const int64_t rl0 = p->sv_retry_launched, rp0 = p->sv_retry_skipped;
+  auto xr_replay = [&](XhDefer& d) -> int {
+    if (src.empty()) return PPR_OK;
+    int r = xr_queue(p, a, R->xr, maxdiff);
+    if (r) return r;
+    d.live = true;
+    d.depth = 0;
+    d.o_ov = R->xr.o_ov;
+    d.src = &src; d.cand = &cand; d.deg = &deg; d.dest = &dest;
+    d.xvp = &R->xr.xv;
+    return PPR_OK;
+  };
+  auto sieve_go = [&]() -> int {
+    if (ssrc.empty()) return PPR_OK;
+    if (!replay) { int r = sieve_plan(p, ssrc, scand, sdeg, svp, R); if (r) return r; }
+    return sieve_queue(p, a, svp, maxdiff, run);
+  };
   XhDefer df;
   df.want = p->xh_first && src.size() > ssrc.size();
-  if (df.want) { int r = run_xhubs_list(p, a, src, cand, deg, dest, maxdiff, 0, &df); if (r) return r; }
-  if (!ssrc.empty()) { int r = sieve_launch(p, a, ssrc, scand, sdeg, maxdiff, run); if (r) return r; }
+  if (df.want) { int r = replay ? xr_replay(df) : run_xhubs_list(p, a, src, cand, deg, dest, maxdiff, 0, &df, R); if (r) return r; }
+  { int r = sieve_go(); if (r) return r; }
   lap(2, tl);
-  if (df.want) {
+  if (!df.want && replay) { int r = xr_replay(df); if (r) return r; }
+  if (df.want || replay) {
     int r = xhubs_finish(p, a, df, maxdiff);
     if (r) return r;
   } else if (!src.empty()) {
-    int r = run_xhubs_list(p, a, src, cand, deg, dest, maxdiff, 0);
+    int r = run_xhubs_list(p, a, src, cand, deg, dest, maxdiff, 0, nullptr, R);
     if (r) return r;
+  }
+  if (R && !replay) {
+    R->count = count;
+    R->live = src.empty() || R->xr.simple;
   }
   lap(3, tl);
   std::vector<int32_t>& back = p->xhs.back;
@@ -1928,7 +2045,7 @@
   if (getenv("PPR_SV_LOG")) {
     long long hn[4] = {0, 0, 0, 0}, hc[4] = {0, 0, 0, 0}, sc = 0;
     std::vector<int32_t> desc_of(ssrc.size(), 0);
-    for (size_t d = 0; d < run.pos.size(); d++) desc_of[(size_t)run.pos[d]] = (int32_t)d;
+    for (size_t d = 0; d < svp.pos.size() && !ssrc.empty(); d++) desc_of[(size_t)svp.pos[d]] = (int32_t)d;
     for (size_t k = 0; k < back.size(); k++) {
       int c = 0;
       while (c < 3 && (size_t)desc_of[(size_t)back[k]] >= run.cls_end[c]) c++;
@@ -1946,16 +2063,17 @@
             (long long)(p->sv_seedless_done - sd0));
   }
   if (back.empty()) return PPR_OK;
-  src.clear(); cand.clear(); deg.clear(); dest.clear();
+  std::vector<int32_t> bsrc, bcand, bdeg;
+  std::vector<int64_t> bdest;
   for (int32_t k : back) {
     const size_t i = (size_t)sidx[(size_t)k];
-    src.push_back(h[i]);
-    cand.push_back(h[nh + i]);
-    deg.push_back(h[2 * nh + i]);
-    dest.push_back(estimate(i));
+    bsrc.push_back(h[i]);
+    bcand.push_back(h[nh + i]);
+    bdeg.push_back(h[2 * nh + i]);
+    bdest.push_back(estimate(i));
   }
   lap(5, tl);
-  const int r = run_xhubs_list(p, a, src, cand, deg, dest, maxdiff, 0);
+  const int r = run_xhubs_list(p, a, bsrc, bcand, bdeg, bdest, maxdiff, 0);
   lap(6, tl);
   return r;
 }
@@ -1970,14 +2088,36 @@
     HIP_OK(hipEventRecord(p->ev_wave, p->stream_wave));
     HIP_OK(hipStreamWaitEvent(p->stream, p->ev_wave, 0));
   }
+  const bool clock = !rc && a.xs && !a.mc;
+  unsigned long long lenchg = 0;
+  constexpr size_t NSH = (size_t)PPR_LENCHG_SHARDS * PPR_LENCHG_STRIDE;
+  if (clock) p->rp_shards.resize(NSH);
+  auto sum_shards = [&] {
+    lenchg = 0;
+    for (int k = 0; k < PPR_LENCHG_SHARDS; k++) lenchg += p->rp_shards[(size_t)k * PPR_LENCHG_STRIDE];
+  };
   if (!rc && p->wave_x_launched) {
     int32_t nw = 0;
     HIP_OK(hipMemcpyAsync(&nw, p->d_wovl, 4, hipMemcpyDeviceToHost, p->stream));
+    if (clock) HIP_OK(hipMemcpyAsync(p->rp_shards.data(), p->d_stats + PPR_STAT_LENCHG, 8 * NSH, hipMemcpyDeviceToHost, p->stream));
     HIP_OK(hipStreamSynchronize(p->stream));
     if (nw) {
       p->wave_redo += nw;
       rc = run_xhubs(p, a, p->d_wovl + 1, nw, maxdiff);
-    }
+      if (!rc && clock) {
+        HIP_OK(hipMemcpyAsync(p->rp_shards.data(), p->d_stats + PPR_STAT_LENCHG, 8 * NSH, hipMemcpyDeviceToHost, p->stream));
+        HIP_OK(hipStreamSynchronize(p->stream));
+      }
+    }
+  } else if (clock) {
+    HIP_OK(hipMemcpyAsync(p->rp_shards.data(), p->d_stats + PPR_STAT_LENCHG, 8 * NSH, hipMemcpyDeviceToHost, p->stream));
+    HIP_OK(hipStreamSynchronize(p->stream));
+  }
+  if (clock && !rc) {
+    sum_shards();
+    if (p->rp_clock.valid && !a.unit) p->rp_len_changes += (int64_t)(lenchg - p->rp_clock.len_changes);
+    p->rp_clock.len_changes = lenchg;
+    p->rp_clock.valid = true;
   }
   if (rc || a.mc) return rc;
   HIP_OK(hipEventRecord(p->ev_m1, p->stream));
@@ -2076,24 +2216,69 @@
     p->h_hub_pin = (int32_t*)ptr;
     p->h_hub_cap = capb / 12;
   }
+  ReplayRec* RR = nullptr;
+  int64_t rp_begin = 0;
+  bool replayed = false;
+  {
+    const int part = a.active == 1 ? 1 : 0;
+    const ReplayKnobs kn = replay_knobs(p);
+    const bool grank_update = a.xs && !a.unit && !a.mc && (a.active == 0 || a.active == 1);
+    const bool in_list = grank_update && list >= p->d_act[part] && list + count <= p->d_act[part] + p->nact[part];
+    if (grank_update) replay_begin_update(p->rp_clock, a.iter, count, p->nact[part ^ 1], in_list);
+    if (in_list && replay_allowed(kn)) {
+      RR = &p->rp[part];
+      rp_begin = (int64_t)(list - p->d_act[part]);
+      replayed = replay_valid(RR->stamp, p->rp_clock, part, rp_begin, rp_begin + count, kn);
+      if (!replayed) {
+        if (RR->stamp.live) p->rp_dropped++;
+        RR->stamp.live = false;
+        for (XhRec& x : RR->xh) x.live = false;
+        int rc = ensure_dev((unsigned char**)&RR->d_tl, &RR->tl_bytes, 4 * (size_t)NLISTS * (size_t)count);
+        if (rc) return rc;
+        RR->tl_cap = count;
+        if (!RR->d_st) HIP_OK(hipMalloc((void**)&RR->d_st, 8 * 4));
+        HIP_OK(hipMemsetAsync(RR->d_st, 0, 8 * 4, st));
+      }
+    }
+  }
+  int32_t* const tlists = RR ? RR->d_tl : p->d_tier_lists;
+  const int64_t tcap = RR ? RR->tl_cap : p->n;
+  unsigned long long* const cls_stats = RR ? RR->d_st : p->d_stats;
+  uint32_t cnt[NLISTS + 1];
 reclassify:
-  HIP_OK(hipMemsetAsync(p->d_tier_cnt, 0, sizeof(uint32_t) * (NLISTS + 2), st));
-  const int cls_pw = count <= CLS_SMALL ? 1 : CLS_PER_WAVE;
-  const int64_t cls_pb = (int64_t)cls_pw * WAVES_PER_BLOCK;
-  const int64_t nb = (count + cls_pb - 1) / cls_pb;
-  hipLaunchKernelGGL(k_classify, dim3((unsigned)nb), dim3(256), 0, st, g, s, a, list, count,
-                     p->d_tier_cap, p->d_tier_lists, p->d_tier_cnt, p->n, p->d_cand, p->d_stats, p->d_big, cls_pw,
-                     (p->wave_by_d && a.xs && !a.unit && !a.mc) ? (const int32_t*)p->d_dlast : nullptr);
-  HIP_OK(hipGetLastError());
-  if (!a.unit && p->max_deg > CLS_BIG_DEG) {
-    hipLaunchKernelGGL(k_classify_big, dim3((unsigned)std::min<int64_t>(256, count)), dim3(CLS_BIG_THREADS), 0, st, g,
-                       s, a, p->d_tier_cap,
-                       p->d_tier_lists, p->d_tier_cnt, p->n, p->d_cand, p->d_stats, p->d_big,
+  if (!replayed) {
+    HIP_OK(hipMemsetAsync(p->d_tier_cnt, 0, sizeof(uint32_t) * (NLISTS + 2), st));
+    const int cls_pw = count <= CLS_SMALL ? 1 : CLS_PER_WAVE;
+    const int64_t cls_pb = (int64_t)cls_pw * WAVES_PER_BLOCK;
+    const int64_t nb = (count + cls_pb - 1) / cls_pb;
+    hipLaunchKernelGGL(k_classify, dim3((unsigned)nb), dim3(256), 0, st, g, s, a, list, count,
+                       p->d_tier_cap, tlists, p->d_tier_cnt, tcap, p->d_cand, cls_stats, p->d_big, cls_pw,
                        (p->wave_by_d && a.xs && !a.unit && !a.mc) ? (const int32_t*)p->d_dlast : nullptr);
-  }
-  HIP_OK(hipGetLastError());
-  uint32_t cnt[NLISTS + 1];
-  if (fused) {
+    HIP_OK(hipGetLastError());
+    if (!a.unit && p->max_deg > CLS_BIG_DEG) {
+      hipLaunchKernelGGL(k_classify_big, dim3((unsigned)std::min<int64_t>(256, count)), dim3(CLS_BIG_THREADS), 0, st, g,
+                         s, a, p->d_tier_cap,
+                         tlists, p->d_tier_cnt, tcap, p->d_cand, cls_stats, p->d_big,
+                         (p->wave_by_d && a.xs && !a.unit && !a.mc) ? (const int32_t*)p->d_dlast : nullptr);
+    }
+    HIP_OK(hipGetLastError());
+  }
+  if (RR && a.stats) {
+    hipLaunchKernelGGL(k_stats_add, dim3(1), dim3(64), 0, st, p->d_stats, (const unsigned long long*)RR->d_st);
+    HIP_OK(hipGetLastError());
+  }
+  if (replayed) {
+    std::memcpy(cnt, RR->cnt, sizeof(cnt));
+    p->rp_replayed++;
+    if (!p->ev_rp) HIP_OK(hipEventCreateWithFlags(&p->ev_rp, hipEventDisableTiming));
+    HIP_OK(hipEventRecord(p->ev_rp, st));
+    hipStream_t side[5] = {p->stream_wave, p->stream3, p->stream_sv, p->stream_sv2, p->stream_sv3};
+    for (int i = 0; i < 5; i++) {
+      bool seen = !side[i] || side[i] == st;
+      for (int j = 0; j < i; j++) seen = seen || side[j] == side[i];
+      if (!seen) HIP_OK(hipStreamWaitEvent(side[i], p->ev_rp, 0));
+    }
+  } else if (fused) {
     static_assert(NLISTS + 1 < GATHER_HDR, "tier counters and the pending count fit the header");
     hipLaunchKernelGGL(k_gather_cand_deg_dev, dim3((unsigned)((count + 255) / 256)), dim3(256), 0, st,
                        p->d_tier_lists + (int64_t)TIER_BIG * p->n, p->d_tier_cnt, NLISTS + 1, TIER_BIG,
@@ -2114,6 +2299,11 @@
   } else {
     HIP_OK(hipMemcpyAsync(cnt, p->d_tier_cnt, sizeof(cnt), hipMemcpyDeviceToHost, st));
     HIP_OK(hipStreamSynchronize(st));
+    if (RR) {
+      std::memcpy(RR->cnt, cnt, sizeof(cnt));
+      RR->stamp = replay_stamp(p->rp_clock, a.active == 1 ? 1 : 0, rp_begin, rp_begin + count);
+      if (RR->stamp.live) p->rp_recorded++;
+    }
   }
   hipStream_t sw = p->stream_wave ? p->stream_wave : st;
   bool wave_ev = false;
@@ -2163,7 +2353,7 @@
       const int Tw = std::max(64, p->tierT[t] >> p->wave_tdiv);
       const WList wl = wls[t];
       const bool split = wl.cap != 0;
-      const int32_t* tl = p->d_tier_lists + (int64_t)t * p->n;
+      const int32_t* tl = tlists + (int64_t)t * tcap;
       const size_t wlds = split ? lds_wave_bytes_xs(Tw) : lds_wave_bytes_x(Tw, p->Lp);
       const int64_t step = split ? wchunk : (int64_t)cnt[t];
       for (int64_t c0 = 0; c0 < (int64_t)cnt[t]; c0 += step) {
@@ -2202,10 +2392,16 @@
   if (wave_ev) kst_end(p, 0, sw, 0.0);
   if (a.xs) {
     int r = PPR_OK;
+    static_assert(ReplayRec::NCALL == NLISTS, "one recorded run_xhubs call per tier list");
     for (int t = 0; t < NT && !r; t++)
-      if (cnt[t] && !p->tierT[t]) r = run_xhubs(p, a, p->d_tier_lists + (int64_t)t * p->n, cnt[t], maxdiff);
-    if (!r && cnt[TIER_WG]) r = run_xhubs(p, a, p->d_tier_lists + (int64_t)TIER_WG * p->n, cnt[TIER_WG], maxdiff);
-    if (!r && cnt[TIER_BIG]) r = run_xhubs(p, a, p->d_tier_lists + (int64_t)TIER_BIG * p->n, cnt[TIER_BIG], maxdiff);
+      if (cnt[t] && !p->tierT[t])
+        r = run_xhubs(p, a, tlists + (int64_t)t * tcap, cnt[t], maxdiff, RR ? &RR->xh[t] : nullptr, replayed);
+    if (!r && cnt[TIER_WG])
+      r = run_xhubs(p, a, tlists + (int64_t)TIER_WG * tcap, cnt[TIER_WG], maxdiff, RR ? &RR->xh[TIER_WG] : nullptr,
+                    replayed);
+    if (!r && cnt[TIER_BIG])
+      r = run_xhubs(p, a, tlists + (int64_t)TIER_BIG * tcap, cnt[TIER_BIG], maxdiff, RR ? &RR->xh[TIER_BIG] : nullptr,
+                    replayed);
     return r;
   }
   if (cnt[TIER_WG]) {
@@ -2300,6 +2496,7 @@
   p->hot_built_it = -1;
   if (p->d_dlast) HIP_OK(hipMemsetAsync(p->d_dlast, 0, 4 * (size_t)std::max<int64_t>(1, p->n), p->stream));
   p->sv_hist[0] = p->sv_hist[1] = SvHist{};
+  plan_replay_drop(p);
   IterArgs a = iter_args(p, 0, true);
   int rc = init_dangling(p, p->d_all + p->n_nd, p->n - p->n_nd);
   if (rc) return rc;
@@ -2588,6 +2785,7 @@
 }
 
 static int xunpack_nodes(ppr_plan* p, int nxt, const int32_t* list, int64_t cnt, const unsigned char* buf) {
+  plan_replay_drop(p);
   if (cnt == 0) return PPR_OK;
   hipLaunchKernelGGL(k_xunpack, dim3((unsigned)((cnt + 3) / 4)), dim3(256), 0, p->stream, dev_slab(p), nxt, list, cnt,
                      buf);
@@ -3139,6 +3337,8 @@
   if (iterations == 0) return PPR_ERR_ITERS;
   if (p->nranks > 1 && !p->comm && !p->lgroup) return PPR_ERR_ARG;
   HIP_OK(hipSetDevice(p->device));
+  p->replay_sharded = true;
+  plan_replay_drop(p);
   hipStream_t s = p->stream;
   HIP_OK(hipMemsetAsync(p->d_maxdiff, 0, 8 * (PPR_MAX_ITER_STATS + 1), s));
   HIP_OK(hipMemsetAsync(p->d_stats, 0, 8 * PPR_NSTATS, s));
diff --git a/approximated_personalized_pagerank_amd/csrc/mccp2.hip b/approximated_personalized_pagerank_amd/csrc/mccp2.hip
--- a/approximated_personalized_pagerank_amd/csrc/mccp2.hip
+++ b/approximated_personalized_pagerank_amd/csrc/mccp2.hip
@@ -111,6 +111,7 @@
   end = std::min<int64_t>(p->mc_nwalk, end);
   if (end <= begin) return PPR_OK;
   HIP_OK(hipSetDevice(p->device));
+  plan_replay_drop(p);
   McArgs m;
   m.R = walks;
   m.nw = (uint64_t)((double)walks * p->damping);
@@ -137,6 +138,7 @@
   if (!p || !p->mc) return PPR_ERR_ARG;
   if (p->n == 0) return PPR_OK;
   HIP_OK(hipSetDevice(p->device));
+  plan_replay_drop(p);
   const DevSlab s = dev_slab(p);
   if (p->mc_ndangling) {
     hipLaunchKernelGGL(k_mc_selfrow, dim3((unsigned)((p->mc_ndangling + 3) / 4)), dim3(256), 0, p->stream, s,
diff --git a/approximated_personalized_pagerank_amd/csrc/merge_wave.h b/approximated_personalized_pagerank_amd/csrc/merge_wave.h
--- a/approximated_personalized_pagerank_amd/csrc/merge_wave.h
+++ b/approximated_personalized_pagerank_amd/csrc/merge_wave.h
@@ -163,6 +163,10 @@
   }
 }
 
+__global__ void k_stats_add(unsigned long long* stats, const unsigned long long* add) {
+  if (threadIdx.x < 3 && add[threadIdx.x]) atomicAdd(&stats[threadIdx.x], add[threadIdx.x]);
+}
+
 __host__ __device__ constexpr size_t lds_wave_bytes(int T, int Lp) {
   return (size_t)T * 13 + (size_t)Lp * 12 + 1024 + (size_t)Lp * 20;
 }
diff --git a/approximated_personalized_pagerank_amd/csrc/plan.h b/approximated_personalized_pagerank_amd/csrc/plan.h
--- a/approximated_personalized_pagerank_amd/csrc/plan.h
+++ b/approximated_personalized_pagerank_amd/csrc/plan.h
@@ -9,6 +9,7 @@
 #include "../../include/ppr_hip.h"
 #include "ppr_common.h"
 #include "sv_plan.h"
+#include "replay_rule.h"
 
 using namespace pprk;
 
@@ -29,6 +30,48 @@
   return p;
 }
 
+
+struct SvPlan {
+  std::vector<int32_t> pos;
+  size_t n = 0, nm = 0, nt = 0;
+  size_t cls_end[3] = {0, 0, 0};
+  size_t o_v = 0, o_d = 0, o_t = 0, up = 0, o_sk = 0, o_sv = 0, o_z = 0, o_ov = 0, o_os = 0, o_om = 0, o_ol = 0,
+         o_sn = 0, o_cn = 0, o_of = 0, o_mk = 0, o_sd = 0, o_pt = 0, o_gs = 0, o_gk = 0, o_ga = 0, o_gb = 0, total = 0;
+  double bytes[4] = {0, 0, 0, 0};
+  unsigned char* d_up = nullptr;
+};
+struct XrPlan {
+  size_t n = 0, nx = 0, nmulti = 0, nxm = 0, ntask = 0;
+  size_t tcount[3] = {0, 0, 0}, tofs[3] = {0, 0, 0};
+  int64_t pt = 0;
+  size_t o_d = 0, o_t = 0, o_m = 0, up = 0, o_k = 0, o_s = 0, o_z = 0, o_pc = 0, o_ds = 0, o_of = 0, o_ov = 0,
+         o_xt = 0, total = 0;
+  double bytes = 0.0;
+  bool simple = false;
+  std::vector<int32_t> xv;
+  unsigned char* d_up = nullptr;
+};
+struct XhRec {
+  bool live = false;
+  int64_t count = 0;
+  std::vector<int32_t> h, src, cand, deg, ssrc, scand, sdeg, sidx;
+  std::vector<int64_t> dest;
+  SvPlan sv;
+  XrPlan xr;
+  unsigned char* d_sv_up = nullptr;
+  unsigned char* d_xr_up = nullptr;
+  size_t sv_up_bytes = 0, xr_up_bytes = 0;
+};
+struct ReplayRec {
+  static constexpr int NCALL = NT + 2;
+  ReplayStamp stamp;
+  uint32_t cnt[NLISTS + 1] = {};
+  int32_t* d_tl = nullptr;
+  int64_t tl_cap = 0;
+  size_t tl_bytes = 0;
+  unsigned long long* d_st = nullptr;
+  XhRec xh[NCALL];
+};
 
 struct ppr_plan {
   int device = 0;
@@ -199,6 +242,13 @@
     std::vector<uint32_t> svcnt;
   } xhs;
   double xh_sub[8] = {0, 0, 0, 0, 0, 0, 0, 0};
+  bool replay = true;
+  bool replay_sharded = false;
+  ReplayRec rp[2];
+  ReplayClock rp_clock;
+  std::vector<unsigned long long> rp_shards;
+  hipEvent_t ev_rp = nullptr;
+  int64_t rp_recorded = 0, rp_replayed = 0, rp_dropped = 0, rp_len_changes = 0;
   int xr_cap = 0;
   int wave_cap = 0;
   unsigned char* d_wl = nullptr;
@@ -257,6 +307,14 @@
   int64_t mc_walks = 0;
 };
 
+inline void plan_replay_drop(ppr_plan* p) {
+  for (ReplayRec& r : p->rp) {
+    if (r.stamp.live) p->rp_dropped++;
+    r.stamp.live = false;
+  }
+  replay_drop(p->rp_clock);
+}
+
 inline void plan_free(ppr_plan* p) {
   if (!p) return;
   hipFree(p->d_rp); hipFree(p->d_colx); hipFree(p->d_part); hipFree(p->d_ids); hipFree(p->d_sc); hipFree(p->d_rix); hipFree(p->d_rmin);
@@ -300,6 +358,15 @@
   hipFree(p->d_r); hipFree(p->d_rl); hipFree(p->d_rt);
   if (p->h_sv_pin) hipHostFree(p->h_sv_pin);
   if (p->ev_sv) hipEventDestroy(p->ev_sv);
+  if (p->ev_rp) hipEventDestroy(p->ev_rp);
+  for (ReplayRec& r : p->rp) {
+    hipFree(r.d_tl); hipFree(r.d_st);
+    for (XhRec& x : r.xh) { hipFree(x.d_sv_up); hipFree(x.d_xr_up); }
+  }
+  if (getenv("PPR_TIMING") && p->xsum && !p->mc)
+    fprintf(stderr, "ppr_timing replay recorded %lld replayed %lld dropped %lld len_changes %lld\n",
+            (long long)p->rp_recorded, (long long)p->rp_replayed, (long long)p->rp_dropped,
+            (long long)p->rp_len_changes);
   if (getenv("PPR_TIMING") && p->sv_sources)
     fprintf(stderr, "ppr_timing sieve_sources %lld sieve_redo %lld sieve_redo_dev %lld sieve_reseed %lld "
             "sieve_reseed_ok %lld\n", (long long)p->sv_sources, (long long)p->sv_redo, (long long)p->sv_redo_dev,
diff --git a/approximated_personalized_pagerank_amd/csrc/ppr_common.h b/approximated_personalized_pagerank_amd/csrc/ppr_common.h
--- a/approximated_personalized_pagerank_amd/csrc/ppr_common.h
+++ b/approximated_personalized_pagerank_amd/csrc/ppr_common.h
@@ -13,6 +13,9 @@
 constexpr int MAX_L = 4096;
 constexpr int WAVES_PER_BLOCK = 4;
 constexpr int PPR_NSTATS = 8;
+constexpr int PPR_STAT_LENCHG = PPR_NSTATS;
+constexpr int PPR_LENCHG_SHARDS = 256, PPR_LENCHG_STRIDE = 16;
+constexpr int PPR_NSTATS_ALL = PPR_NSTATS + PPR_LENCHG_SHARDS * PPR_LENCHG_STRIDE;
 constexpr int PPR_DIAG_BASE = 304;
 constexpr int PPR_DIAG_SHARDS = 256;
 constexpr int PPR_DIAG_SLOTS = PPR_DIAG_BASE * (1 + PPR_DIAG_SHARDS);
@@ -315,6 +318,7 @@
   const int nxt = cur ^ 1;
   fs_lap(a, dg, 0, tl);
   double d1;
+  int oldlen = olen;
   if (reg) {
     const int l = lane_id();
     const int k0 = l < cnt ? rk[l] : EMPTY, k1 = l + WAVE < cnt ? rk[l + WAVE] : EMPTY;
@@ -327,6 +331,7 @@
     fs_lap(a, dg, 1, tl);
     const int64_t ro = s.row(cur, v);
     const int olen2 = s.len[s.lrow(cur, v)];
+    oldlen = olen2;
     d1 = row_norm1(rv, rk, cnt, s.ids + ro, s.sc + ro, olen2, hk, hv, mf, 2 * Lp,
                    [&](int32_t id) { return s.key(id); });
   }
@@ -334,12 +339,13 @@
   if (lane_id() == 0) {
     const unsigned long long b = (unsigned long long)dbits(d1);
     if (b > __hip_atomic_load(maxdiff, __ATOMIC_RELAXED, __HIP_MEMORY_SCOPE_AGENT)) atomicMax(maxdiff, b);
+    if (cnt != oldlen)
+      atomicAdd(&stats[PPR_STAT_LENCHG + (v & (PPR_LENCHG_SHARDS - 1)) * PPR_LENCHG_STRIDE], 1ull);
     if (a.diag) {
       atomicAdd(&a.diag[150], 1ull);
       if (d1 == 0.0) atomicAdd(&a.diag[151], 1ull);
     }
   }
-  (void)stats;
-}
-
-}
+}
+
+}
diff --git a/approximated_personalized_pagerank_amd/csrc/replay_rule.h b/approximated_personalized_pagerank_amd/csrc/replay_rule.h
--- /dev/null
+++ b/approximated_personalized_pagerank_amd/csrc/replay_rule.h
@@ -0,0 +1,68 @@
+#pragma once
+#include <cstdint>
+
+struct ReplayKnobs {
+  bool enabled = true;
+  bool sharded = false;
+  bool wave_by_d = false;
+  bool sv_seedless = false;
+  bool hot = false;
+};
+inline bool replay_allowed(const ReplayKnobs& k) {
+  return k.enabled && !k.sharded && !k.wave_by_d && !k.sv_seedless && !k.hot;
+}
+
+struct ReplayClock {
+  uint64_t len_changes = 0;
+  uint64_t epoch = 0;
+  bool valid = false;
+  int last_it = -1;
+  int64_t covered = 0;
+};
+
+struct ReplayStamp {
+  bool live = false;
+  int part = -1;
+  int64_t begin = 0, end = 0;
+  uint64_t len_changes = 0;
+  uint64_t epoch = 0;
+};
+
+inline ReplayStamp replay_stamp(const ReplayClock& c, int part, int64_t begin, int64_t end) {
+  ReplayStamp s;
+  s.live = c.valid;
+  s.part = part;
+  s.begin = begin;
+  s.end = end;
+  s.len_changes = c.len_changes;
+  s.epoch = c.epoch;
+  return s;
+}
+
+inline bool replay_valid(const ReplayStamp& s, const ReplayClock& now, int part, int64_t begin, int64_t end,
+                         const ReplayKnobs& k) {
+  return replay_allowed(k) && s.live && now.valid && s.epoch == now.epoch && s.part == part && s.begin == begin &&
+         s.end == end && s.len_changes == now.len_changes;
+}
+
+inline void replay_drop(ReplayClock& c) {
+  c.epoch++;
+  c.valid = false;
+  c.last_it = -1;
+  c.covered = 0;
+}
+
+inline void replay_begin_update(ReplayClock& c, int it, int64_t count, int64_t prev_list, bool in_list) {
+  if (in_list && it == c.last_it) {
+    c.covered += count;
+    return;
+  }
+  const bool next = in_list && it == c.last_it + 1 && (c.last_it < 0 || c.covered == prev_list);
+  if (!next) {
+    const bool was_valid = c.valid;
+    replay_drop(c);
+    c.valid = was_valid && in_list;
+  }
+  c.last_it = it;
+  c.covered = count;
+}
```
